# cloneofsimo/vqgan-training

Hardware: NVIDIA H100
Metric: images/sec (higher is better)
Workload: dtype bf16

## Files before the change

include/vqb200.h:

```cpp
#ifndef VQB200_H_
#define VQB200_H_

#include <stddef.h>
#include <stdint.h>

#ifdef __cplusplus
extern "C" {
#endif

#define VQB_OK 0
#define VQB_EINVAL (-1)
#define VQB_ENODEVICE (-2)
#define VQB_ECUDA (-3)

#define VQB_MAX_VIEWS 16
#define VQB_MAX_TAPS 16

#define VQB_EPI_BIAS 1
#define VQB_EPI_RES 2
#define VQB_EPI_RELU 4
#define VQB_EPI_MASK 8
#define VQB_EPI_STATS 16

typedef struct VqbView {
    int64_t offset;
    int32_t Wv, Hv, Nv;
    int32_t _pad;
    int64_t sw, sh, sn;
} VqbView;

typedef struct VqbTap {
    int32_t view, dw, dh, _pad;
} VqbTap;

typedef struct VqbConvDesc {
    int32_t C;
    int32_t Cout;
    int32_t N, H, W;
    int32_t nviews, ntaps;
    int32_t flags;
    int32_t out_f32;
    int32_t _pad;
    int64_t on, oh, ow, oc;
    VqbView views[VQB_MAX_VIEWS];
    VqbTap taps[VQB_MAX_TAPS];
} VqbConvDesc;

int vqb_conv_gemm(const VqbConvDesc* d, const void* a, const void* w_packed ,
                  const float* bias, const void* res, const void* mask, void* out, float* stats, void* stream);

typedef struct VqbWgradDesc {
    int32_t C;
    int32_t Cout;
    int32_t N, H, W;
    int32_t nviews, ntaps;
    int32_t ksplit;
    int64_t ld_override;
    int64_t col_offset;
    VqbView dy_view;
    VqbView views[VQB_MAX_VIEWS];
    VqbTap taps[VQB_MAX_TAPS];
} VqbWgradDesc;

int vqb_conv_stats_ok(const VqbConvDesc* d);

int vqb_wgrad_gemm(const VqbWgradDesc* d, const void* dy, const void* x, float* partial, void* stream);

int vqb_wgrad_cols(int ntaps, int C);

int vqb_wgrad_reduce(const float* partial, float* grad, int ksplit, int Cout, int CoutPad, int Cin, int T, int nslots,
                     int C64, const int* tapmap_dev, int accumulate, void* stream);

int vqb_pack_weights(const float* w_oihw, void* out, int Cout, int Cin, int T, int nslots, const int* tapmap_dev,
                     int transpose, int Kpad, void* stream);

int vqb_pack_weights_fold(const float* w_oihw, void* out, int Cout, int Cin, int T, int nslots, const int* tapmask_dev,
                          int transpose, int Kpad, void* stream);
int vqb_wgrad_reduce_fold(const float* partial, float* grad, int ksplit, int Cout, int CoutPad, int Cin, int T,
                          int nslots, int C64, const int* tapmask_dev, void* stream);

int vqb_nchw_to_nhwc(const float* x, void* y, int N, int C, int H, int W, int Cpad, const float* shift,
                     const float* inv_scale, void* stream);
int vqb_nhwc_to_nchw(const void* g, float* gx, int N, int C, int H, int W, int Cpad, const float* inv_scale,
                     void* stream);
int vqb_nchw_to_nhwc_pad(const float* x, void* y, int N, int C, int H, int W, int Cpad, int pad, const float* shift,
                         const float* inv_scale, void* stream);
int vqb_nhwc_to_nchw_pad(const void* g, float* gx, int N, int C, int H, int W, int Cpad, int pad,
                         const float* inv_scale, void* stream);

int vqb_gn_silu_fwd(const void* x, void* y, const float* gamma, const float* beta, float* mr, double* ws, int N,
                    int HW, int C, int G, float eps, int silu, void* stream);
int vqb_gn_silu_fwd_pre(const void* x, void* y, const float* gamma, const float* beta, float* mr, const float* chsums,
                        int N, int HW, int C, int G, float eps, int silu, void* stream);
int vqb_gn_silu_apply(const void* x, void* y, const float* gamma, const float* beta, const float* mr, int N, int HW,
                      int C, int G, int silu, void* stream);
int vqb_gn_silu_bwd(const void* x, const void* dy, const void* add, void* dx, const float* gamma, const float* beta,
                    const float* mr, float* dgamma, float* dbeta, float* ws, int N, int HW, int C, int G, int silu,
                    float* dx_colsum, void* stream);

int vqb_wavelet_fwd(const float* x, void* y, const float* filt, int N, int C, int H, int W, int Cpad, void* stream);

int vqb_pack_weights_bf16(const void* w_oihw, void* out, int Cout, int Cin, int T, int nslots, const int* tapmap_dev,
                          int transpose, int Kpad, void* stream);
int vqb_pack_weights_fold_bf16(const void* w_oihw, void* out, int Cout, int Cin, int T, int nslots,
                               const int* tapmask_dev, int transpose, int Kpad, void* stream);
int vqb_nchw_to_nhwc_bf16(const void* x, void* y, int N, int C, int H, int W, int Cpad, const float* shift,
                          const float* inv_scale, void* stream);
int vqb_nchw_to_nhwc_pad_bf16(const void* x, void* y, int N, int C, int H, int W, int Cpad, int pad,
                              const float* shift, const float* inv_scale, void* stream);
int vqb_nhwc_to_nchw_bf16(const void* y, void* x, int N, int C, int H, int W, int Cpad, void* stream);
int vqb_wavelet_fwd_bf16(const void* x, void* y, const float* filt, int N, int C, int H, int W, int Cpad,
                         void* stream);

#define VQB_MAX_VIEWS_3D 8
#define VQB_MAX_TAPS_3D 27

typedef struct VqbView3d {
    int64_t offset;
    int32_t Wv, Hv, Tv, Nv;
    int64_t sw, sh, st, sn;
} VqbView3d;

typedef struct VqbTap3d {
    int32_t view, dw, dh, dt;
} VqbTap3d;

typedef struct VqbConv3dDesc {
    int32_t C;
    int32_t Cout;
    int32_t N, T, H, W;
    int32_t nviews, ntaps;
    int32_t flags;
    int32_t out_f32;
    int64_t on, ot, oh, ow, oc;
    VqbView3d views[VQB_MAX_VIEWS_3D];
    VqbTap3d taps[VQB_MAX_TAPS_3D];
} VqbConv3dDesc;

int vqb_conv3d_gemm(const VqbConv3dDesc* d, const void* a, const void* w_packed ,
                    const float* bias, const void* res, void* out, void* stream);

#define VQB_MAX_TAPS_3D_DGRAD 64
typedef struct VqbConv3dDgradDesc {
    int32_t C;
    int32_t Cout;
    int32_t N, T, H, W;
    int32_t nviews, ntaps;
    int32_t flags;
    int32_t out_f32;
    int64_t on, ot, oh, ow, oc;
    VqbView3d views[VQB_MAX_VIEWS_3D];
    VqbTap3d taps[VQB_MAX_TAPS_3D_DGRAD];
} VqbConv3dDgradDesc;

int vqb_conv3d_dgrad_gemm(const VqbConv3dDgradDesc* d, const void* dy, const void* w_packed ,
                          void* dx, void* stream);

typedef struct VqbWgrad3dDesc {
    int32_t C;
    int32_t Cout;
    int32_t N, T, H, W;
    int32_t nviews, ntaps;
    int32_t ksplit, _pad;
    int64_t ld_override;
    int64_t col_offset;
    VqbView3d dy_view;
    VqbView3d views[VQB_MAX_VIEWS_3D];
    VqbTap3d taps[VQB_MAX_TAPS_3D];
} VqbWgrad3dDesc;

int vqb_wgrad3d_gemm(const VqbWgrad3dDesc* d, const void* dy, const void* x, float* partial, void* stream);

int vqb_attn_fwd_hd(const void* qkv, void* out, float* lse, int N, int T, int C, int head_dim, void* stream);
int vqb_attn_bwd_hd(const void* qkv, const void* out, const void* dout, const float* lse, float* dvec, void* dqkv,
                    int N, int T, int C, int head_dim, void* stream);

int vqb_gauss_reparam(const void* z, const void* eps, void* out, int N, int Z, int64_t S, int bf16, void* stream);
int vqb_gauss_reparam_bwd(const float* g, const float* z, const float* eps, float* dz, int N, int Z, int64_t S,
                          void* stream);

int vqb_ncthw_frames_to_nhwc_pad(const float* x, void* y, int B, int C, int T, int H, int W, int Cpad, int pad,
// ... 67 lines not shown
```

vqgan-training_b200/ae.py:

```python
from __future__ import annotations

import math
import os
import sys

_HERE = os.path.dirname(os.path.abspath(__file__))
if _HERE not in sys.path:
    sys.path.insert(0, _HERE)

import torch
import torch.nn.functional as F
from torch import Tensor, nn

import ops
import plans
from utils import wavelet_transform_multi_channel


class Act:

    __slots__ = ("t", "C", "stats", "framed")

    def __init__(self, t: Tensor, C: int, stats=None, framed=False):
        self.t = t
        self.C = C
        self.stats = stats
        self.framed = framed

    @property
    def shape(self):
        n, h, w, _ = self.t.shape
        return (n, self.C, h, w)


def _param_dtype(module: nn.Module):
    p = next(module.parameters(), None)
    if p is None:
        return torch.float32
    ops.check_master_dtype(p, f"{type(module).__name__} parameter")
    return p.dtype


def _enter(x, module: nn.Module):
    if isinstance(x, Act):
        return x, False
    _param_dtype(module)
    return Act(ops.to_nhwc(x), x.shape[1]), True


def _exit(a: Act, external: bool, module: nn.Module):
    return ops.to_nchw(a.t, a.C, _param_dtype(module)) if external else a


def _stats_fusion() -> bool:
    return torch.is_grad_enabled()


def swish(x):
    if isinstance(x, Act):
        raise RuntimeError("swish on internal activations is fused into FP32GroupNorm.forward(..., silu=True)")
    return x * torch.sigmoid(x)


class StandardizedC2d(nn.Conv2d):

    def __init__(self, *args, **kwargs):
        super().__init__(*args, **kwargs)
        self._packed = ops.PackedCache()

    def _kind(self):
        k, s, p = self.kernel_size[0], self.stride[0], self.padding[0]
        if s == 1 and p == (k - 1) // 2:
            return "s1"
        if s == 2 and k == 3 and p == 0:
            return "s2"
        if s == k and p == 0:
            return "patch"
        raise NotImplementedError(f"conv k={k} s={s} p={p} is not on the hot path")

    def forward_act(self, a: Act, residual: Act = None, relu=False, input_is_relu=False, nchw_out=False,
                    want_stats=False):
        want_stats = want_stats and not nchw_out
        kind = "fat3" if a.framed else self._kind()
        out = ops.conv(a.t, self.weight, self.bias, self._packed, kind,
                       residual.t if residual is not None else None, relu, input_is_relu, nchw_out, want_stats)
        if nchw_out:
            return out
        if want_stats:
            return Act(out[0], self.out_channels, out[1])
        return Act(out, self.out_channels)

    def forward(self, x):
        if isinstance(x, Act):
            return self.forward_act(x)
        if self._kind() == "s2":
            raise RuntimeError("stride-2 StandardizedC2d is only reachable through Downsample")
        a, ext = _enter(x, self)
        return _exit(self.forward_act(a), ext, self)


class FP32GroupNorm(nn.GroupNorm):

    def __init__(self, *args, **kwargs):
        super().__init__(*args, **kwargs)

    def forward(self, input, silu: bool = False):
        a, ext = _enter(input, self)
        y = ops.group_norm_silu(a.t, self.weight, self.bias, self.num_groups, self.eps, silu, chsums=a.stats)
        return _exit(Act(y, a.C), ext, self)

    def forward_with_skip(self, a: "Act", silu: bool = True):
        y, skip = ops.group_norm_silu(a.t, self.weight, self.bias, self.num_groups, self.eps, silu, with_skip=True,
                                      chsums=a.stats)
        return Act(y, a.C), Act(skip, a.C)


class AttnBlock(nn.Module):
    def __init__(self, in_channels: int):
        super().__init__()
        self.in_channels = in_channels

        self.head_dim = 64
        self.num_heads = in_channels // self.head_dim
        self.norm = FP32GroupNorm(num_groups=32, num_channels=in_channels, eps=1e-6, affine=True)
        self.qkv = StandardizedC2d(in_channels, in_channels * 3, kernel_size=1, bias=False)
        self.proj_out = StandardizedC2d(in_channels, in_channels, kernel_size=1, bias=False)
        nn.init.normal_(self.proj_out.weight, std=0.2 / math.sqrt(in_channels))

    def attention(self, h_) -> Act:
        a, _ = _enter(h_, self)
        return self.attention_from_normed(self.norm(a))

    def attention_from_normed(self, h: Act) -> Act:
        qkv = self.qkv.forward_act(h)
        import attention as attn_core

        o = attn_core.mhsa(qkv.t, self.num_heads, self.head_dim)
        return Act(o, self.in_channels)

    def forward(self, x):
        a, ext = _enter(x, self)
        hn, a_skip = self.norm.forward_with_skip(a, silu=False)
        h = self.attention_from_normed(hn)
        out = self.proj_out.forward_act(h, residual=a_skip)
        return _exit(out, ext, self)


class ResnetBlock(nn.Module):
    def __init__(self, in_channels: int, out_channels: int):
        super().__init__()
        self.in_channels = in_channels
        out_channels = in_channels if out_channels is None else out_channels
        self.out_channels = out_channels
        self.norm1 = FP32GroupNorm(num_groups=32, num_channels=in_channels, eps=1e-6, affine=True)
        self.conv1 = StandardizedC2d(in_channels, out_channels, kernel_size=3, stride=1, padding=1)
        self.norm2 = FP32GroupNorm(num_groups=32, num_channels=out_channels, eps=1e-6, affine=True)
        self.conv2 = StandardizedC2d(out_channels, out_channels, kernel_size=3, stride=1, padding=1)
        if self.in_channels != self.out_channels:
            self.nin_shortcut = StandardizedC2d(in_channels, out_channels, kernel_size=1, stride=1, padding=0)

        nn.init.normal_(self.conv2.weight, std=0.0001 / self.out_channels)
        nn.init.zeros_(self.conv2.bias)
        self.counter = 0

    def _recompute(self, a: Act) -> Act:
        nin = self.nin_shortcut if self.in_channels != self.out_channels else None
        spec = (self.norm1.num_groups, self.norm1.eps, self.norm2.num_groups, self.norm2.eps, self.conv1._packed,
                self.conv2._packed, nin._packed if nin is not None else None)
        out, stats = ops.resnet_block_recompute(
            a.t, a.stats, spec, self.norm1.weight, self.norm1.bias, self.conv1.weight, self.conv1.bias,
            self.norm2.weight, self.norm2.bias, self.conv2.weight, self.conv2.bias,
            nin.weight if nin is not None else None, nin.bias if nin is not None else None)
        return Act(out, self.out_channels, stats)

    def forward(self, x):
        a, ext = _enter(x, self)
        if torch.is_grad_enabled() and getattr(self, "_vqb_recompute", False):
            return _exit(self._recompute(a), ext, self)
        h, a_skip = self.norm1.forward_with_skip(a, silu=True)
        h = self.conv1.forward_act(h, want_stats=_stats_fusion())
        h = self.norm2(h, silu=True)
        skip = self.nin_shortcut.forward_act(a_skip) if self.in_channels != self.out_channels else a_skip
        out = self.conv2.forward_act(h, residual=skip, want_stats=_stats_fusion())
        return _exit(out, ext, self)


def enable_recompute(module: nn.Module, enabled: bool = True) -> nn.Module:
    for m in module.modules():
        if isinstance(m, ResnetBlock):
            m._vqb_recompute = bool(enabled)
    return module


class Downsample(nn.Module):
    def __init__(self, in_channels: int):
        super().__init__()
        self.conv = StandardizedC2d(in_channels, in_channels, kernel_size=3, stride=2, padding=0)
# ... 254 lines not shown
```

vqgan-training_b200/csrc/common.cu:

```cuda
#include "common.cuh"

#include <atomic>
#include <cstring>
#include <cudaTypedefs.h>
#include <mutex>

namespace vqb {

static thread_local char g_err[512] = "";
static std::atomic<int> g_launches{0};

int set_error(int code, const char* fmt, ...) {
    va_list ap;
    va_start(ap, fmt);
    vsnprintf(g_err, sizeof(g_err), fmt, ap);
    va_end(ap);
    return code;
}

void count_launch(int n) { g_launches.fetch_add(n, std::memory_order_relaxed); }

typedef CUresult (*EncodeTiledFn)(CUtensorMap*, CUtensorMapDataType, cuuint32_t, void*, const cuuint64_t*,
                                  const cuuint64_t*, const cuuint32_t*, const cuuint32_t*, CUtensorMapInterleave,
                                  CUtensorMapSwizzle, CUtensorMapL2promotion, CUtensorMapFloatOOBfill);
// ... 7 lines not shown
        if (cudaGetDriverEntryPoint("cuTensorMapEncodeTiled", &p, cudaEnableDefault, &q) == cudaSuccess &&
            q == cudaDriverEntryPointSuccess)
            fn = reinterpret_cast<EncodeTiledFn>(p);
        else
            (void)cudaGetLastError();
    });
    return fn;
}

int encode_tmap_bf16(CUtensorMap* out, const void* base, int rank, const uint64_t* dims, const uint64_t* strides_bytes,
                     const uint32_t* box, int swizzle_bytes) {
    EncodeTiledFn fn = get_encode_fn();
    if (!fn) return set_error(VQB_ENODEVICE, "cuTensorMapEncodeTiled driver entry point unavailable");
    if ((reinterpret_cast<uintptr_t>(base) & 15u) != 0)
        return set_error(VQB_EINVAL, "tensor map base %p not 16-byte aligned", base);
    cuuint64_t gdim[5];
    cuuint64_t gstr[4];
    cuuint32_t bx[5];
    cuuint32_t es[5];
    for (int i = 0; i < rank; ++i) {
        gdim[i] = dims[i];
        bx[i] = box[i];
        es[i] = 1;
        if (box[i] == 0 || box[i] > 256) return set_error(VQB_EINVAL, "tensor map box[%d]=%u out of range", i, box[i]);
    }
    for (int i = 0; i + 1 < rank; ++i) {
        gstr[i] = strides_bytes[i];
        if (gstr[i] % 16 != 0) return set_error(VQB_EINVAL, "tensor map stride[%d]=%llu not a multiple of 16 B", i,
                                                (unsigned long long)gstr[i]);
    }
    CUtensorMapSwizzle sw = CU_TENSOR_MAP_SWIZZLE_NONE;
    if (swizzle_bytes == 32) sw = CU_TENSOR_MAP_SWIZZLE_32B;
    if (swizzle_bytes == 64) sw = CU_TENSOR_MAP_SWIZZLE_64B;
    if (swizzle_bytes == 128) sw = CU_TENSOR_MAP_SWIZZLE_128B;
    CUresult r = fn(out, CU_TENSOR_MAP_DATA_TYPE_BFLOAT16, static_cast<cuuint32_t>(rank), const_cast<void*>(base), gdim,
                    gstr, bx, es, CU_TENSOR_MAP_INTERLEAVE_NONE, sw, CU_TENSOR_MAP_L2_PROMOTION_L2_256B,
                    CU_TENSOR_MAP_FLOAT_OOB_FILL_NONE);
    if (r == CUDA_ERROR_INVALID_CONTEXT || r == CUDA_ERROR_NOT_INITIALIZED) {
        cudaFree(nullptr);
        r = fn(out, CU_TENSOR_MAP_DATA_TYPE_BFLOAT16, static_cast<cuuint32_t>(rank), const_cast<void*>(base), gdim, gstr,
               bx, es, CU_TENSOR_MAP_INTERLEAVE_NONE, sw, CU_TENSOR_MAP_L2_PROMOTION_L2_256B,
               CU_TENSOR_MAP_FLOAT_OOB_FILL_NONE);
    }
    if (r != CUDA_SUCCESS) {
        return set_error(VQB_ECUDA,
                         "cuTensorMapEncodeTiled failed (%d): rank %d dims [%llu %llu %llu %llu] box [%u %u %u %u] "
                         "stride0 %llu",
                         (int)r, rank, (unsigned long long)gdim[0], (unsigned long long)(rank > 1 ? gdim[1] : 0),
                         (unsigned long long)(rank > 2 ? gdim[2] : 0), (unsigned long long)(rank > 3 ? gdim[3] : 0),
                         bx[0], rank > 1 ? bx[1] : 0, rank > 2 ? bx[2] : 0, rank > 3 ? bx[3] : 0,
                         (unsigned long long)(rank > 1 ? gstr[0] : 0));
    }
    return VQB_OK;
}

int num_sms() {
    static int n = 0;
    if (n == 0) {
        int dev = 0;
        if (cudaGetDevice(&dev) != cudaSuccess) return 0;
        if (cudaDeviceGetAttribute(&n, cudaDevAttrMultiProcessorCount, dev) != cudaSuccess) n = 0;
    }
    return n;
}

bool device_is_sm90() {
    int dev = 0, major = 0;
    if (cudaGetDevice(&dev) != cudaSuccess) {
        (void)cudaGetLastError();
        return false;
    }
    if (cudaDeviceGetAttribute(&major, cudaDevAttrComputeCapabilityMajor, dev) != cudaSuccess) {
        (void)cudaGetLastError();
        return false;
    }
    return major == 9;
}

}

extern "C" {

const char* vqb_last_error(void) { return vqb::g_err; }
int vqb_version(void) { return 103; }
int vqb_device_ok(void) { return (vqb::device_is_sm90() && vqb::get_encode_fn() != nullptr) ? 1 : 0; }
int vqb_kernel_launch_count(void) { return vqb::g_launches.load(std::memory_order_relaxed); }

}
```

vqgan-training_b200/csrc/conv_gemm.cu:

```cuda
#include "common.cuh"
#include "ptx.cuh"

#include <cstring>

namespace vqb {

constexpr int kBlockM = 128;
constexpr int kBlockK = 64;
constexpr int kABytes = kBlockM * kBlockK * 2;
constexpr int kThreads = 384;
constexpr int kMaxStages = 8;
constexpr int kConsumerWarps = 8;
constexpr int kProducerRegs = 40;
constexpr int kConsumerRegs = 232;
constexpr int kStagedKChunksPerTensor = 18;

struct alignas(64) ConvParams {
    static constexpr int kRank = 4;
    static constexpr int kViews = VQB_MAX_VIEWS;
    CUtensorMap amap[VQB_MAX_VIEWS];
    CUtensorMap bmap;
    CUtensorMap omap;
    CUtensorMap emap;
    int32_t tap_view[VQB_MAX_TAPS];
    int32_t tap_dw[VQB_MAX_TAPS];
    int32_t tap_dh[VQB_MAX_TAPS];
    int32_t ntaps, kchunks, C, Cout;
    int32_t N, H, W;
    int32_t lbw, lbh, lbn;
    int32_t tiles_w, tiles_h;
    int32_t n_tiles, total_tiles;
    int32_t stages, do_stats;
    int32_t flags, out_f32;
    int32_t vec_store, _pad0;
    int64_t on, oh, ow, oc;
    void* out;
    const void* res;
    const void* mask;
    const float* bias;
    float* stats;
};

template <int kTaps>
struct alignas(64) Conv3dParamsT {
    static constexpr int kRank = 5;
    static constexpr int kViews = VQB_MAX_VIEWS_3D;
    CUtensorMap amap[VQB_MAX_VIEWS_3D];
    CUtensorMap bmap;
    int32_t tap_view[kTaps];
    int32_t tap_dw[kTaps];
    int32_t tap_dh[kTaps];
    int32_t tap_dt[kTaps];
    int32_t ntaps, kchunks, C, Cout;
    int32_t N, T, H, W;
    int32_t lbw, lbh, lbt, lbn;
    int32_t tiles_w, tiles_h, tiles_t;
    int32_t n_tiles, total_tiles;
    int32_t stages, do_stats;
    int32_t flags, out_f32;
    int32_t vec_store, _pad0;
    int64_t on, ot, oh, ow, oc;
    void* out;
    const void* res;
    const void* mask;
    const float* bias;
    float* stats;
};
using Conv3dParams = Conv3dParamsT<VQB_MAX_TAPS_3D>;
using Conv3dDgradParams = Conv3dParamsT<VQB_MAX_TAPS_3D_DGRAD>;

template <int BN, class P, bool kStaged>
__global__ void __launch_bounds__(kThreads, 1) conv_gemm_kernel(const __grid_constant__ P p) {
    constexpr bool kR5 = P::kRank == 5;
    static_assert(!kStaged || (!kR5 && BN >= 64), "the staged epilogue stores whole 64-channel slabs of 2-D outputs");
    extern __shared__ uint8_t smem_raw[];
    constexpr uint32_t kBBytes = BN * kBlockK * 2;
    constexpr uint32_t kStageBytes = kABytes + kBBytes;
    uint8_t* base = smem_raw + ((1024u - (smem_u32(smem_raw) & 1023u)) & 1023u);
    const uint32_t stages = p.stages;
    constexpr uint32_t kSlabBytes = kBlockM * kBlockK * 2;
    constexpr uint32_t kEpiBytes = kBlockM * BN * 2;
    constexpr uint32_t kRowOff[4] = {0, 8 * 128, 64 * 128, 72 * 128};
    uint8_t* epi = base + stages * kStageBytes;
    float* sStat = reinterpret_cast<float*>(epi + (kStaged ? 2 * kEpiBytes : 0));
    uint64_t* full = reinterpret_cast<uint64_t*>(sStat + kConsumerWarps * BN * 2);
    uint64_t* empty = full + stages;
    uint64_t* order = empty + stages;
    uint64_t* epi_full = order + 2;
    uint64_t* epi_empty = epi_full + 2;
    const uint32_t wg = threadIdx.x >> 7;
    const uint32_t warp = (threadIdx.x >> 5) & 3u;
    const uint32_t lane = threadIdx.x & 31u;

    if (threadIdx.x == 0) {
        for (int v = 0; v < P::kViews; ++v) {
            bool used = false;
            for (int t = 0; t < p.ntaps; ++t) used |= (p.tap_view[t] == v);
            if (used) tma_prefetch_desc(&p.amap[v]);
        }
        tma_prefetch_desc(&p.bmap);
        if constexpr (kStaged) {
            tma_prefetch_desc(&p.omap);
            if (p.flags & (VQB_EPI_RES | VQB_EPI_MASK)) tma_prefetch_desc(&p.emap);
        }
        for (uint32_t i = 0; i < stages; ++i) {
            mbar_init(&full[i], 1);
            mbar_init(&empty[i], 4);
        }
        for (int c = 0; c < 2; ++c) {
            mbar_init(&order[c], 4);
            mbar_init(&epi_full[c], 1);
            mbar_init(&epi_empty[c], 1);
        }
        fence_mbar_init();
    }
    __syncthreads();

    const int num_kb = p.ntaps * p.kchunks;
    if (wg == 0) {
        setmaxnreg_dec<kProducerRegs>();
        if (warp == 0 && elect_one()) {
            uint32_t stage = 0, phase = 0;
            for (int tile = blockIdx.x, l = 0; tile < p.total_tiles; tile += gridDim.x, ++l) {
                const int n_tile = tile % p.n_tiles;
                const int m_tile = tile / p.n_tiles;
                const int tw = m_tile % p.tiles_w;
                const int th = (m_tile / p.tiles_w) % p.tiles_h;
                int tt = 0, tn;
                if constexpr (kR5) {
                    tt = (m_tile / (p.tiles_w * p.tiles_h)) % p.tiles_t;
                    tn = m_tile / (p.tiles_w * p.tiles_h * p.tiles_t);
                } else {
                    tn = m_tile / (p.tiles_w * p.tiles_h);
                }
                const int w0 = tw << p.lbw, h0 = th << p.lbh, n0 = tn << p.lbn;
                const int ncol0 = n_tile * BN;
                if constexpr (kStaged) {
                    const uint32_t c = l & 1;
                    mbar_wait(&epi_empty[c], ((l >> 1) & 1) ^ 1);
                    if (p.flags & (VQB_EPI_RES | VQB_EPI_MASK)) {
                        const int nslab = min(BN, p.Cout - ncol0) / kBlockK;
                        mbar_arrive_expect_tx(&epi_full[c], nslab * kSlabBytes);
                        for (int s = 0; s < nslab; ++s)
                            tma_load_4d(&p.emap, &epi_full[c], epi + c * kEpiBytes + s * kSlabBytes,
                                        ncol0 + s * kBlockK, w0, h0, n0);
                    } else {
                        mbar_arrive(&epi_full[c]);
                    }
                }
                for (int t = 0; t < p.ntaps; ++t) {
                    for (int kc = 0; kc < p.kchunks; ++kc) {
                        mbar_wait(&empty[stage], phase ^ 1);
                        uint8_t* a_dst = base + stage * kStageBytes;
                        mbar_arrive_expect_tx(&full[stage], kStageBytes);
                        if constexpr (kR5)
                            tma_load_5d(&p.amap[p.tap_view[t]], &full[stage], a_dst, kc * kBlockK, w0 + p.tap_dw[t],
                                        h0 + p.tap_dh[t], (tt << p.lbt) + p.tap_dt[t], n0);
                        else
                            tma_load_4d(&p.amap[p.tap_view[t]], &full[stage], a_dst, kc * kBlockK, w0 + p.tap_dw[t],
                                        h0 + p.tap_dh[t], n0);
                        tma_load_2d(&p.bmap, &full[stage], a_dst + kABytes, t * p.C + kc * kBlockK, ncol0);
                        if (++stage == stages) {
                            stage = 0;
                            phase ^= 1;
                        }
                    }
                }
            }
        }
        return;
    }

    setmaxnreg_inc<kConsumerRegs>();
    const uint32_t cw = wg - 1;
    const uint32_t cwarp = cw * 4 + warp;
    const uint32_t wtid = threadIdx.x & 127u;
    const uint32_t ring = smem_u32(base);
    const bool has_bias = p.flags & VQB_EPI_BIAS, has_res = p.flags & VQB_EPI_RES;
    const bool do_relu = !kR5 && (p.flags & VQB_EPI_RELU), has_mask = !kR5 && (p.flags & VQB_EPI_MASK);
    const bool vec_path = p.vec_store != 0;
    const bool reduce = !kR5 && p.do_stats;
    const __nv_bfloat16* res = reinterpret_cast<const __nv_bfloat16*>(p.res);
    const __nv_bfloat16* mask = reinterpret_cast<const __nv_bfloat16*>(p.mask);
    float acc[2][BN / 2];
#pragma unroll
    for (int mb = 0; mb < 2; ++mb)
#pragma unroll
        for (int i = 0; i < BN / 2; ++i) acc[mb][i] = 0.f;
    uint32_t stage = 0, phase = 0;
    for (int l = static_cast<int>(cw);; l += 2) {
        const int tile = blockIdx.x + l * gridDim.x;
        if (tile >= p.total_tiles) break;
        if (l > 0) {
            stage += num_kb;
            phase ^= (stage / stages) & 1u;
            stage %= stages;
            mbar_wait(&order[cw ^ 1u], ((l - 1) >> 1) & 1);
        }
        uint32_t prev = 0;
        for (int kb = 0; kb < num_kb; ++kb) {
            mbar_wait(&full[stage], phase);
            if (kb == num_kb - 1 && lane == 0) mbar_arrive(&order[cw]);
            const uint32_t a = ring + stage * kStageBytes;
            const uint64_t da0 = make_smem_desc(a, 16, 1024);
            const uint64_t da1 = make_smem_desc(a + 8192u, 16, 1024);
            const uint64_t db = make_smem_desc(a + kABytes, 16, 1024);
            fence_operands(acc[0]);
            fence_operands(acc[1]);
            wgmma_fence();
#pragma unroll
            for (int k = 0; k < kBlockK / 16; ++k) {
                wgmma_bf16<BN, 0, 0>(acc[0], da0 + 2 * k, db + 2 * k, (kb | k) != 0 ? 1u : 0u);
                wgmma_bf16<BN, 0, 0>(acc[1], da1 + 2 * k, db + 2 * k, (kb | k) != 0 ? 1u : 0u);
            }
            wgmma_commit();
            fence_operands(acc[0]);
            fence_operands(acc[1]);
            wgmma_wait<1>();
            if (kb > 0 && lane == 0) mbar_arrive(&empty[prev]);
            prev = stage;
            if (++stage == stages) {
                stage = 0;
                phase ^= 1;
            }
        }
        wgmma_wait<0>();
        fence_operands(acc[0]);
        fence_operands(acc[1]);
        if (lane == 0) mbar_arrive(&empty[prev]);

        const int n_tile = tile % p.n_tiles;
        const int m_tile = tile / p.n_tiles;
        const int tw = m_tile % p.tiles_w;
        const int th = (m_tile / p.tiles_w) % p.tiles_h;
        int tt = 0, tn;
        if constexpr (kR5) {
            tt = (m_tile / (p.tiles_w * p.tiles_h)) % p.tiles_t;
            tn = m_tile / (p.tiles_w * p.tiles_h * p.tiles_t);
        } else {
            tn = m_tile / (p.tiles_w * p.tiles_h);
        }
        const int col0 = n_tile * BN;
        uint8_t* tbuf = epi + cw * kEpiBytes;
        const uint32_t trow = smem_u32(tbuf) + (warp * 16 + (lane >> 2)) * 128u + (lane & 3u) * 4u;
        if (kStaged) mbar_wait(&epi_full[cw], (l >> 1) & 1);
        int64_t pix[4] = {0, 0, 0, 0};
        bool valid[4] = {true, true, true, true};
        if constexpr (!kStaged) {
#pragma unroll
            for (int r = 0; r < 4; ++r) {
                const uint32_t row = (r >> 1) * 64 + warp * 16 + (lane >> 2) + 8 * (r & 1);
                const int w = (tw << p.lbw) + static_cast<int>(row & ((1u << p.lbw) - 1));
                const int h = (th << p.lbh) + static_cast<int>((row >> p.lbw) & ((1u << p.lbh) - 1));
                if constexpr (kR5) {
                    const int t = (tt << p.lbt) + static_cast<int>((row >> (p.lbw + p.lbh)) & ((1u << p.lbt) - 1));
                    const int n = (tn << p.lbn) + static_cast<int>(row >> (p.lbw + p.lbh + p.lbt));
                    valid[r] = (w < p.W) && (h < p.H) && (t < p.T) && (n < p.N);
                    pix[r] = static_cast<int64_t>(n) * p.on + static_cast<int64_t>(t) * p.ot +
                             static_cast<int64_t>(h) * p.oh + static_cast<int64_t>(w) * p.ow;
                } else {
                    const int n = (tn << p.lbn) + static_cast<int>(row >> (p.lbw + p.lbh));
                    valid[r] = (w < p.W) && (h < p.H) && (n < p.N);
                    pix[r] = static_cast<int64_t>(n) * p.on + static_cast<int64_t>(h) * p.oh +
                             static_cast<int64_t>(w) * p.ow;
                }
            }
        }
#pragma unroll
        for (int j = 0; j < BN / 8; ++j) {
            const int col = col0 + j * 8 + 2 * static_cast<int>(lane & 3u);
            const bool ok0 = col < p.Cout, ok1 = col + 1 < p.Cout;
            float b0 = 0.f, b1 = 0.f;
            if (has_bias) {
                b0 = ok0 ? __ldg(p.bias + col) : 0.f;
                b1 = ok1 ? __ldg(p.bias + col + 1) : 0.f;
            }
            float r1[2] = {0.f, 0.f}, r2[2] = {0.f, 0.f};
            if (kStaged ? ok1 : vec_path && ok1) {
                __nv_bfloat162 rv[4], mv[4];
                const uint32_t tj = trow + (j >> 3) * kSlabBytes + (((j & 7u) ^ (lane >> 2)) << 4);
#pragma unroll
                for (int r = 0; r < 4; ++r) {
                    rv[r] = mv[r] = __floats2bfloat162_rn(0.f, 0.f);
                    if constexpr (kStaged) {
                        if (has_res || has_mask) {
                            const __nv_bfloat162 v = u32_as_bf16x2(ld_shared_u32(tj + kRowOff[r]));
                            if (has_res) rv[r] = v;
                            if (has_mask) mv[r] = v;
                        }
                        continue;
                    }
                    const int64_t o = pix[r] + col;
                    if (has_res && valid[r]) rv[r] = *reinterpret_cast<const __nv_bfloat162*>(res + o);
                    if (has_mask && valid[r]) mv[r] = *reinterpret_cast<const __nv_bfloat162*>(mask + o);
                }
#pragma unroll
                for (int r = 0; r < 4; ++r) {
                    if (!valid[r]) continue;
                    const int a0 = 4 * j + 2 * (r & 1);
                    float f[2] = {acc[r >> 1][a0] + b0, acc[r >> 1][a0 + 1] + b1};
                    if (has_res) {
                        const float2 rf = __bfloat1622float2(rv[r]);
                        f[0] += rf.x;
                        f[1] += rf.y;
                    }
                    if (do_relu) {
                        f[0] = fmaxf(f[0], 0.f);
                        f[1] = fmaxf(f[1], 0.f);
                    }
                    if (has_mask) {
                        const float2 m = __bfloat1622float2(mv[r]);
                        if (!(m.x > 0.f)) f[0] = 0.f;
                        if (!(m.y > 0.f)) f[1] = 0.f;
                    }
                    const __nv_bfloat162 ob = __floats2bfloat162_rn(f[0], f[1]);
                    if constexpr (kStaged)
                        st_shared_u32(tj + kRowOff[r], bf16x2_as_u32(ob));
                    else
                        *reinterpret_cast<__nv_bfloat162*>(reinterpret_cast<__nv_bfloat16*>(p.out) + pix[r] + col) = ob;
                    if (reduce) {
                        const float2 v = __bfloat1622float2(ob);
                        r1[0] += v.x;
                        r2[0] = fmaf(v.x, v.x, r2[0]);
                        r1[1] += v.y;
                        r2[1] = fmaf(v.y, v.y, r2[1]);
                    }
                }
            } else if constexpr (!kStaged) {
#pragma unroll
                for (int r = 0; r < 4; ++r) {
                    if (!valid[r]) continue;
                    const int a0 = 4 * j + 2 * (r & 1);
                    const float f[2] = {acc[r >> 1][a0] + b0, acc[r >> 1][a0 + 1] + b1};
#pragma unroll
                    for (int e = 0; e < 2; ++e) {
                        if (!(e ? ok1 : ok0)) continue;
                        const int64_t o = pix[r] + static_cast<int64_t>(col + e) * p.oc;
                        float x = f[e];
                        if (has_res) x += __bfloat162float(res[o]);
                        if (do_relu) x = fmaxf(x, 0.f);
                        if (has_mask && !(__bfloat162float(mask[o]) > 0.f)) x = 0.f;
                        if (p.out_f32)
                            reinterpret_cast<float*>(p.out)[o] = x;
                        else
                            reinterpret_cast<__nv_bfloat16*>(p.out)[o] = __float2bfloat16(x);
                    }
                }
            }
            if (reduce) {
#pragma unroll
                for (int off = 4; off < 32; off <<= 1) {
#pragma unroll
                    for (int e = 0; e < 2; ++e) {
                        r1[e] += __shfl_xor_sync(0xffffffffu, r1[e], off);
                        r2[e] += __shfl_xor_sync(0xffffffffu, r2[e], off);
                    }
                }
                if (lane < 4) {
                    float* s = sStat + (cwarp * BN + j * 8 + 2 * lane) * 2;
                    *reinterpret_cast<float4*>(s) = make_float4(r1[0], r2[0], r1[1], r2[1]);
                }
            }
        }
        if constexpr (kStaged) {
            fence_proxy_async_shared();
            named_bar_sync(1 + cw, 128);
            if (wtid == 0) {
                const int nslab = min(BN, p.Cout - col0) / kBlockK;
                for (int s = 0; s < nslab; ++s)
                    tma_store_4d(&p.omap, tbuf + s * kSlabBytes, col0 + s * kBlockK, tw << p.lbw, th << p.lbh,
                                 tn << p.lbn);
                bulk_commit_group();
            }
        }
        if (reduce) {
            named_bar_sync(1 + cw, 128);
            const int n_img = tn << p.lbn;
            const float* sw = sStat + cw * 4 * BN * 2;
            for (uint32_t idx = wtid; idx < BN * 2u; idx += 128u) {
                const int c = col0 + static_cast<int>(idx >> 1);
                float v = 0.f;
#pragma unroll
                for (int w4 = 0; w4 < 4; ++w4) v += sw[w4 * BN * 2 + idx];
                if (c < p.Cout) atomicAdd(p.stats + (static_cast<int64_t>(n_img) * p.Cout + c) * 2 + (idx & 1u), v);
            }
            named_bar_sync(1 + cw, 128);
        }
        if (kStaged && wtid == 0) {
            bulk_wait_group_read<0>();
            mbar_arrive(&epi_empty[cw]);
        }
    }
    if (kStaged && wtid == 0) bulk_wait_group<0>();
}

static int fill_views(const VqbView* views, int nviews, const void* a, int C, int lbw, int lbh, int lbn,
                      CUtensorMap* maps) {
    for (int v = 0; v < nviews; ++v) {
        const VqbView& vw = views[v];
        uint64_t dims[4] = {static_cast<uint64_t>(C), static_cast<uint64_t>(vw.Wv), static_cast<uint64_t>(vw.Hv),
                            static_cast<uint64_t>(vw.Nv)};
        uint64_t str[3] = {static_cast<uint64_t>(vw.sw) * 2, static_cast<uint64_t>(vw.sh) * 2,
                           static_cast<uint64_t>(vw.sn) * 2};
        uint32_t box[4] = {kBlockK, 1u << lbw, 1u << lbh, 1u << lbn};
        const void* base = static_cast<const uint8_t*>(a) + vw.offset * 2;
        int rc = encode_tmap_bf16(&maps[v], base, 4, dims, str, box, 128);
        if (rc != VQB_OK) return rc;
    }
    return VQB_OK;
}

static size_t conv_smem_bytes(int block_n, int stages, bool staged) {
    return 1024 + static_cast<size_t>(stages) * (kABytes + block_n * kBlockK * 2) +
           (staged ? 2 * kBlockM * block_n * 2 : 0) + kConsumerWarps * block_n * 2 * sizeof(float) + 8 * (2 * stages + 6);
}

static int ring_stages(int block_n, bool staged) {
    int stages = kMaxStages;
    while (conv_smem_bytes(block_n, stages, staged) > 227 * 1024) --stages;
    return stages;
}

template <int BN, bool kStaged = false, class P>
static int launch_conv(const P& p, void* stream) {
    const size_t smem = conv_smem_bytes(BN, p.stages, kStaged);
    static bool attr_set = false;
    if (!attr_set) {
        VQB_CUDA(cudaFuncSetAttribute(conv_gemm_kernel<BN, P, kStaged>, cudaFuncAttributeMaxDynamicSharedMemorySize,
                                      227 * 1024));
        attr_set = true;
    }
    const int grid = p.total_tiles < num_sms() ? p.total_tiles : num_sms();
    conv_gemm_kernel<BN, P, kStaged><<<grid, kThreads, smem, static_cast<cudaStream_t>(stream)>>>(p);
    VQB_CUDA(cudaGetLastError());
    return VQB_OK;
}

}

using namespace vqb;

static int conv_gemm_impl(const VqbConvDesc* d, const void* a, const void* w_packed, const float* bias, const void* res,
                          const void* mask, void* out, float* stats, void* stream, bool query_only);

extern "C" int vqb_conv_gemm(const VqbConvDesc* d, const void* a, const void* w_packed, const float* bias,
                             const void* res, const void* mask, void* out, float* stats, void* stream) {
    return conv_gemm_impl(d, a, w_packed, bias, res, mask, out, stats, stream, false);
}

extern "C" int vqb_conv_stats_ok(const VqbConvDesc* d) {
    if (!d) return 0;
    VqbConvDesc q = *d;
    q.flags &= ~VQB_EPI_STATS;
    alignas(16) static const uint64_t dummy_aligned[4] = {0, 0, 0, 0};
    const void* dp = dummy_aligned;
    const int r = conv_gemm_impl(&q, dp, dp, static_cast<const float*>(dp), dp, dp, const_cast<void*>(dp), nullptr,
                                 nullptr, true);
    return r == 1 ? 1 : 0;
}

static int conv_gemm_impl(const VqbConvDesc* d, const void* a, const void* w_packed, const float* bias, const void* res,
                          const void* mask, void* out, float* stats, void* stream, bool query_only) {
    VQB_CHECK(d && a && w_packed && out, "vqb_conv_gemm: null pointer");
    VQB_CHECK(d->C > 0 && d->C % 8 == 0, "vqb_conv_gemm: C=%d must be a positive multiple of 8", d->C);
    VQB_CHECK(d->Cout > 0 && d->N > 0 && d->H > 0 && d->W > 0, "vqb_conv_gemm: bad extents");
    VQB_CHECK(d->ntaps >= 1 && d->ntaps <= VQB_MAX_TAPS && d->nviews >= 1 && d->nviews <= VQB_MAX_VIEWS,
              "vqb_conv_gemm: ntaps=%d nviews=%d out of range", d->ntaps, d->nviews);
    VQB_CHECK(((int64_t)d->ntaps * d->C) % 8 == 0, "vqb_conv_gemm: weight row stride must be 16-byte aligned");
    if ((d->flags & VQB_EPI_BIAS))
        VQB_CHECK(bias != nullptr && (reinterpret_cast<uintptr_t>(bias) & 15u) == 0,
                  "vqb_conv_gemm: VQB_EPI_BIAS needs a 16-byte aligned bias pointer");
    if ((d->flags & VQB_EPI_RES)) VQB_CHECK(res != nullptr, "vqb_conv_gemm: VQB_EPI_RES without res");
    if ((d->flags & VQB_EPI_MASK)) VQB_CHECK(mask != nullptr, "vqb_conv_gemm: VQB_EPI_MASK without mask");
    if ((d->flags & VQB_EPI_STATS)) VQB_CHECK(stats != nullptr, "vqb_conv_gemm: VQB_EPI_STATS without stats");
    const uintptr_t ops = reinterpret_cast<uintptr_t>(res) | reinterpret_cast<uintptr_t>(mask);
    const bool nhwc_bf16 = d->oc == 1 && !d->out_f32 && d->on % 8 == 0 && d->oh % 8 == 0 && d->ow % 8 == 0 &&
                           (reinterpret_cast<uintptr_t>(out) & 15u) == 0 && (ops & 3u) == 0;
    if (!nhwc_bf16)
        VQB_CHECK((reinterpret_cast<uintptr_t>(out) & (d->out_f32 ? 3u : 1u)) == 0 && (ops & 1u) == 0,
                  "vqb_conv_gemm: misaligned output / residual / mask");
    for (int t = 0; t < d->ntaps; ++t)
        VQB_CHECK(d->taps[t].view >= 0 && d->taps[t].view < d->nviews, "vqb_conv_gemm: tap %d view out of range", t);
    if (!query_only && !device_is_sm90()) return set_error(VQB_ENODEVICE, "vqb_conv_gemm: current device is not sm_90");

    ConvParams p;
    const int block_n = d->Cout > 64 ? 128 : (d->Cout > 32 ? 64 : (d->Cout > 16 ? 32 : 16));
    p.n_tiles = (d->Cout + block_n - 1) / block_n;
    uint32_t bw = next_pow2(d->W);
    if (bw > 128) bw = 128;
    uint32_t bh = next_pow2(d->H);
    if (bh > 128 / bw) bh = 128 / bw;
    const uint32_t bn = 128 / (bw * bh);
    p.lbw = ilog2(bw);
    p.lbh = ilog2(bh);
    p.lbn = ilog2(bn);
    p.tiles_w = (d->W + bw - 1) / bw;
    p.tiles_h = (d->H + bh - 1) / bh;
    const int tiles_nb = (d->N + bn - 1) / bn;
    p.total_tiles = p.tiles_w * p.tiles_h * tiles_nb * p.n_tiles;
    const bool stats_ok = nhwc_bf16 && bn == 1 && (d->W % bw == 0) && (d->H % bh == 0) && (d->Cout % 64 == 0);
    if (d->flags & VQB_EPI_STATS) {
        if (!stats_ok)
            return set_error(VQB_EINVAL, "vqb_conv_gemm: VQB_EPI_STATS unsupported for this shape (N=%d H=%d W=%d Cout=%d)",
                             d->N, d->H, d->W, d->Cout);
    }
    p.do_stats = (d->flags & VQB_EPI_STATS) ? 1 : 0;
    if (query_only) return stats_ok ? 1 : 0;
    const bool has_res = d->flags & VQB_EPI_RES, has_mask = d->flags & VQB_EPI_MASK;
    const void* eop = has_res ? res : mask;
    const int moved = (has_res || has_mask) ? 2 : 1;
    const bool staged = nhwc_bf16 && d->Cout % 64 == 0 && d->on > 0 && d->oh > 0 && d->ow > 0 &&
                        !(has_res && has_mask) && (reinterpret_cast<uintptr_t>(eop) & 15u) == 0 &&
                        d->ntaps * ((d->C + kBlockK - 1) / kBlockK) <= kStagedKChunksPerTensor * moved;
    p.stages = ring_stages(block_n, staged);
    p.ntaps = d->ntaps;
    p.kchunks = (d->C + kBlockK - 1) / kBlockK;
    p.C = d->C;
    p.Cout = d->Cout;
    p.N = d->N;
    p.H = d->H;
    p.W = d->W;
    p.flags = d->flags;
    p.out_f32 = d->out_f32;
    p.vec_store = nhwc_bf16 ? 1 : 0;
    p._pad0 = 0;
    p.on = d->on;
    p.oh = d->oh;
    p.ow = d->ow;
    p.oc = d->oc;
    p.out = out;
    p.res = res;
    p.mask = mask;
    p.bias = bias;
    p.stats = stats;
    for (int t = 0; t < d->ntaps; ++t) {
        p.tap_view[t] = d->taps[t].view;
        p.tap_dw[t] = d->taps[t].dw;
        p.tap_dh[t] = d->taps[t].dh;
    }
    int rc = fill_views(d->views, d->nviews, a, d->C, p.lbw, p.lbh, p.lbn, p.amap);
    if (rc != VQB_OK) return rc;
    if (staged) {
        uint64_t dims[4] = {static_cast<uint64_t>(d->Cout), static_cast<uint64_t>(d->W), static_cast<uint64_t>(d->H),
                            static_cast<uint64_t>(d->N)};
        uint64_t str[3] = {static_cast<uint64_t>(d->ow) * 2, static_cast<uint64_t>(d->oh) * 2,
                           static_cast<uint64_t>(d->on) * 2};
        uint32_t box[4] = {kBlockK, bw, bh, bn};
        rc = encode_tmap_bf16(&p.omap, out, 4, dims, str, box, 128);
        if (rc == VQB_OK && (has_res || has_mask)) rc = encode_tmap_bf16(&p.emap, eop, 4, dims, str, box, 128);
        if (rc != VQB_OK) return rc;
    }
    {
        const uint64_t ktot = static_cast<uint64_t>(d->ntaps) * d->C;
        uint64_t dims[2] = {ktot, static_cast<uint64_t>(d->Cout)};
        uint64_t str[1] = {ktot * 2};
        uint32_t box[2] = {kBlockK, static_cast<uint32_t>(block_n)};
        rc = encode_tmap_bf16(&p.bmap, w_packed, 2, dims, str, box, 128);
        if (rc != VQB_OK) return rc;
    }
    switch (block_n) {
        case 16: rc = launch_conv<16>(p, stream); break;
        case 32: rc = launch_conv<32>(p, stream); break;
        case 64: rc = staged ? launch_conv<64, true>(p, stream) : launch_conv<64>(p, stream); break;
        default: rc = staged ? launch_conv<128, true>(p, stream) : launch_conv<128>(p, stream); break;
    }
    if (rc != VQB_OK) return rc;
    count_launch();
    return VQB_OK;
}

template <class D, class P, int kMaxTaps>
static int conv3d_impl(const char* fn, const D* d, const void* a, const void* w_packed, const float* bias,
                       const void* res, void* out, void* stream) {
    VQB_CHECK(d && a && w_packed && out, "%s: null pointer", fn);
    VQB_CHECK(d->C > 0 && d->C % 8 == 0, "%s: C=%d must be a positive multiple of 8", fn, d->C);
    VQB_CHECK(d->Cout > 0 && d->N > 0 && d->T > 0 && d->H > 0 && d->W > 0, "%s: bad extents", fn);
    VQB_CHECK(d->ntaps >= 1 && d->ntaps <= kMaxTaps && d->nviews >= 1 && d->nviews <= VQB_MAX_VIEWS_3D,
              "%s: ntaps=%d nviews=%d out of range", fn, d->ntaps, d->nviews);
    VQB_CHECK((d->flags & ~(VQB_EPI_BIAS | VQB_EPI_RES)) == 0,
              "%s: flags 0x%x: only VQB_EPI_BIAS and VQB_EPI_RES are supported", fn, d->flags);
    VQB_CHECK(d->out_f32 == 0 || d->out_f32 == 1, "%s: out_f32 must be 0 or 1", fn);
    if (d->flags & VQB_EPI_BIAS)
        VQB_CHECK(bias != nullptr && (reinterpret_cast<uintptr_t>(bias) & 15u) == 0,
                  "%s: VQB_EPI_BIAS needs a 16-byte aligned bias pointer", fn);
    if (d->flags & VQB_EPI_RES) VQB_CHECK(res != nullptr, "%s: VQB_EPI_RES without res", fn);
    VQB_CHECK(d->on >= 0 && d->ot >= 0 && d->oh >= 0 && d->ow >= 0 && d->oc > 0,
              "%s: output strides must be non-negative (oc > 0)", fn);
    const bool vec3 = d->oc == 1 && !d->out_f32 && d->on % 8 == 0 && d->ot % 8 == 0 && d->oh % 8 == 0 &&
                      d->ow % 8 == 0 && (reinterpret_cast<uintptr_t>(out) & 15u) == 0 &&
                      (reinterpret_cast<uintptr_t>(res) & 3u) == 0;
    if (!vec3)
        VQB_CHECK((reinterpret_cast<uintptr_t>(out) & (d->out_f32 ? 3u : 1u)) == 0 &&
                      (reinterpret_cast<uintptr_t>(res) & 1u) == 0,
                  "%s: misaligned output / residual", fn);
    for (int v = 0; v < d->nviews; ++v) {
        const VqbView3d& vw = d->views[v];
        VQB_CHECK(vw.offset >= 0 && vw.Wv > 0 && vw.Hv > 0 && vw.Tv > 0 && vw.Nv > 0 && vw.sw > 0 && vw.sw % 8 == 0 &&
                      vw.sh > 0 && vw.sh % 8 == 0 && vw.st > 0 && vw.st % 8 == 0 && vw.sn > 0 && vw.sn % 8 == 0,
                  "%s: view %d has bad extents / strides (strides must be positive multiples of 8)", fn, v);
    }
    for (int t = 0; t < d->ntaps; ++t)
        VQB_CHECK(d->taps[t].view >= 0 && d->taps[t].view < d->nviews, "%s: tap %d view out of range", fn, t);
    if (!device_is_sm90()) return set_error(VQB_ENODEVICE, "%s: current device is not sm_90", fn);

    P p;
    memset(&p, 0, sizeof(p));
    const int block_n = d->Cout > 64 ? 128 : (d->Cout > 32 ? 64 : (d->Cout > 16 ? 32 : 16));
    p.n_tiles = (d->Cout + block_n - 1) / block_n;
    uint32_t bw = next_pow2(d->W);
    if (bw > 128) bw = 128;
    uint32_t bh = next_pow2(d->H);
    if (bh > 128 / bw) bh = 128 / bw;
    uint32_t bt = next_pow2(d->T);
    if (bt > 128 / (bw * bh)) bt = 128 / (bw * bh);
    const uint32_t bn = 128 / (bw * bh * bt);
    p.lbw = ilog2(bw);
    p.lbh = ilog2(bh);
    p.lbt = ilog2(bt);
    p.lbn = ilog2(bn);
    p.tiles_w = (d->W + bw - 1) / bw;
    p.tiles_h = (d->H + bh - 1) / bh;
    p.tiles_t = (d->T + bt - 1) / bt;
    const int64_t total = static_cast<int64_t>(p.tiles_w) * p.tiles_h * p.tiles_t * ((d->N + bn - 1) / bn) * p.n_tiles;
    VQB_CHECK(total < (1ll << 31), "%s: too many tiles", fn);
    p.total_tiles = static_cast<int32_t>(total);
    p.stages = ring_stages(block_n, false);
    p.ntaps = d->ntaps;
    p.kchunks = (d->C + kBlockK - 1) / kBlockK;
    p.C = d->C;
    p.Cout = d->Cout;
    p.N = d->N;
    p.T = d->T;
    p.H = d->H;
    p.W = d->W;
    p.flags = d->flags;
    p.out_f32 = d->out_f32;
    p.vec_store = vec3 ? 1 : 0;
    p.on = d->on;
    p.ot = d->ot;
    p.oh = d->oh;
    p.ow = d->ow;
    p.oc = d->oc;
    p.out = out;
    p.res = res;
    p.bias = bias;
    for (int t = 0; t < d->ntaps; ++t) {
        p.tap_view[t] = d->taps[t].view;
// ... 50 lines not shown
```

vqgan-training_b200/csrc/elementwise.cu:

```cuda
#ifndef VQB_EXACT_SIGMOID
#define VQB_EXACT_SIGMOID 0
#endif
#include "common.cuh"
#include "ptx.cuh"

namespace vqb {

__device__ __forceinline__ void load8(const __nv_bfloat16* p, float (&f)[8]) {
    const uint4 u = *reinterpret_cast<const uint4*>(p);
    float2 a = unpack_bf16x2(u.x), b = unpack_bf16x2(u.y), c = unpack_bf16x2(u.z), d = unpack_bf16x2(u.w);
    f[0] = a.x; f[1] = a.y; f[2] = b.x; f[3] = b.y; f[4] = c.x; f[5] = c.y; f[6] = d.x; f[7] = d.y;
}
__device__ __forceinline__ uint4 ldg16(const __nv_bfloat16* p) { return __ldg(reinterpret_cast<const uint4*>(p)); }
__device__ __forceinline__ void cvt8(const uint4& u, float (&f)[8]) {
    float2 a = unpack_bf16x2(u.x), b = unpack_bf16x2(u.y), c = unpack_bf16x2(u.z), d = unpack_bf16x2(u.w);
    f[0] = a.x; f[1] = a.y; f[2] = b.x; f[3] = b.y; f[4] = c.x; f[5] = c.y; f[6] = d.x; f[7] = d.y;
}
__device__ __forceinline__ void store8(__nv_bfloat16* p, const float (&f)[8]) {
    uint4 u;
    u.x = pack_bf16x2(f[0], f[1]);
    u.y = pack_bf16x2(f[2], f[3]);
    u.z = pack_bf16x2(f[4], f[5]);
    u.w = pack_bf16x2(f[6], f[7]);
    *reinterpret_cast<uint4*>(p) = u;
}
__device__ __forceinline__ float sigmoidf_(float x) {
#if VQB_EXACT_SIGMOID
    return 1.f / (1.f + __expf(-x));
#else
    float t;
    asm("tanh.approx.f32 %0, %1;" : "=f"(t) : "f"(0.5f * x));
    return fmaf(0.5f, t, 0.5f);
#endif
}

__device__ __forceinline__ float tanh_fast(float x) {
#if VQB_EXACT_SIGMOID
    return 2.f / (1.f + __expf(-2.f * x)) - 1.f;
#else
    float t;
    asm("tanh.approx.f32 %0, %1;" : "=f"(t) : "f"(x));
    return t;
#endif
}

template <typename Src>
__global__ void pack_weights_kernel(const Src* __restrict__ w, __nv_bfloat16* __restrict__ out, int Cout, int Cin,
                                    int T, int nslots, const int* __restrict__ tapmap, int transpose, int Kpad) {
    const int R = transpose ? Cin : Cout;
    const int K = transpose ? Cout : Cin;
    const int64_t total = static_cast<int64_t>(R) * nslots * Kpad;
    for (int64_t i = blockIdx.x * static_cast<int64_t>(blockDim.x) + threadIdx.x; i < total;
         i += static_cast<int64_t>(gridDim.x) * blockDim.x) {
        const int k = static_cast<int>(i % Kpad);
        const int slot = static_cast<int>((i / Kpad) % nslots);
        const int r = static_cast<int>(i / (static_cast<int64_t>(Kpad) * nslots));
        float v = 0.f;
        if (k < K) {
            const int tap = tapmap[slot];
            const int co = transpose ? k : r, ci = transpose ? r : k;
            v = to_f32(w[(static_cast<int64_t>(co) * Cin + ci) * T + tap]);
        }
        out[i] = __float2bfloat16(v);
    }
}

template <typename Src>
__global__ void pack_weights_fold_kernel(const Src* __restrict__ w, __nv_bfloat16* __restrict__ out, int Cout,
                                         int Cin, int T, int nslots, const int* __restrict__ tapmask, int transpose,
                                         int Kpad) {
    const int R = transpose ? Cin : Cout;
    const int K = transpose ? Cout : Cin;
    const int64_t total = static_cast<int64_t>(R) * nslots * Kpad;
    for (int64_t i = blockIdx.x * static_cast<int64_t>(blockDim.x) + threadIdx.x; i < total;
         i += static_cast<int64_t>(gridDim.x) * blockDim.x) {
        const int k = static_cast<int>(i % Kpad);
        const int slot = static_cast<int>((i / Kpad) % nslots);
        const int r = static_cast<int>(i / (static_cast<int64_t>(Kpad) * nslots));
        float v = 0.f;
        if (k < K) {
            const int mask = tapmask[slot];
            const int co = transpose ? k : r, ci = transpose ? r : k;
            const Src* wp = w + (static_cast<int64_t>(co) * Cin + ci) * T;
            for (int t = 0; t < T; ++t)
                if ((mask >> t) & 1) v += to_f32(wp[t]);
        }
        out[i] = __float2bfloat16(v);
    }
}

template <typename In>
__global__ void nchw_to_nhwc_kernel(const In* __restrict__ x, __nv_bfloat16* __restrict__ y, int N, int C, int HW,
                                    int Cpad, const float* __restrict__ shift, const float* __restrict__ inv_scale,
                                    int W, int pad) {
    const int64_t total = static_cast<int64_t>(N) * HW;
    const int H = HW / W;
    for (int64_t i = blockIdx.x * static_cast<int64_t>(blockDim.x) + threadIdx.x; i < total;
         i += static_cast<int64_t>(gridDim.x) * blockDim.x) {
        const int64_t n = i / HW, p = i % HW;
        const In* xp = x + n * C * HW + p;
        int64_t opix = i;
        if (pad) {
            const int h = static_cast<int>(p / W), w = static_cast<int>(p % W);
            opix = (n * (H + 2 * pad) + h + pad) * (W + 2 * pad) + w + pad;
        }
        __nv_bfloat16* yp = y + opix * Cpad;
        for (int c0 = 0; c0 < Cpad; c0 += 8) {
            float f[8];
#pragma unroll
            for (int j = 0; j < 8; ++j) {
                const int c = c0 + j;
                float v = 0.f;
                if (c < C) {
                    v = to_f32(xp[static_cast<int64_t>(c) * HW]);
                    if (shift) v = (v - shift[c]) * inv_scale[c];
                }
                f[j] = v;
            }
            store8(yp + c0, f);
        }
    }
}

template <typename Out>
__global__ void nhwc_to_nchw_kernel(const __nv_bfloat16* __restrict__ g, Out* __restrict__ gx, int N, int C, int HW,
// ... 180 lines not shown
    const int n = blockIdx.y, cpg = C / G;
    float a[8], b[8];
#pragma unroll
    for (int j = 0; j < 8; ++j) {
        const int c = cv * 8 + j, g = c / cpg;
        const float mean = mr[(n * G + g) * 2], rstd = mr[(n * G + g) * 2 + 1];
        a[j] = rstd * gamma[c];
        b[j] = beta[c] - mean * a[j];
    }
    const int p0 = blockIdx.x * pix_per_chunk;
    const int p1 = min(HW, p0 + pix_per_chunk);
    const int64_t base = (static_cast<int64_t>(n) * HW) * C + cv * 8;
    int p = p0 + pr;
    for (; p + 3 * R < p1; p += 4 * R) {
        uint4 u4[4];
#pragma unroll
        for (int k = 0; k < 4; ++k) u4[k] = ldg16(x + base + static_cast<int64_t>(p + k * R) * C);
#pragma unroll
        for (int k = 0; k < 4; ++k) {
            float f[8];
            cvt8(u4[k], f);
#pragma unroll
            for (int j = 0; j < 8; ++j) {
                float u = fmaf(a[j], f[j], b[j]);
                f[j] = silu ? u * sigmoidf_(u) : u;
            }
            store8(y + base + static_cast<int64_t>(p + k * R) * C, f);
        }
    }
    for (; p < p1; p += R) {
        float f[8];
        load8(x + base + static_cast<int64_t>(p) * C, f);
#pragma unroll
        for (int j = 0; j < 8; ++j) {
            float u = fmaf(a[j], f[j], b[j]);
            f[j] = silu ? u * sigmoidf_(u) : u;
        }
        store8(y + base + static_cast<int64_t>(p) * C, f);
    }
}

__global__ void gn_bwd_reduce_kernel(const __nv_bfloat16* __restrict__ x, const __nv_bfloat16* __restrict__ dy,
                                     const float* __restrict__ mr, const float* __restrict__ gamma,
                                     const float* __restrict__ beta, float* __restrict__ cs , int HW,
                                     int C, int G, int pix_per_chunk, int silu) {
    extern __shared__ float sm[];
    const int V = C >> 3, R = blockDim.x / V;
    const int cv = threadIdx.x % V, pr = threadIdx.x / V;
    const int n = blockIdx.y, cpg = C / G;
    for (int i = threadIdx.x; i < 2 * C; i += blockDim.x) sm[i] = 0.f;
    __syncthreads();
    if (pr < R) {
        float mean[8], rstd[8], a2[8], b2[8], s1[8], s2[8];
#pragma unroll
        for (int j = 0; j < 8; ++j) {
            const int c = cv * 8 + j, g = c / cpg;
            mean[j] = mr[(n * G + g) * 2];
            rstd[j] = mr[(n * G + g) * 2 + 1];
            const float a = gamma[c] * rstd[j];
            a2[j] = 0.5f * a;
            b2[j] = 0.5f * (beta[c] - mean[j] * a);
            s1[j] = s2[j] = 0.f;
        }
        const int p0 = blockIdx.x * pix_per_chunk;
        const int p1 = min(HW, p0 + pix_per_chunk);
        const int64_t base = (static_cast<int64_t>(n) * HW) * C + cv * 8;
        constexpr int U = 4;
        for (int p = p0 + pr; p < p1; p += U * R) {
            uint4 ux[U], ud[U];
#pragma unroll
            for (int k = 0; k < U; ++k) {
                const bool in = (p + k * R) < p1;
                ux[k] = in ? ldg16(x + base + static_cast<int64_t>(p + k * R) * C) : make_uint4(0, 0, 0, 0);
                ud[k] = in ? ldg16(dy + base + static_cast<int64_t>(p + k * R) * C) : make_uint4(0, 0, 0, 0);
            }
#pragma unroll
            for (int k = 0; k < U; ++k) {
                if ((p + k * R) >= p1) break;
                float f[8], d[8];
                cvt8(ux[k], f);
                cvt8(ud[k], d);
#pragma unroll
                for (int j = 0; j < 8; ++j) {
                    float du2 = 2.f * d[j];
                    if (silu) {
                        const float h = fmaf(f[j], a2[j], b2[j]);
                        const float t = tanh_fast(h);
                        const float r = fmaf(-h, t, h + 1.f);
                        du2 = d[j] * fmaf(t, r, r);
                    }
                    s1[j] += du2;
                    s2[j] = fmaf(du2, f[j] - mean[j], s2[j]);
                }
            }
        }
#pragma unroll
        for (int j = 0; j < 8; ++j) {
            atomicAdd(&sm[(cv * 8 + j) * 2], 0.5f * s1[j]);
            atomicAdd(&sm[(cv * 8 + j) * 2 + 1], 0.5f * rstd[j] * s2[j]);
        }
    }
    __syncthreads();
    for (int i = threadIdx.x; i < 2 * C; i += blockDim.x) atomicAdd(&cs[static_cast<int64_t>(n) * 2 * C + i], sm[i]);
}

__global__ void gn_bwd_finalize_kernel(const float* __restrict__ cs, const float* __restrict__ gamma,
                                       float* __restrict__ gs , float* __restrict__ dgamma,
                                       float* __restrict__ dbeta, int N, int C, int G, int HW) {
    const int i = blockIdx.x * blockDim.x + threadIdx.x;
    const int cpg = C / G;
    if (i < N * G) {
        const int n = i / G, g = i % G;
        float a = 0.f, b = 0.f;
        for (int c = g * cpg; c < (g + 1) * cpg; ++c) {
            a += gamma[c] * cs[(static_cast<int64_t>(n) * C + c) * 2];
            b += gamma[c] * cs[(static_cast<int64_t>(n) * C + c) * 2 + 1];
        }
        const float m = static_cast<float>(cpg) * HW;
        gs[i * 2] = a / m;
        gs[i * 2 + 1] = b / m;
    }
    if (i < C) {
        float a = 0.f, b = 0.f;
        for (int n = 0; n < N; ++n) {
            a += cs[(static_cast<int64_t>(n) * C + i) * 2];
            b += cs[(static_cast<int64_t>(n) * C + i) * 2 + 1];
        }
        dbeta[i] = a;
        dgamma[i] = b;
    }
}

template <bool ADD, int U>
__global__ void __launch_bounds__(256, 2)
gn_bwd_apply_kernel(const __nv_bfloat16* __restrict__ x, const __nv_bfloat16* __restrict__ dy,
                    const __nv_bfloat16* __restrict__ add, __nv_bfloat16* __restrict__ dx,
                    const float* __restrict__ mr, const float* __restrict__ gs, const float* __restrict__ gamma,
                    const float* __restrict__ beta, int HW, int C, int G, int pix_per_chunk, int silu,
                    float* __restrict__ colsum ) {
    extern __shared__ float sm[];
    const int V = C >> 3, R = blockDim.x / V;
    const int cv = threadIdx.x % V, pr = threadIdx.x / V;
    if (colsum) {
        for (int i = threadIdx.x; i < C; i += blockDim.x) sm[i] = 0.f;
        __syncthreads();
    }
    if (pr < R) {
        const int n = blockIdx.y, cpg = C / G;
        float mean[8], a2[8], b2[8], k0[8], k2[8], cs8[8];
#pragma unroll
        for (int j = 0; j < 8; ++j) {
            const int c = cv * 8 + j, g = c / cpg;
            mean[j] = mr[(n * G + g) * 2];
            const float rstd = mr[(n * G + g) * 2 + 1];
            const float a = gamma[c] * rstd;
            a2[j] = 0.5f * a;
            b2[j] = 0.5f * (beta[c] - mean[j] * a);
            k0[j] = -rstd * gs[(n * G + g) * 2];
            k2[j] = -rstd * rstd * gs[(n * G + g) * 2 + 1];
            cs8[j] = 0.f;
        }
        const int p0 = blockIdx.x * pix_per_chunk;
        const int p1 = min(HW, p0 + pix_per_chunk);
        const int64_t base = (static_cast<int64_t>(n) * HW) * C + cv * 8;
        for (int pp = p0 + pr; pp < p1; pp += U * R) {
            uint4 ux[U], ud[U], ua[U];
#pragma unroll
            for (int k = 0; k < U; ++k) {
                const bool in = (pp + k * R) < p1;
                const int64_t off = base + static_cast<int64_t>(pp + k * R) * C;
                ux[k] = in ? ldg16(x + off) : make_uint4(0, 0, 0, 0);
                ud[k] = in ? ldg16(dy + off) : make_uint4(0, 0, 0, 0);
                if (ADD) ua[k] = in ? ldg16(add + off) : make_uint4(0, 0, 0, 0);
            }
#pragma unroll
            for (int k = 0; k < U; ++k) {
                if ((pp + k * R) >= p1) break;
                float f[8], d[8], r[8];
                cvt8(ux[k], f);
                cvt8(ud[k], d);
                if (ADD) cvt8(ua[k], r);
#pragma unroll
                for (int j = 0; j < 8; ++j) {
                    float du2 = 2.f * d[j];
                    if (silu) {
                        const float h = fmaf(f[j], a2[j], b2[j]);
                        const float t = tanh_fast(h);
                        const float rr = fmaf(-h, t, h + 1.f);
                        du2 = d[j] * fmaf(t, rr, rr);
                    }
                    float v = fmaf(du2, a2[j], fmaf(f[j] - mean[j], k2[j], k0[j]));
                    if (ADD) v += r[j];
                    f[j] = v;
                    cs8[j] += __bfloat162float(__float2bfloat16(v));
                }
                store8(dx + base + static_cast<int64_t>(pp + k * R) * C, f);
            }
        }
        if (colsum) {
#pragma unroll
            for (int j = 0; j < 8; ++j) atomicAdd(&sm[cv * 8 + j], cs8[j]);
        }
    }
    if (colsum) {
        __syncthreads();
        for (int i = threadIdx.x; i < C; i += blockDim.x) atomicAdd(&colsum[i], sm[i]);
    }
}

__global__ void colsum_kernel(const __nv_bfloat16* __restrict__ x, float* __restrict__ out ,
                              int64_t P, int C, int pix_per_chunk) {
    extern __shared__ float sm[];
    const int V = C >> 3, R = blockDim.x / V;
    const int cv = threadIdx.x % V, pr = threadIdx.x / V;
    for (int i = threadIdx.x; i < C; i += blockDim.x) sm[i] = 0.f;
    __syncthreads();
    if (pr < R) {
        float s[8];
#pragma unroll
        for (int j = 0; j < 8; ++j) s[j] = 0.f;
        const int64_t p0 = static_cast<int64_t>(blockIdx.x) * pix_per_chunk;
        const int64_t p1 = min(P, p0 + pix_per_chunk);
        int64_t p = p0 + pr;
        for (; p + 3 * R < p1; p += 4 * R) {
            uint4 u[4];
#pragma unroll
            for (int k = 0; k < 4; ++k) u[k] = ldg16(x + (p + k * R) * C + cv * 8);
#pragma unroll
            for (int k = 0; k < 4; ++k) {
                float f[8];
                cvt8(u[k], f);
#pragma unroll
                for (int j = 0; j < 8; ++j) s[j] += f[j];
            }
        }
        for (; p < p1; p += R) {
            float f[8];
            load8(x + p * C + cv * 8, f);
#pragma unroll
            for (int j = 0; j < 8; ++j) s[j] += f[j];
        }
#pragma unroll
        for (int j = 0; j < 8; ++j) atomicAdd(&sm[cv * 8 + j], s[j]);
    }
    __syncthreads();
    for (int i = threadIdx.x; i < C; i += blockDim.x) atomicAdd(&out[i], sm[i]);
}

__global__ void wgrad_reduce_kernel(const float* __restrict__ partial, float* __restrict__ grad, int ksplit, int Cout,
                                    int CoutPad, int Cin, int T, int nslots, int C64,
                                    const int* __restrict__ tapmap, int accumulate) {
    const int64_t total = static_cast<int64_t>(Cout) * Cin * T;
    const int64_t ld = static_cast<int64_t>(nslots) * C64;
    for (int64_t i = blockIdx.x * static_cast<int64_t>(blockDim.x) + threadIdx.x; i < total;
         i += static_cast<int64_t>(gridDim.x) * blockDim.x) {
        const int ci = static_cast<int>(i % Cin);
        const int tap = static_cast<int>((i / Cin) % T);
        const int co = static_cast<int>(i / (static_cast<int64_t>(T) * Cin));
        float acc = 0.f;
        bool any = false;
        for (int slot = 0; slot < nslots; ++slot) {
            if (tapmap[slot] != tap) continue;
            any = true;
            for (int s = 0; s < ksplit; ++s)
                acc += partial[(static_cast<int64_t>(s) * CoutPad + co) * ld + static_cast<int64_t>(slot) * C64 + ci];
        }
        const int64_t o = (static_cast<int64_t>(co) * Cin + ci) * T + tap;
        if (any || !accumulate) grad[o] = accumulate ? grad[o] + acc : acc;
    }
}

__global__ void wgrad_reduce_fold_kernel(const float* __restrict__ partial, float* __restrict__ grad, int ksplit,
                                         int Cout, int CoutPad, int Cin, int T, int nslots, int C64,
// ... 336 lines not shown
int vqb_ncthw_frames_to_nhwc(const float* x, void* y, int B, int C, int T, int H, int W, int Cpad, const int* frames,
                             int Tsel, const float* shift, const float* inv_scale, void* stream) {
    return clip_to_frames("vqb_ncthw_frames_to_nhwc", x, y, B, C, T, H, W, Cpad, 0, frames, Tsel, shift, inv_scale,
                          stream);
}

int vqb_ncthw_frames_to_nhwc_bf16(const void* x, void* y, int B, int C, int T, int H, int W, int Cpad,
                                  const int* frames, int Tsel, const float* shift, const float* inv_scale,
                                  void* stream) {
    return clip_to_frames("vqb_ncthw_frames_to_nhwc_bf16", static_cast<const __nv_bfloat16*>(x), y, B, C, T, H, W,
                          Cpad, 0, frames, Tsel, shift, inv_scale, stream);
}

int vqb_nhwc_pad_frames_to_ncthw(const void* g, float* gx, int B, int C, int T, int H, int W, int Cpad, int pad,
                                 const int* frames, int Tsel, const float* inv_scale, void* stream) {
    return frames_to_clip("vqb_nhwc_pad_frames_to_ncthw", g, gx, B, C, T, H, W, Cpad, pad, frames, Tsel, inv_scale,
                          stream);
}

int vqb_nhwc_frames_to_ncthw(const void* g, float* gx, int B, int C, int T, int H, int W, int Cpad, const int* frames,
                             int Tsel, const float* inv_scale, void* stream) {
    return frames_to_clip("vqb_nhwc_frames_to_ncthw", g, gx, B, C, T, H, W, Cpad, 0, frames, Tsel, inv_scale, stream);
}

int vqb_gn_silu_fwd(const void* x, void* y, const float* gamma, const float* beta, float* mr, double* ws, int N,
                    int HW, int C, int G, float eps, int silu, void* stream) {
    VQB_CHECK(x && y && gamma && beta && mr && ws, "vqb_gn_silu_fwd: null pointer");
    VQB_CHECK(C % 8 == 0 && C % G == 0 && C <= 2048, "vqb_gn_silu_fwd: C=%d G=%d unsupported", C, G);
    cudaStream_t st = static_cast<cudaStream_t>(stream);
    VQB_CUDA(cudaMemsetAsync(ws, 0, sizeof(double) * 2 * N * C, st));
    int chunks, ppc;
    const int T = cv_threads(C);
    const size_t stats_smem = static_cast<size_t>(T / (C / 8)) * 2 * C * sizeof(float);
    cv_grid(HW, C, N, gn_stats_kernel, stats_smem, chunks, ppc);
    gn_stats_kernel<<<dim3(chunks, N), T, stats_smem, st>>>(static_cast<const __nv_bfloat16*>(x), ws, HW, C,
                                                                        ppc);
    gn_finalize_kernel<<<(N * G + 127) / 128, 128, 0, st>>>(ws, mr, N, C, G, HW, eps);
    cv_grid(HW, C, N, gn_apply_kernel, 0, chunks, ppc);
    gn_apply_kernel<<<dim3(chunks, N), T, 0, st>>>(static_cast<const __nv_bfloat16*>(x),
                                                   static_cast<__nv_bfloat16*>(y), mr, gamma, beta, HW, C, G, ppc,
                                                   silu);
    VQB_CUDA(cudaGetLastError());
    count_launch(3);
    return VQB_OK;
}

int vqb_gn_silu_apply(const void* x, void* y, const float* gamma, const float* beta, const float* mr, int N, int HW,
                      int C, int G, int silu, void* stream) {
    VQB_CHECK(x && y && gamma && beta && mr, "vqb_gn_silu_apply: null pointer");
    VQB_CHECK(N > 0 && HW > 0 && G > 0 && C % 8 == 0 && C % G == 0 && C <= 2048 && (silu == 0 || silu == 1),
              "vqb_gn_silu_apply: N=%d HW=%d C=%d G=%d silu=%d unsupported", N, HW, C, G, silu);
    VQB_CHECK(((reinterpret_cast<uintptr_t>(x) | reinterpret_cast<uintptr_t>(y)) & 15u) == 0 &&
                  ((reinterpret_cast<uintptr_t>(gamma) | reinterpret_cast<uintptr_t>(beta) |
                    reinterpret_cast<uintptr_t>(mr)) & 3u) == 0,
              "vqb_gn_silu_apply: x and y must be 16-byte aligned, gamma, beta and mr 4-byte aligned");
    if (!device_is_sm90()) return set_error(VQB_ENODEVICE, "vqb_gn_silu_apply: current device is not sm_90");
    int chunks, ppc;
    const int T = cv_threads(C);
    cv_grid(HW, C, N, gn_apply_kernel, 0, chunks, ppc);
    gn_apply_kernel<<<dim3(chunks, N), T, 0, static_cast<cudaStream_t>(stream)>>>(
        static_cast<const __nv_bfloat16*>(x), static_cast<__nv_bfloat16*>(y), mr, gamma, beta, HW, C, G, ppc, silu);
    VQB_CUDA(cudaGetLastError());
    count_launch();
    return VQB_OK;
}

int vqb_gn_silu_fwd_pre(const void* x, void* y, const float* gamma, const float* beta, float* mr, const float* chsums,
                        int N, int HW, int C, int G, float eps, int silu, void* stream) {
    VQB_CHECK(x && y && gamma && beta && mr && chsums, "vqb_gn_silu_fwd_pre: null pointer");
    VQB_CHECK(C % 8 == 0 && C % G == 0 && C <= 2048, "vqb_gn_silu_fwd_pre: C=%d G=%d unsupported", C, G);
    cudaStream_t st = static_cast<cudaStream_t>(stream);
    gn_finalize_f32_kernel<<<(N * G + 127) / 128, 128, 0, st>>>(chsums, mr, N, C, G, HW, eps);
    int chunks, ppc;
    const int T = cv_threads(C);
    cv_grid(HW, C, N, gn_apply_kernel, 0, chunks, ppc);
    gn_apply_kernel<<<dim3(chunks, N), T, 0, st>>>(static_cast<const __nv_bfloat16*>(x),
                                                   static_cast<__nv_bfloat16*>(y), mr, gamma, beta, HW, C, G, ppc,
                                                   silu);
    VQB_CUDA(cudaGetLastError());
    count_launch(2);
    return VQB_OK;
}

int vqb_gn_silu_bwd(const void* x, const void* dy, const void* add, void* dx, const float* gamma, const float* beta,
                    const float* mr, float* dgamma, float* dbeta, float* ws, int N, int HW, int C, int G, int silu,
                    float* dx_colsum, void* stream) {
    VQB_CHECK(x && dy && dx && gamma && beta && mr && dgamma && dbeta && ws, "vqb_gn_silu_bwd: null pointer");
    VQB_CHECK(C % 8 == 0 && C % G == 0 && C <= 2048, "vqb_gn_silu_bwd: C=%d G=%d unsupported", C, G);
    cudaStream_t st = static_cast<cudaStream_t>(stream);
    int chunks, ppc;
    const int T = cv_threads(C);
    float* cs = ws;
    float* gsum = ws + static_cast<int64_t>(N) * C * 2;
    VQB_CUDA(cudaMemsetAsync(cs, 0, sizeof(float) * 2 * N * C, st));
    cv_grid(HW, C, N, gn_bwd_reduce_kernel, 2 * C * sizeof(float), chunks, ppc);
    gn_bwd_reduce_kernel<<<dim3(chunks, N), T, 2 * C * sizeof(float), st>>>(
        static_cast<const __nv_bfloat16*>(x), static_cast<const __nv_bfloat16*>(dy), mr, gamma, beta, cs, HW, C, G,
        ppc, silu);
    count_launch();
    const int fin = (N * G > C ? N * G : C);
    gn_bwd_finalize_kernel<<<(fin + 127) / 128, 128, 0, st>>>(cs, gamma, gsum, dgamma, dbeta, N, C, G, HW);
    const size_t cs_smem = dx_colsum ? C * sizeof(float) : 0;
    if (dx_colsum) VQB_CUDA(cudaMemsetAsync(dx_colsum, 0, sizeof(float) * C, st));
    if (add) {
        cv_grid(HW, C, N, gn_bwd_apply_kernel<true, 2>, cs_smem, chunks, ppc);
        gn_bwd_apply_kernel<true, 2><<<dim3(chunks, N), T, cs_smem, st>>>(
            static_cast<const __nv_bfloat16*>(x), static_cast<const __nv_bfloat16*>(dy),
            static_cast<const __nv_bfloat16*>(add), static_cast<__nv_bfloat16*>(dx), mr, gsum, gamma, beta, HW, C, G,
            ppc, silu, dx_colsum);
    } else {
        cv_grid(HW, C, N, gn_bwd_apply_kernel<false, 3>, cs_smem, chunks, ppc);
        gn_bwd_apply_kernel<false, 3><<<dim3(chunks, N), T, cs_smem, st>>>(
            static_cast<const __nv_bfloat16*>(x), static_cast<const __nv_bfloat16*>(dy), nullptr,
            static_cast<__nv_bfloat16*>(dx), mr, gsum, gamma, beta, HW, C, G, ppc, silu, dx_colsum);
    }
    VQB_CUDA(cudaGetLastError());
    count_launch(2);
    return VQB_OK;
}

int vqb_wavelet_fwd(const float* x, void* y, const float* filt, int N, int C, int H, int W, int Cpad, void* stream) {
    VQB_CHECK(x && y && filt && H % 2 == 0 && W % 2 == 0 && Cpad % 8 == 0 && Cpad >= 4 * C,
              "vqb_wavelet_fwd: bad arguments (H, W even; Cpad >= 4C, multiple of 8)");
    const int64_t total = static_cast<int64_t>(N) * (H / 2) * (W / 2);
    wavelet_fwd_kernel<float><<<gs_blocks(total, 128), 128, 0, static_cast<cudaStream_t>(stream)>>>(
        x, static_cast<__nv_bfloat16*>(y), filt, N, C, H, W, Cpad);
    VQB_CUDA(cudaGetLastError());
    count_launch();
    return VQB_OK;
}

int vqb_wavelet_fwd_bf16(const void* x, void* y, const float* filt, int N, int C, int H, int W, int Cpad,
                         void* stream) {
    VQB_CHECK(x && y && filt && N > 0 && C > 0 && H > 0 && W > 0 && H % 2 == 0 && W % 2 == 0 && Cpad % 8 == 0 &&
                  Cpad >= 4 * C,
              "vqb_wavelet_fwd_bf16: bad arguments (H, W even; Cpad >= 4C, multiple of 8)");
    if (!device_is_sm90()) return set_error(VQB_ENODEVICE, "vqb_wavelet_fwd_bf16: current device is not sm_90");
    const int64_t total = static_cast<int64_t>(N) * (H / 2) * (W / 2);
    wavelet_fwd_kernel<__nv_bfloat16><<<gs_blocks(total, 128), 128, 0, static_cast<cudaStream_t>(stream)>>>(
        static_cast<const __nv_bfloat16*>(x), static_cast<__nv_bfloat16*>(y), filt, N, C, H, W, Cpad);
    VQB_CUDA(cudaGetLastError());
    count_launch();
    return VQB_OK;
}

int vqb_colsum(const void* x, float* out, int64_t P, int C, void* stream) {
    VQB_CHECK(x && out && C % 8 == 0 && C <= 2048, "vqb_colsum: bad arguments");
    cudaStream_t st = static_cast<cudaStream_t>(stream);
    VQB_CUDA(cudaMemsetAsync(out, 0, sizeof(float) * C, st));
    const int V = C / 8, T = cv_threads(C), R = T / V;
    int bpsm = 0;
    if (cudaOccupancyMaxActiveBlocksPerMultiprocessor(&bpsm, colsum_kernel, T, C * sizeof(float)) != cudaSuccess || bpsm < 1)
        bpsm = 4;
    const int64_t concurrent = static_cast<int64_t>(num_sms() > 0 ? num_sms() : 132) * bpsm;
    int64_t nblk = concurrent;
    while (nblk < concurrent * 8 && (P + nblk - 1) / nblk > 2048) nblk += concurrent;
    int64_t ppc = (P + nblk - 1) / nblk;
    if (ppc < R * 4) ppc = R * 4;
    ppc = ((ppc + R - 1) / R) * R;
    const int chunks = static_cast<int>((P + ppc - 1) / ppc);
    colsum_kernel<<<chunks, T, C * sizeof(float), st>>>(static_cast<const __nv_bfloat16*>(x), out, P, C,
                                                        static_cast<int>(ppc));
    VQB_CUDA(cudaGetLastError());
    count_launch();
    return VQB_OK;
}

int vqb_wgrad_reduce(const float* partial, float* grad, int ksplit, int Cout, int CoutPad, int Cin, int T, int nslots,
                     int C64, const int* tapmap_dev, int accumulate, void* stream) {
    VQB_CHECK(partial && grad && tapmap_dev, "vqb_wgrad_reduce: null pointer");
    const int64_t total = static_cast<int64_t>(Cout) * Cin * T;
    wgrad_reduce_kernel<<<gs_blocks(total, 256), 256, 0, static_cast<cudaStream_t>(stream)>>>(
        partial, grad, ksplit, Cout, CoutPad, Cin, T, nslots, C64, tapmap_dev, accumulate);
    VQB_CUDA(cudaGetLastError());
    count_launch();
    return VQB_OK;
}

int vqb_gauss_reparam(const void* z, const void* eps, void* out, int N, int Z, int64_t S, int bf16, void* stream) {
    VQB_CHECK(z && eps && out, "vqb_gauss_reparam: null pointer");
    VQB_CHECK(N > 0 && Z > 0 && S > 0 && (bf16 == 0 || bf16 == 1),
              "vqb_gauss_reparam: bad arguments (N=%d Z=%d S=%lld bf16=%d)", N, Z, (long long)S, bf16);
    if (!device_is_sm90()) return set_error(VQB_ENODEVICE, "vqb_gauss_reparam: current device is not sm_90");
    const int64_t total = static_cast<int64_t>(N) * Z * S;
    cudaStream_t st = static_cast<cudaStream_t>(stream);
    if (bf16)
        gauss_reparam_kernel<__nv_bfloat16><<<gs_blocks(total, 256), 256, 0, st>>>(
            static_cast<const __nv_bfloat16*>(z), static_cast<const __nv_bfloat16*>(eps),
            static_cast<__nv_bfloat16*>(out), Z, S, total);
    else
        gauss_reparam_kernel<float><<<gs_blocks(total, 256), 256, 0, st>>>(
            static_cast<const float*>(z), static_cast<const float*>(eps), static_cast<float*>(out), Z, S, total);
    VQB_CUDA(cudaGetLastError());
    count_launch();
    return VQB_OK;
}

int vqb_gauss_reparam_bwd(const float* g, const float* z, const float* eps, float* dz, int N, int Z, int64_t S,
                          void* stream) {
    VQB_CHECK(g && z && eps && dz, "vqb_gauss_reparam_bwd: null pointer");
    VQB_CHECK(N > 0 && Z > 0 && S > 0, "vqb_gauss_reparam_bwd: bad arguments (N=%d Z=%d S=%lld)", N, Z, (long long)S);
// ... 14 lines not shown
```

vqgan-training_b200/csrc/ptx.cuh:

```cuda
#pragma once
#include <cstdint>
#include <cstdio>
#include <cuda.h>
#include <cuda_runtime.h>
#include <cuda_bf16.h>

namespace vqb {

__device__ __forceinline__ uint32_t smem_u32(const void* p) {
    return static_cast<uint32_t>(__cvta_generic_to_shared(p));
}

__device__ __forceinline__ uint32_t elect_one() {
    uint32_t pred = 0;
    asm volatile(
        "{\n"
        ".reg .b32 %%rx;\n"
        ".reg .pred %%px;\n"
        "elect.sync %%rx|%%px, %1;\n"
        "@%%px mov.s32 %0, 1;\n"
        "}\n"
        : "+r"(pred)
        : "r"(0xFFFFFFFFu));
    return pred;
}

__device__ __forceinline__ void mbar_init(uint64_t* bar, uint32_t count) {
    asm volatile("mbarrier.init.shared::cta.b64 [%0], %1;" ::"r"(smem_u32(bar)), "r"(count) : "memory");
}

__device__ __forceinline__ void fence_mbar_init() {
    asm volatile("fence.mbarrier_init.release.cluster;" ::: "memory");
}

__device__ __forceinline__ void mbar_arrive(uint64_t* bar) {
    asm volatile("mbarrier.arrive.shared::cta.b64 _, [%0];" ::"r"(smem_u32(bar)) : "memory");
}

__device__ __forceinline__ void mbar_arrive_expect_tx(uint64_t* bar, uint32_t bytes) {
    asm volatile("mbarrier.arrive.expect_tx.shared::cta.b64 _, [%0], %1;" ::"r"(smem_u32(bar)), "r"(bytes)
                 : "memory");
}

__device__ __forceinline__ bool mbar_try_wait(uint64_t* bar, uint32_t parity) {
    uint32_t ok;
    asm volatile(
        "{\n"
        ".reg .pred p;\n"
        "mbarrier.try_wait.parity.shared::cta.b64 p, [%1], %2;\n"
        "selp.u32 %0, 1, 0, p;\n"
        "}\n"
        : "=r"(ok)
        : "r"(smem_u32(bar)), "r"(parity)
        : "memory");
    return ok != 0;
}

#ifndef VQB_WATCHDOG
#define VQB_WATCHDOG 1
#endif
__device__ __forceinline__ uint64_t globaltimer_ns() {
    uint64_t t;
    asm volatile("mov.u64 %0, %%globaltimer;" : "=l"(t));
    return t;
}
__device__ __forceinline__ void mbar_wait(uint64_t* bar, uint32_t parity) {
#if VQB_WATCHDOG
    if (mbar_try_wait(bar, parity)) return;
    const uint64_t t0 = globaltimer_ns();
    while (!mbar_try_wait(bar, parity)) {
        if (globaltimer_ns() - t0 > 4000000000ull) __trap();
    }
#else
    while (!mbar_try_wait(bar, parity)) {
    }
#endif
}

__device__ __forceinline__ void tma_prefetch_desc(const void* desc) {
    asm volatile("prefetch.tensormap [%0];" ::"l"(reinterpret_cast<uint64_t>(desc)) : "memory");
}

__device__ __forceinline__ void tma_load_2d(const void* desc, uint64_t* bar, void* smem, int32_t c0, int32_t c1) {
    asm volatile(
        "cp.async.bulk.tensor.2d.shared::cluster.global.mbarrier::complete_tx::bytes"
        " [%0], [%1, {%3, %4}], [%2];"
        :
        : "r"(smem_u32(smem)), "l"(reinterpret_cast<uint64_t>(desc)), "r"(smem_u32(bar)), "r"(c0), "r"(c1)
// ... 108 lines not shown
        "{\n"
        ".reg .pred p;\n"
        "setp.ne.b32 p, %34, 0;\n"
        "wgmma.mma_async.sync.aligned.m64n64k16.f32.bf16.bf16 "
        "{"
        "%0, %1, %2, %3, %4, %5, %6, %7, %8, %9, %10, %11, %12, %13, %14, %15, "
        "%16, %17, %18, %19, %20, %21, %22, %23, %24, %25, %26, %27, %28, %29, %30, %31"
        "}, %32, %33, p, 1, 1, %35, %36;\n"
        "}\n"
        : "+f"(d[0]), "+f"(d[1]), "+f"(d[2]), "+f"(d[3]), "+f"(d[4]), "+f"(d[5]), "+f"(d[6]), "+f"(d[7]),
          "+f"(d[8]), "+f"(d[9]), "+f"(d[10]), "+f"(d[11]), "+f"(d[12]), "+f"(d[13]), "+f"(d[14]), "+f"(d[15]),
          "+f"(d[16]), "+f"(d[17]), "+f"(d[18]), "+f"(d[19]), "+f"(d[20]), "+f"(d[21]), "+f"(d[22]), "+f"(d[23]),
          "+f"(d[24]), "+f"(d[25]), "+f"(d[26]), "+f"(d[27]), "+f"(d[28]), "+f"(d[29]), "+f"(d[30]), "+f"(d[31])
        : "l"(da), "l"(db), "r"(scale_d), "n"(TA), "n"(TB));
}

template <int TA, int TB>
__device__ __forceinline__ void wgmma_m64n128(float (&d)[64], uint64_t da, uint64_t db, uint32_t scale_d) {
    asm volatile(
        "{\n"
        ".reg .pred p;\n"
        "setp.ne.b32 p, %66, 0;\n"
        "wgmma.mma_async.sync.aligned.m64n128k16.f32.bf16.bf16 "
        "{"
        "%0, %1, %2, %3, %4, %5, %6, %7, %8, %9, %10, %11, %12, %13, %14, %15, "
        "%16, %17, %18, %19, %20, %21, %22, %23, %24, %25, %26, %27, %28, %29, %30, %31, "
        "%32, %33, %34, %35, %36, %37, %38, %39, %40, %41, %42, %43, %44, %45, %46, %47, "
        "%48, %49, %50, %51, %52, %53, %54, %55, %56, %57, %58, %59, %60, %61, %62, %63"
        "}, %64, %65, p, 1, 1, %67, %68;\n"
        "}\n"
        : "+f"(d[0]), "+f"(d[1]), "+f"(d[2]), "+f"(d[3]), "+f"(d[4]), "+f"(d[5]), "+f"(d[6]), "+f"(d[7]),
          "+f"(d[8]), "+f"(d[9]), "+f"(d[10]), "+f"(d[11]), "+f"(d[12]), "+f"(d[13]), "+f"(d[14]), "+f"(d[15]),
          "+f"(d[16]), "+f"(d[17]), "+f"(d[18]), "+f"(d[19]), "+f"(d[20]), "+f"(d[21]), "+f"(d[22]), "+f"(d[23]),
          "+f"(d[24]), "+f"(d[25]), "+f"(d[26]), "+f"(d[27]), "+f"(d[28]), "+f"(d[29]), "+f"(d[30]), "+f"(d[31]),
          "+f"(d[32]), "+f"(d[33]), "+f"(d[34]), "+f"(d[35]), "+f"(d[36]), "+f"(d[37]), "+f"(d[38]), "+f"(d[39]),
          "+f"(d[40]), "+f"(d[41]), "+f"(d[42]), "+f"(d[43]), "+f"(d[44]), "+f"(d[45]), "+f"(d[46]), "+f"(d[47]),
          "+f"(d[48]), "+f"(d[49]), "+f"(d[50]), "+f"(d[51]), "+f"(d[52]), "+f"(d[53]), "+f"(d[54]), "+f"(d[55]),
          "+f"(d[56]), "+f"(d[57]), "+f"(d[58]), "+f"(d[59]), "+f"(d[60]), "+f"(d[61]), "+f"(d[62]), "+f"(d[63])
        : "l"(da), "l"(db), "r"(scale_d), "n"(TA), "n"(TB));
}


template <int N>
__device__ __forceinline__ void fence_operands(float (&d)[N]) {
#pragma unroll
    for (int i = 0; i < N; ++i) asm volatile("" : "+f"(d[i])::"memory");
}

template <int N, int TA, int TB>
__device__ __forceinline__ void wgmma_bf16(float (&d)[N / 2], uint64_t da, uint64_t db, uint32_t scale_d) {
    if constexpr (N == 16) wgmma_m64n16<TA, TB>(d, da, db, scale_d);
    else if constexpr (N == 32) wgmma_m64n32<TA, TB>(d, da, db, scale_d);
    else if constexpr (N == 64) wgmma_m64n64<TA, TB>(d, da, db, scale_d);
    else {
        static_assert(N == 128, "wgmma_bf16: N must be 16, 32, 64 or 128");
        wgmma_m64n128<TA, TB>(d, da, db, scale_d);
    }
}

__device__ __forceinline__ uint32_t pack_bf16x2(float a, float b) {
    __nv_bfloat162 h = __floats2bfloat162_rn(a, b);
    return *reinterpret_cast<uint32_t*>(&h);
}
__device__ __forceinline__ __nv_bfloat162 u32_as_bf16x2(uint32_t u) { return *reinterpret_cast<__nv_bfloat162*>(&u); }
__device__ __forceinline__ uint32_t bf16x2_as_u32(__nv_bfloat162 h) { return *reinterpret_cast<uint32_t*>(&h); }
__device__ __forceinline__ uint32_t ld_shared_u32(uint32_t addr) {
    uint32_t v;
    asm volatile("ld.shared.b32 %0, [%1];" : "=r"(v) : "r"(addr) : "memory");
    return v;
}
__device__ __forceinline__ void st_shared_u32(uint32_t addr, uint32_t v) {
    asm volatile("st.shared.b32 [%0], %1;" ::"r"(addr), "r"(v) : "memory");
}
__device__ __forceinline__ float2 unpack_bf16x2(uint32_t u) {
    __nv_bfloat162 h = *reinterpret_cast<__nv_bfloat162*>(&u);
    return __bfloat1622float2(h);
}

__device__ __forceinline__ float to_f32(float v) { return v; }
__device__ __forceinline__ float to_f32(__nv_bfloat16 v) { return __bfloat162float(v); }
__device__ __forceinline__ void from_f32(float& d, float v) { d = v; }
__device__ __forceinline__ void from_f32(__nv_bfloat16& d, float v) { d = __float2bfloat16(v); }

}
```

vqgan-training_b200/native.py:

```python
from __future__ import annotations

import ctypes as C
import os

import torch

_HERE = os.path.dirname(os.path.abspath(__file__))
_LIB_PATH = os.path.join(_HERE, "libvqb200.so")

VQB_MAX_VIEWS = 16
VQB_MAX_TAPS = 16
VQB_MAX_VIEWS_3D = 8
VQB_MAX_TAPS_3D = 27
VQB_MAX_TAPS_3D_DGRAD = 64
EPI_BIAS, EPI_RES, EPI_RELU, EPI_MASK, EPI_STATS = 1, 2, 4, 8, 16


class VqbView(C.Structure):
    _fields_ = [("offset", C.c_int64), ("Wv", C.c_int32), ("Hv", C.c_int32), ("Nv", C.c_int32), ("_pad", C.c_int32),
                ("sw", C.c_int64), ("sh", C.c_int64), ("sn", C.c_int64)]


class VqbTap(C.Structure):
    _fields_ = [("view", C.c_int32), ("dw", C.c_int32), ("dh", C.c_int32), ("_pad", C.c_int32)]


class VqbConvDesc(C.Structure):
    _fields_ = [("C", C.c_int32), ("Cout", C.c_int32), ("N", C.c_int32), ("H", C.c_int32), ("W", C.c_int32),
                ("nviews", C.c_int32), ("ntaps", C.c_int32), ("flags", C.c_int32), ("out_f32", C.c_int32),
                ("_pad", C.c_int32), ("on", C.c_int64), ("oh", C.c_int64), ("ow", C.c_int64), ("oc", C.c_int64),
                ("views", VqbView * VQB_MAX_VIEWS), ("taps", VqbTap * VQB_MAX_TAPS)]


class VqbWgradDesc(C.Structure):
    _fields_ = [("C", C.c_int32), ("Cout", C.c_int32), ("N", C.c_int32), ("H", C.c_int32), ("W", C.c_int32),
                ("nviews", C.c_int32), ("ntaps", C.c_int32), ("ksplit", C.c_int32), ("ld_override", C.c_int64),
                ("col_offset", C.c_int64), ("dy_view", VqbView),
                ("views", VqbView * VQB_MAX_VIEWS), ("taps", VqbTap * VQB_MAX_TAPS)]


class VqbPackJob(C.Structure):
    _fields_ = [("w", C.c_void_p), ("out", C.c_void_p), ("tapmap", C.c_void_p), ("Cout", C.c_int32), ("Cin", C.c_int32),
                ("T", C.c_int32), ("nslots", C.c_int32), ("transpose", C.c_int32), ("Kpad", C.c_int32),
                ("fold", C.c_int32), ("sg", C.c_int32), ("ld_g", C.c_int32), ("ld_r", C.c_int32),
                ("first_block", C.c_int32), ("w_bf16", C.c_int32)]


class VqbView3d(C.Structure):
    _fields_ = [("offset", C.c_int64), ("Wv", C.c_int32), ("Hv", C.c_int32), ("Tv", C.c_int32), ("Nv", C.c_int32),
                ("sw", C.c_int64), ("sh", C.c_int64), ("st", C.c_int64), ("sn", C.c_int64)]


class VqbTap3d(C.Structure):
    _fields_ = [("view", C.c_int32), ("dw", C.c_int32), ("dh", C.c_int32), ("dt", C.c_int32)]


class VqbConv3dDesc(C.Structure):
    _fields_ = [("C", C.c_int32), ("Cout", C.c_int32), ("N", C.c_int32), ("T", C.c_int32), ("H", C.c_int32),
                ("W", C.c_int32), ("nviews", C.c_int32), ("ntaps", C.c_int32), ("flags", C.c_int32),
                ("out_f32", C.c_int32), ("on", C.c_int64), ("ot", C.c_int64), ("oh", C.c_int64), ("ow", C.c_int64),
                ("oc", C.c_int64), ("views", VqbView3d * VQB_MAX_VIEWS_3D), ("taps", VqbTap3d * VQB_MAX_TAPS_3D)]


class VqbConv3dDgradDesc(C.Structure):
    _fields_ = [("C", C.c_int32), ("Cout", C.c_int32), ("N", C.c_int32), ("T", C.c_int32), ("H", C.c_int32),
                ("W", C.c_int32), ("nviews", C.c_int32), ("ntaps", C.c_int32), ("flags", C.c_int32),
                ("out_f32", C.c_int32), ("on", C.c_int64), ("ot", C.c_int64), ("oh", C.c_int64), ("ow", C.c_int64),
                ("oc", C.c_int64), ("views", VqbView3d * VQB_MAX_VIEWS_3D),
                ("taps", VqbTap3d * VQB_MAX_TAPS_3D_DGRAD)]


class VqbWgrad3dDesc(C.Structure):
    _fields_ = [("C", C.c_int32), ("Cout", C.c_int32), ("N", C.c_int32), ("T", C.c_int32), ("H", C.c_int32),
                ("W", C.c_int32), ("nviews", C.c_int32), ("ntaps", C.c_int32), ("ksplit", C.c_int32),
                ("_pad", C.c_int32), ("ld_override", C.c_int64), ("col_offset", C.c_int64), ("dy_view", VqbView3d),
                ("views", VqbView3d * VQB_MAX_VIEWS_3D), ("taps", VqbTap3d * VQB_MAX_TAPS_3D)]


class VqbAdamwGroup(C.Structure):
    _fields_ = [("lr", C.c_float), ("beta1", C.c_float), ("beta2", C.c_float), ("eps", C.c_float),
                ("weight_decay", C.c_float), ("step", C.c_int32)]


_lib = None


def lib_path() -> str:
    return _LIB_PATH


def load():
    global _lib
    if _lib is not None:
        return _lib
    if not os.path.exists(_LIB_PATH):
        raise RuntimeError(
            f"{_LIB_PATH} is missing: run `python vqgan-training_b200/build_native.py` (nvcc, sm_90a). "
            "There is no CPU / PyTorch fallback for the hot path.")
    L = C.CDLL(_LIB_PATH)
    vp, i32, i64, f32 = C.c_void_p, C.c_int, C.c_int64, C.c_float
    sigs = {
        "vqb_last_error": (C.c_char_p, []),
        "vqb_version": (i32, []),
        "vqb_device_ok": (i32, []),
        "vqb_kernel_launch_count": (i32, []),
        "vqb_wgrad_cols": (i32, [i32, i32]),
        "vqb_conv_gemm": (i32, [C.POINTER(VqbConvDesc), vp, vp, vp, vp, vp, vp, vp, vp]),
        "vqb_wgrad_gemm": (i32, [C.POINTER(VqbWgradDesc), vp, vp, vp, vp]),
        "vqb_pack_weights": (i32, [vp, vp, i32, i32, i32, i32, vp, i32, i32, vp]),
        "vqb_nchw_to_nhwc": (i32, [vp, vp, i32, i32, i32, i32, i32, vp, vp, vp]),
        "vqb_nhwc_to_nchw": (i32, [vp, vp, i32, i32, i32, i32, i32, vp, vp]),
        "vqb_gn_silu_fwd": (i32, [vp, vp, vp, vp, vp, vp, i32, i32, i32, i32, f32, i32, vp]),
        "vqb_gn_silu_bwd": (i32, [vp, vp, vp, vp, vp, vp, vp, vp, vp, vp, i32, i32, i32, i32, i32, vp, vp]),
        "vqb_wavelet_fwd": (i32, [vp, vp, vp, i32, i32, i32, i32, i32, vp]),
        "vqb_colsum": (i32, [vp, vp, i64, i32, vp]),
        "vqb_wgrad_reduce": (i32, [vp, vp, i32, i32, i32, i32, i32, i32, i32, vp, i32, vp]),
        "vqb_maxpool2_fwd": (i32, [vp, vp, i32, i32, i32, i32, vp]),
        "vqb_maxpool2_bwd": (i32, [vp, vp, vp, vp, i32, i32, i32, i32, i32, vp]),
        "vqb_lpips_tail_fwd": (i32, [vp, vp, vp, vp, i32, i32, i32, vp]),
        "vqb_lpips_tail_bwd": (i32, [vp, vp, vp, vp, vp, i32, i32, i32, vp]),
        "vqb_lpips_tail_fwd_dropout": (i32, [vp, vp, vp, vp, i32, i32, i32, C.c_uint64, vp]),
        "vqb_lpips_tail_bwd_dropout": (i32, [vp, vp, vp, vp, vp, i32, i32, i32, C.c_uint64, vp]),
        "vqb_lpips_dropout_mask": (i32, [C.c_uint64, i32, i32, i32, vp, vp]),
        "vqb_attn_fwd": (i32, [vp, vp, vp, i32, i32, i32, vp]),
        "vqb_attn_bwd": (i32, [vp, vp, vp, vp, vp, vp, i32, i32, i32, vp]),
        "vqb_vq_argmin": (i32, [vp, vp, vp, vp, vp, i32, i32, i32, vp]),
        "vqb_nchw_to_nhwc_pad": (i32, [vp, vp, i32, i32, i32, i32, i32, i32, vp, vp, vp]),
        "vqb_nhwc_to_nchw_pad": (i32, [vp, vp, i32, i32, i32, i32, i32, i32, vp, vp]),
        "vqb_gn_silu_fwd_pre": (i32, [vp, vp, vp, vp, vp, vp, i32, i32, i32, i32, f32, i32, vp]),
        "vqb_conv_stats_ok": (i32, [C.POINTER(VqbConvDesc)]),
        "vqb_pack_weights_fold": (i32, [vp, vp, i32, i32, i32, i32, vp, i32, i32, vp]),
        "vqb_wgrad_reduce_fold": (i32, [vp, vp, i32, i32, i32, i32, i32, i32, i32, vp, vp]),
        "vqb_adamw_flat": (i32, [vp, vp, vp, vp, vp, i64, i32, C.POINTER(VqbAdamwGroup), f32, vp]),
        "vqb_pack_weights_multi": (i32, [vp, i32, i32, vp]),
        "vqb_adamw_fill_record": (i32, [i32, C.POINTER(VqbAdamwGroup), vp]),
        "vqb_adamw_flat_dev": (i32, [vp, vp, vp, vp, vp, i64, vp, f32, vp]),
        "vqb_pack_weights_bf16": (i32, [vp, vp, i32, i32, i32, i32, vp, i32, i32, vp]),
        "vqb_pack_weights_fold_bf16": (i32, [vp, vp, i32, i32, i32, i32, vp, i32, i32, vp]),
        "vqb_nchw_to_nhwc_bf16": (i32, [vp, vp, i32, i32, i32, i32, i32, vp, vp, vp]),
        "vqb_nchw_to_nhwc_pad_bf16": (i32, [vp, vp, i32, i32, i32, i32, i32, i32, vp, vp, vp]),
        "vqb_nhwc_to_nchw_bf16": (i32, [vp, vp, i32, i32, i32, i32, i32, vp]),
        "vqb_wavelet_fwd_bf16": (i32, [vp, vp, vp, i32, i32, i32, i32, i32, vp]),
        "vqb_conv3d_gemm": (i32, [C.POINTER(VqbConv3dDesc), vp, vp, vp, vp, vp, vp]),
        "vqb_attn_fwd_hd": (i32, [vp, vp, vp, i32, i32, i32, i32, vp]),
        "vqb_gauss_reparam": (i32, [vp, vp, vp, i32, i32, i64, i32, vp]),
        "vqb_conv3d_dgrad_gemm": (i32, [C.POINTER(VqbConv3dDgradDesc), vp, vp, vp, vp]),
        "vqb_wgrad3d_gemm": (i32, [C.POINTER(VqbWgrad3dDesc), vp, vp, vp, vp]),
        "vqb_attn_bwd_hd": (i32, [vp, vp, vp, vp, vp, vp, i32, i32, i32, i32, vp]),
        "vqb_gauss_reparam_bwd": (i32, [vp, vp, vp, vp, i32, i32, i64, vp]),
        "vqb_gn_silu_apply": (i32, [vp, vp, vp, vp, vp, i32, i32, i32, i32, i32, vp]),
        "vqb_ncthw_frames_to_nhwc_pad": (i32, [vp, vp] + [i32] * 7 + [vp, i32, vp, vp, vp]),
        "vqb_ncthw_frames_to_nhwc_pad_bf16": (i32, [vp, vp] + [i32] * 7 + [vp, i32, vp, vp, vp]),
        "vqb_ncthw_frames_to_nhwc": (i32, [vp, vp] + [i32] * 6 + [vp, i32, vp, vp, vp]),
        "vqb_ncthw_frames_to_nhwc_bf16": (i32, [vp, vp] + [i32] * 6 + [vp, i32, vp, vp, vp]),
        "vqb_nhwc_pad_frames_to_ncthw": (i32, [vp, vp] + [i32] * 7 + [vp, i32, vp, vp]),
        "vqb_nhwc_frames_to_ncthw": (i32, [vp, vp] + [i32] * 6 + [vp, i32, vp, vp]),
    }
    for name, (res, args) in sigs.items():
        fn = getattr(L, name, None)
        if fn is None:
            continue
        fn.restype = res
        fn.argtypes = args
    _lib = L
    return L


def check(rc: int, what: str = ""):
    if rc != 0:
        msg = load().vqb_last_error().decode(errors="replace")
        raise RuntimeError(f"libvqb200 {what} failed (code {rc}): {msg}")


def stream_ptr() -> int:
    return torch.cuda.current_stream().cuda_stream


def ptr(t) -> int:
    return 0 if t is None else t.data_ptr()


def launch_count() -> int:
    return load().vqb_kernel_launch_count()


def dense_view3d(N: int, T: int, H: int, W: int, Cs: int) -> VqbView3d:
    return VqbView3d(offset=0, Wv=W, Hv=H, Tv=T, Nv=N, sw=Cs, sh=W * Cs, st=H * W * Cs, sn=T * H * W * Cs)


def dense_view(N: int, H: int, W: int, Cs: int) -> VqbView:
    return VqbView(offset=0, Wv=W, Hv=H, Nv=N, _pad=0, sw=Cs, sh=W * Cs, sn=H * W * Cs)
```

vqgan-training_b200/ops.py:

```python
from __future__ import annotations

import math
import os
import threading
import weakref
from typing import Optional

import torch

import native
import plans
from native import EPI_BIAS, EPI_MASK, EPI_RELU, EPI_RES, check, ptr, stream_ptr

_tapmap_cache = {}


def _L():
    return native.load()


def require_cuda(t: torch.Tensor):
    if not t.is_cuda:
        raise RuntimeError("vqgan-training_b200: the hot path runs on sm_90a CUDA tensors only (no CPU fallback)")


def tapmap_tensor(tapmap, device) -> torch.Tensor:
    key = (tuple(tapmap), str(device))
    t = _tapmap_cache.get(key)
    if t is None:
        t = torch.tensor(list(tapmap), dtype=torch.int32, device=device)
        _tapmap_cache[key] = t
    return t


MASTER_DTYPES = (torch.float32, torch.bfloat16)


def check_master_dtype(t: torch.Tensor, what="parameter"):
    if t.dtype not in MASTER_DTYPES:
        raise RuntimeError(f"vqgan-training_b200: {what} has dtype {t.dtype}; supported parameter dtypes are "
                           "torch.float32 (training and inference) and torch.bfloat16 (inference only)")


def inference_only(*params):
    for p in params:
        if p is not None and p.dtype != torch.float32:
            raise RuntimeError(
                f"vqgan-training_b200: bf16 modules are inference-only: backward through a module with {p.dtype} "
                "parameters is not supported. Run it under torch.no_grad() / torch.inference_mode(), or train the "
                "float32 module (`.float()`).")


def pack_weights(weight: torch.Tensor, tapmap, transpose: bool, Kpad: int, fold: bool = False) -> torch.Tensor:
    Cout, Cin, KH, KW = weight.shape
    R = Cin if transpose else Cout
    out = torch.empty(R, len(tapmap), Kpad, device=weight.device, dtype=torch.bfloat16)
    tm = tapmap_tensor(tapmap, weight.device)
    w = weight.detach()
    if w.dtype == torch.bfloat16:
        w = w.contiguous()
        fn = _L().vqb_pack_weights_fold_bf16 if fold else _L().vqb_pack_weights_bf16
    else:
        if w.dtype != torch.float32 or not w.is_contiguous():
            w = w.float().contiguous()
        fn = _L().vqb_pack_weights_fold if fold else _L().vqb_pack_weights
    check(fn(ptr(w), ptr(out), Cout, Cin, KH * KW, len(tapmap), ptr(tm), 1 if transpose else 0, Kpad, stream_ptr()),
          "pack_weights")
    return out


class _PackEntry:

    __slots__ = ("wref", "out", "tm", "spec", "ver", "dtype", "__weakref__")

    def __init__(self, weight, out, tm, spec):
        self.wref = weakref.ref(weight)
        self.out, self.tm, self.spec = out, tm, spec
        self.ver = (weight._version, weight.data_ptr())
        self.dtype = weight.dtype

    def job(self, first_block):
        w = self.wref()
        Cout, Cin, T, nslots, transpose, Kpad, fold, sg, ld_g, ld_r = self.spec
        return native.VqbPackJob(w=w.data_ptr(), out=self.out.data_ptr(), tapmap=self.tm.data_ptr(), Cout=Cout, Cin=Cin,
# ... 137 lines not shown
            self._store[key] = ent
            with torch.no_grad():
                _run_pack([ent])
        elif ent.ver[0] != weight._version:
            with torch.no_grad():
                _run_pack([ent])
        return ent.out


_grad_slots = {}


def register_grad_slot(param, store, index):
    _grad_slots[param.data_ptr()] = (weakref.ref(store), index)


def grad_out(param: torch.Tensor) -> torch.Tensor:
    ent = _grad_slots.get(param.data_ptr())
    if ent is not None:
        store = ent[0]()
        if store is None:
            _grad_slots.pop(param.data_ptr(), None)
        else:
            q = store.plist[ent[1]]
            if q.data_ptr() == param.data_ptr() and q.shape == param.shape:
                s = store.take_slot(ent[1])
                if s is not None:
                    return s
    return torch.empty(param.shape, device=param.device, dtype=torch.float32)


H100_SMS = 132


def _num_sms() -> int:
    if torch.cuda.is_available():
        return torch.cuda.get_device_properties(torch.cuda.current_device()).multi_processor_count
    return H100_SMS


def _wgrad_block_n(cols: int) -> int:
    return 128 if cols % 128 == 0 else 64


def _wgrad_tile_blocks(cols: int) -> int:
    return 2 if cols % 256 == 0 else 1


def choose_ksplit(g: plans.ConvGeom, Cout_pad: int) -> int:
    cols = len(g.taps) * ((g.C + 63) // 64) * 64
    rows = 128
    kpix = 64
    tiles = ((Cout_pad + rows - 1) // rows) * (cols // (_wgrad_block_n(cols) * _wgrad_tile_blocks(cols)))

    def p2(v, cap):
        p = 1
        while p < v:
            p <<= 1
        return min(p, cap)

    bw = p2(g.Wo, kpix)
    bh = p2(g.Ho, kpix // bw)
    if isinstance(g, plans.ConvGeom3d):
        bt = p2(g.To, kpix // (bw * bh))
        bn = kpix // (bw * bh * bt)
        boxes = -(-g.Wo // bw) * -(-g.Ho // bh) * -(-g.To // bt) * -(-g.N // bn)
    else:
        bn = kpix // (bw * bh)
        boxes = -(-g.Wo // bw) * -(-g.Ho // bh) * -(-g.N // bn)
    sms = _num_sms()
    max_ks = max(1, min(boxes // 4, 128, (256 << 20) // max(1, Cout_pad * cols * 4)))
    best, best_score = 1, -1.0
    for ks in range(1, max_ks + 1):
        units = tiles * ks
        waves = -(-units // sms)
        eff = units / (waves * sms)
        score = eff - 0.06 * (waves - 1) - 0.0005 * ks
        if score > best_score:
            best, best_score = ks, score
    return best


def run_conv_gemm(g: plans.ConvGeom, a: torch.Tensor, wp: torch.Tensor, Cout: int, out: torch.Tensor, out_strides,
                  out_ptr_offset_bytes=0, bias=None, res=None, mask=None, relu=False, out_f32=False, stats=None):
    flags = (EPI_BIAS if bias is not None else 0) | (EPI_RES if res is not None else 0) | \
            (EPI_MASK if mask is not None else 0) | (EPI_RELU if relu else 0) | \
            (native.EPI_STATS if stats is not None else 0)
    dk = (Cout, tuple(out_strides), flags, out_f32)
    descs = g.__dict__.setdefault("_descs", {})
    d = descs.get(dk)
    if d is None:
        d = plans.conv_desc(g, Cout, out_strides, flags, out_f32)
        descs[dk] = d
    off = out_ptr_offset_bytes
    check(_L().vqb_conv_gemm(d, ptr(a), ptr(wp), ptr(bias), (ptr(res) + off) if res is not None else 0,
                             (ptr(mask) + off) if mask is not None else 0, ptr(out) + off, ptr(stats), stream_ptr()),
          "conv_gemm")


def conv_stats_supported(g: plans.ConvGeom, Cout: int, out_strides) -> bool:
    descs = g.__dict__.setdefault("_descs", {})
    key = ("stats_ok", Cout, tuple(out_strides))
    ok = descs.get(key)
    if ok is None:
        ok = bool(_L().vqb_conv_stats_ok(plans.conv_desc(g, Cout, out_strides, 0, False)))
        descs[key] = ok
    return ok


def run_wgrad(g: plans.ConvGeom, x: torch.Tensor, dy: torch.Tensor, weight_shape, Cout_pad: int,
              dy_view=None, out=None) -> torch.Tensor:
    Cout, Cin, KH, KW = weight_shape
    wk = ("wgrad", Cout_pad, dy_view is not None)
    descs = g.__dict__.setdefault("_descs", {})
    ent = descs.get(wk)
    if ent is None:
        ksplit = choose_ksplit(g, Cout_pad)
        ent = (ksplit, plans.wgrad_desc(g, Cout_pad, ksplit, dy_view=dy_view), _L().vqb_wgrad_cols(len(g.taps), g.C))
        descs[wk] = ent
    ksplit, d, cols = ent
    partial = torch.empty(ksplit, Cout_pad, cols, device=x.device, dtype=torch.float32)
    check(_L().vqb_wgrad_gemm(d, ptr(dy), ptr(x), ptr(partial), stream_ptr()), "wgrad_gemm")
    grad = out if out is not None else torch.empty(Cout, Cin, KH, KW, device=x.device, dtype=torch.float32)
    assert grad.shape == (Cout, Cin, KH, KW) and grad.is_contiguous()
    tm = tapmap_tensor(g.tapmap if len(g.tapmap) == len(g.taps) else list(range(len(g.taps))), x.device)
    check(_L().vqb_wgrad_reduce(ptr(partial), ptr(grad), ksplit, Cout, Cout_pad, Cin, KH * KW, len(g.taps),
                                cols // len(g.taps), ptr(tm), 0, stream_ptr()), "wgrad_reduce")
    return grad


class _Slot(threading.local):

    def __init__(self):
        self.v = None

    def __getitem__(self, i):
        return self.v

    def __setitem__(self, i, val):
        self.v = val


_dx_colsum_slot = _Slot()


def _take_dx_colsum(dy: torch.Tensor, C: int):
    ent = _dx_colsum_slot[0]
    if ent is None:
        return None
    t, ver, cs = ent
    if (t.data_ptr() == dy.data_ptr() and t.shape == dy.shape and t.stride() == dy.stride() and t.dtype == dy.dtype
            and dy._version == ver and cs.numel() == C):
        _dx_colsum_slot[0] = None
        return cs
    return None


def colsum(x2d_rows: int, x: torch.Tensor, C: int, out=None) -> torch.Tensor:
    if out is None:
        out = torch.empty(C, device=x.device, dtype=torch.float32)
    check(_L().vqb_colsum(ptr(x), ptr(out), x2d_rows, C, stream_ptr()), "colsum")
    return out


class ToNHWC(torch.autograd.Function):

    @staticmethod
    def forward(ctx, x, shift, inv_scale, frame):
        require_cuda(x)
        x = x.detach()
        bf16 = x.dtype == torch.bfloat16
        if bf16:
            x = x.contiguous()
        elif x.dtype != torch.float32 or not x.is_contiguous():
            x = x.float().contiguous()
        N, C, H, W = x.shape
        Cp = plans.cpad(C)
        if frame:
            y = alloc_framed(N, H, W, Cp, x.device)
            fn = _L().vqb_nchw_to_nhwc_pad_bf16 if bf16 else _L().vqb_nchw_to_nhwc_pad
            check(fn(ptr(x), ptr(y), N, C, H, W, Cp, 1, ptr(shift), ptr(inv_scale), stream_ptr()), "nchw_to_nhwc_pad")
        else:
            y = torch.empty(N, H, W, Cp, device=x.device, dtype=torch.bfloat16)
            fn = _L().vqb_nchw_to_nhwc_bf16 if bf16 else _L().vqb_nchw_to_nhwc
            check(fn(ptr(x), ptr(y), N, C, H, W, Cp, ptr(shift), ptr(inv_scale), stream_ptr()), "nchw_to_nhwc")
        ctx.shape = (N, C, H, W, Cp)
        ctx.inv_scale, ctx.frame = inv_scale, frame
        return y

    @staticmethod
    def backward(ctx, gy):
        N, C, H, W, Cp = ctx.shape
        gy = gy.contiguous()
        gx = torch.empty(N, C, H, W, device=gy.device, dtype=torch.float32)
        if ctx.frame:
            check(_L().vqb_nhwc_to_nchw_pad(ptr(gy), ptr(gx), N, C, H, W, Cp, 1, ptr(ctx.inv_scale), stream_ptr()),
                  "nhwc_to_nchw_pad")
        else:
            check(_L().vqb_nhwc_to_nchw(ptr(gy), ptr(gx), N, C, H, W, Cp, ptr(ctx.inv_scale), stream_ptr()),
                  "nhwc_to_nchw")
        return gx, None, None, None


def alloc_framed(N, H, W, C, device) -> torch.Tensor:
    n = N * (H + 2) * (W + 2) * C
    return torch.zeros(n + 64, device=device, dtype=torch.bfloat16)[:n].view(N, H + 2, W + 2, C)


def _fat_weights(cache: "PackedCache", weight, key, tapmap, transpose, Kpad):
    return cache.get(weight, tuple(key) + ("k64",), tapmap, transpose, Kpad, fat=True)


_fat_state = {"ok": None}


def fat_conv_enabled() -> bool:
    if _fat_state["ok"] is None:
        _fat_state["ok"] = False
        try:
            with torch.inference_mode(False):
                g = torch.Generator(device="cuda").manual_seed(1)
                x = torch.rand(2, 3, 16, 24, device="cuda", generator=g) - 0.5
                w = torch.rand(64, 3, 3, 3, device="cuda", generator=g) - 0.5
                c1, c2 = PackedCache(), PackedCache()
                a = conv(ToNHWC.apply(x, None, None, False), w, None, c1, "s1")
                b = conv(ToNHWC.apply(x, None, None, True), w, None, c2, "fat3")
                torch.cuda.synchronize()
                _fat_state["ok"] = bool(torch.allclose(a.float(), b.float(), rtol=2e-2, atol=2e-2))
        except Exception:
            _fat_state["ok"] = False
    return _fat_state["ok"]


def wavelet_to_nhwc(x: torch.Tensor, filt: torch.Tensor) -> torch.Tensor:
    require_cuda(x)
    if x.requires_grad:
        raise RuntimeError("wavelet front-end: the input image must not require grad (input-side op without backward)")
    bf16 = x.dtype == torch.bfloat16
    x = x.detach().contiguous() if bf16 else x.detach().float().contiguous()
    N, C, H, W = x.shape
# ... 26 lines not shown
    return f.to(torch.int32).reshape(-1), f.shape[1]


class ClipToFrames(torch.autograd.Function):

    @staticmethod
    def forward(ctx, x, shift, inv_scale, frame, sel, Tsel):
        require_cuda(x)
        x = x.detach()
        bf16 = x.dtype == torch.bfloat16
        if bf16:
            x = x.contiguous()
        elif x.dtype != torch.float32 or not x.is_contiguous():
            x = x.float().contiguous()
        B, C, T, H, W = x.shape
        Cp = plans.cpad(C)
        sel_dev = None if sel is None else sel.pin_memory().to(x.device, non_blocking=True)
        if frame:
            y = alloc_framed(B * Tsel, H, W, Cp, x.device)
            fn = _L().vqb_ncthw_frames_to_nhwc_pad_bf16 if bf16 else _L().vqb_ncthw_frames_to_nhwc_pad
            check(fn(ptr(x), ptr(y), B, C, T, H, W, Cp, 1, ptr(sel_dev), Tsel, ptr(shift), ptr(inv_scale),
                     stream_ptr()), "ncthw_frames_to_nhwc_pad")
        else:
            y = torch.empty(B * Tsel, H, W, Cp, device=x.device, dtype=torch.bfloat16)
            fn = _L().vqb_ncthw_frames_to_nhwc_bf16 if bf16 else _L().vqb_ncthw_frames_to_nhwc
            check(fn(ptr(x), ptr(y), B, C, T, H, W, Cp, ptr(sel_dev), Tsel, ptr(shift), ptr(inv_scale), stream_ptr()),
                  "ncthw_frames_to_nhwc")
        ctx.shape = (B, C, T, H, W, Cp, Tsel)
        ctx.inv_scale, ctx.frame, ctx.sel_dev = inv_scale, frame, sel_dev
        return y

    @staticmethod
    def backward(ctx, gy):
        B, C, T, H, W, Cp, Tsel = ctx.shape
        gy = gy.contiguous()
        gx = torch.empty(B, C, T, H, W, device=gy.device, dtype=torch.float32)
        if ctx.frame:
            check(_L().vqb_nhwc_pad_frames_to_ncthw(ptr(gy), ptr(gx), B, C, T, H, W, Cp, 1, ptr(ctx.sel_dev), Tsel,
                                                    ptr(ctx.inv_scale), stream_ptr()), "nhwc_pad_frames_to_ncthw")
        else:
            check(_L().vqb_nhwc_frames_to_ncthw(ptr(gy), ptr(gx), B, C, T, H, W, Cp, ptr(ctx.sel_dev), Tsel,
                                                ptr(ctx.inv_scale), stream_ptr()), "nhwc_frames_to_ncthw")
        return gx, None, None, None, None, None


def clip_to_frames(x, shift=None, inv_scale=None, frame=False, frames=None):
    if x.dim() != 5:
        raise ValueError(f"clip_to_frames: expected a [B, C, T, H, W] clip, got shape {tuple(x.shape)}")
    sel, Tsel = clip_frame_selection(frames, x.shape[0], x.shape[2])
    return ClipToFrames.apply(x, shift, inv_scale, frame, sel, Tsel)


class ToNCHW(torch.autograd.Function):

    @staticmethod
    def forward(ctx, y, C, dtype=torch.float32):
        N, H, W, Cp = y.shape
        y = y.contiguous()
        if dtype == torch.bfloat16:
            x = torch.empty(N, C, H, W, device=y.device, dtype=torch.bfloat16)
            check(_L().vqb_nhwc_to_nchw_bf16(ptr(y), ptr(x), N, C, H, W, Cp, stream_ptr()), "nhwc_to_nchw_bf16")
        else:
            x = torch.empty(N, C, H, W, device=y.device, dtype=torch.float32)
            check(_L().vqb_nhwc_to_nchw(ptr(y), ptr(x), N, C, H, W, Cp, 0, stream_ptr()), "nhwc_to_nchw")
        ctx.shape = (N, C, H, W, Cp)
        return x

    @staticmethod
    def backward(ctx, gx):
        N, C, H, W, Cp = ctx.shape
        gx = gx.float().contiguous()
        gy = torch.empty(N, H, W, Cp, device=gx.device, dtype=torch.bfloat16)
        check(_L().vqb_nchw_to_nhwc(ptr(gx), ptr(gy), N, C, H, W, Cp, 0, 0, stream_ptr()), "nchw_to_nhwc")
        return gy, None, None


def to_nchw(y, C, dtype=torch.float32):
    return ToNCHW.apply(y, C, dtype)


class ConvFn(torch.autograd.Function):

    @staticmethod
    def forward(ctx, x, weight, bias, residual, cache, kind, relu, input_is_relu, nchw_out, want_stats=False):
        require_cuda(x)
        N, H, W, Cp = x.shape
        Cout, Cin, KH, KW = weight.shape
        assert Cp == plans.cpad(Cin), f"conv input has {Cp} channels, weight expects {Cin}"
        x = x.contiguous()
        if kind == "fat3":
            assert Cp == 8 and KH == 3
        g, H, W = _conv_geom(cache, kind, N, H, W, Cp, KH)
        if kind == "fat3":
            wp = _fat_weights(cache, weight, ("fwd", kind), g.tapmap, False, Cp)
        else:
            wp = cache.get(weight, ("fwd", kind), g.tapmap, False, Cp)
        Cop = plans.cpad(Cout)
        b = None
        if bias is not None:
            b = bias.detach()
            if b.dtype != torch.float32:
                b = b.float()
        if nchw_out:
            f32 = weight.dtype == torch.float32
            out = torch.empty(N, Cout, g.Ho, g.Wo, device=x.device, dtype=torch.float32 if f32 else torch.bfloat16)
            run_conv_gemm(g, x, wp, Cout, out, plans.nchw_strides(Cout, g.Ho, g.Wo), bias=b, relu=relu, out_f32=f32)
        else:
            alloc = torch.empty if Cop == Cout else torch.zeros
            out = alloc(N, g.Ho, g.Wo, Cop, device=x.device, dtype=torch.bfloat16)
            res = residual.contiguous() if residual is not None else None
            ostr = plans.nhwc_strides(g.Ho, g.Wo, Cop)
            stats = None
            if want_stats and Cop == Cout and conv_stats_supported(g, Cout, ostr):
                stats = torch.zeros(N, Cout, 2, device=x.device, dtype=torch.float32)
            run_conv_gemm(g, x, wp, Cout, out, ostr, bias=b, res=res, relu=relu, stats=stats)
        ctx.save_for_backward(x, weight)
        ctx.cache, ctx.kind = cache, kind
        ctx.has_bias, ctx.has_res = bias is not None, residual is not None
        ctx.input_is_relu, ctx.nchw_out = input_is_relu, nchw_out
        if want_stats and not nchw_out:
            if stats is None:
                stats = torch.empty(0, device=x.device)
            ctx.mark_non_differentiable(stats)
            return out, stats
        return out

    @staticmethod
    def backward(ctx, gout, _gstats=None):
        x, weight = ctx.saved_tensors
        inference_only(weight)
        gx, gw, gb, gres = conv_backward(x, weight, gout, ctx.cache, ctx.kind, ctx.has_bias, ctx.has_res,
                                         ctx.input_is_relu, ctx.nchw_out, ctx.needs_input_grad[:4])
        return gx, gw, gb, gres, None, None, None, None, None, None


def _conv_geom(cache, kind, N, H, W, Cp, KH):
    if kind == "fat3":
        H, W = H - 2, W - 2
        return cache.geom(("fat", N, H, W), lambda: plans.geom_fat3(N, H, W)), H, W
    if kind == "s1":
        return cache.geom(("f", N, H, W), lambda: plans.geom_s1(N, H, W, Cp, KH)), H, W
    if kind == "s2":
        return cache.geom(("f", N, H, W), lambda: plans.geom_s2(N, H, W, Cp)), H, W
    if kind == "patch":
        return cache.geom(("f", N, H, W), lambda: plans.geom_patch(N, H, W, Cp, KH)), H, W
    raise ValueError(kind)


def conv_backward(x, weight, gout, cache, kind, has_bias, has_res, input_is_relu, nchw_out, needs):
    N, H, W, Cp = x.shape
    Cout, Cin, KH, KW = weight.shape
    g, H, W = _conv_geom(cache, kind, N, H, W, Cp, KH)
    Cop = plans.cpad(Cout)
    dy_framed = False
    if nchw_out:
        gn = gout.float().contiguous()
        if Cop == 8 and KH == 3 and kind == "s1" and fat_conv_enabled():
            dy_framed = True
            dy = alloc_framed(N, g.Ho, g.Wo, Cop, x.device)
            check(_L().vqb_nchw_to_nhwc_pad(ptr(gn), ptr(dy), N, Cout, g.Ho, g.Wo, Cop, 1, 0, 0, stream_ptr()),
                  "nchw_to_nhwc_pad")
        else:
            dy = torch.empty(N, g.Ho, g.Wo, Cop, device=x.device, dtype=torch.bfloat16)
            check(_L().vqb_nchw_to_nhwc(ptr(gn), ptr(dy), N, Cout, g.Ho, g.Wo, Cop, 0, 0, stream_ptr()),
                  "nchw_to_nhwc")
    else:
        dy = gout.contiguous()
    gx = gw = gb = gres = None
    if needs[0]:
        mask = x if input_is_relu else None
        gx_alloc = torch.empty if Cp == Cin else torch.zeros
        if kind == "fat3":
            gx = torch.zeros(N, H + 2, W + 2, Cp, device=x.device, dtype=torch.bfloat16)
            gd = cache.geom(("d", N, H, W), lambda: plans.geom_s1_dgrad(N, H, W, Cop, KH))
            wpd = cache.get(weight, ("dgrad", "s1"), gd.tapmap, True, Cop)
            run_conv_gemm(gd, dy, wpd, Cin, gx, ((H + 2) * (W + 2) * Cp, (W + 2) * Cp, Cp, 1),
                          out_ptr_offset_bytes=((W + 2) + 1) * Cp * 2)
        elif dy_framed:
            gx = gx_alloc(N, H, W, Cp, device=x.device, dtype=torch.bfloat16)
            gdf = cache.geom(("dfat", N, H, W), lambda: plans.geom_fat3(N, H, W, dgrad=True))
            wpd = _fat_weights(cache, weight, ("dgrad", "fat3"), gdf.tapmap, True, Cop)
            run_conv_gemm(gdf, dy, wpd, Cin, gx, plans.nhwc_strides(H, W, Cp), mask=mask)
        else:
            gx = gx_alloc(N, H, W, Cp, device=x.device, dtype=torch.bfloat16)
        if kind == "fat3" or dy_framed:
            pass
        elif kind == "s1":
            gd = cache.geom(("d", N, H, W), lambda: plans.geom_s1_dgrad(N, H, W, Cop, KH))
            wpd = cache.get(weight, ("dgrad", kind), gd.tapmap, True, Cop)
            run_conv_gemm(gd, dy, wpd, Cin, gx, plans.nhwc_strides(H, W, Cp), mask=mask)
        elif kind == "s2":
            for ph, pw, gd in cache.geom(("d", N, H, W), lambda: plans.geom_s2_dgrad_classes(N, H, W, Cop)):
                wpd = cache.get(weight, ("dgrad", kind, ph, pw), gd.tapmap, True, Cop)
                run_conv_gemm(gd, dy, wpd, Cin, gx, (H * W * Cp, 2 * W * Cp, 2 * Cp, 1),
                              out_ptr_offset_bytes=(ph * W + pw) * Cp * 2, mask=mask)
        elif kind == "patch":
            k = KH
            for kh in range(k):
                for kw in range(k):
                    gd = cache.geom(("d", N, H, W, kh, kw), lambda: plans.ConvGeom(
                        N, g.Ho, g.Wo, Cop, [native.dense_view(N, g.Ho, g.Wo, Cop)], [(0, 0, 0)], [kh * k + kw]))
                    wpd = cache.get(weight, ("dgrad", kind, kh, kw), gd.tapmap, True, Cop)
                    run_conv_gemm(gd, dy, wpd, Cin, gx, (H * W * Cp, k * W * Cp, k * Cp, 1),
                                  out_ptr_offset_bytes=(kh * W + kw) * Cp * 2, mask=mask)
    if needs[1]:
        if kind == "fat3":
            g3 = run_wgrad(g, x, dy, (Cout, plans.FAT_K, 3, 1), Cop)
            gw = g3[:, :24, :, 0].reshape(Cout, 3, 8, 3)[:, :, :Cin, :].permute(0, 2, 3, 1).contiguous()
        elif dy_framed:
            gw = run_wgrad(g, x, dy, weight.shape, Cop,
                           dy_view=plans.framed_interior_view(N, g.Ho, g.Wo, Cop), out=grad_out(weight))
        else:
            gw = run_wgrad(g, x, dy, weight.shape, Cop, out=grad_out(weight))
    if has_bias and needs[2]:
        rows = N * (g.Ho + 2) * (g.Wo + 2) if dy_framed else N * g.Ho * g.Wo
        gb = None if dy_framed else _take_dx_colsum(dy, Cop)
        if gb is None:
            gb = colsum(rows, dy, Cop)[:Cout]
    if has_res and needs[3]:
        gres = dy
    return gx, gw, gb, gres


def conv(x, weight, bias, cache, kind="s1", residual=None, relu=False, input_is_relu=False, nchw_out=False,
         want_stats=False):
    if want_stats and not nchw_out:
        out, st = ConvFn.apply(x, weight, bias, residual, cache, kind, relu, input_is_relu, nchw_out, True)
        return out, (st if st.numel() > 0 else None)
    return ConvFn.apply(x, weight, bias, residual, cache, kind, relu, input_is_relu, nchw_out, False)


class UpConvFn(torch.autograd.Function):

    @staticmethod
    def forward(ctx, x, weight, bias, cache, want_stats=False):
        require_cuda(x)
        x = x.contiguous()
        N, h, w, Cp = x.shape
        Cout, Cin, KH, KW = weight.shape
        assert KH == 3 and KW == 3 and Cp == plans.cpad(Cin)
        Cop = plans.cpad(Cout)
        alloc = torch.empty if Cop == Cout else torch.zeros
        out = alloc(N, 2 * h, 2 * w, Cop, device=x.device, dtype=torch.bfloat16)
        b = bias.detach().float() if bias is not None else None
        strides = (4 * h * w * Cop, 2 * 2 * w * Cop, 2 * Cop, 1)
        stats = None
        g00 = cache.geom(("uf", N, h, w, 0, 0), lambda: plans.geom_up_fwd(N, h, w, Cp, 0, 0))
        if want_stats and Cop == Cout and conv_stats_supported(g00, Cout, strides):
            stats = torch.zeros(N, Cout, 2, device=x.device, dtype=torch.float32)
        for ph in range(2):
            for pw in range(2):
                g = cache.geom(("uf", N, h, w, ph, pw), lambda: plans.geom_up_fwd(N, h, w, Cp, ph, pw))
                wp = cache.get(weight, ("ufwd", ph, pw), g.tapmask, False, Cp, fold=True)
                run_conv_gemm(g, x, wp, Cout, out, strides, out_ptr_offset_bytes=(ph * 2 * w + pw) * Cop * 2, bias=b,
                              stats=stats)
        ctx.save_for_backward(x, weight)
        ctx.cache, ctx.has_bias = cache, bias is not None
        if want_stats:
            if stats is None:
                stats = torch.empty(0, device=x.device)
            ctx.mark_non_differentiable(stats)
            return out, stats
        return out

    @staticmethod
    def backward(ctx, gout, _gstats=None):
        x, weight = ctx.saved_tensors
        inference_only(weight)
        cache = ctx.cache
        N, h, w, Cp = x.shape
        Cout, Cin, KH, KW = weight.shape
        Cop = plans.cpad(Cout)
        dy = gout.contiguous()
        gx = gw = gb = None
        if ctx.needs_input_grad[0]:
            gd = cache.geom(("ud", N, h, w), lambda: plans.geom_up_dgrad(N, h, w, Cop))
            wpd = cache.get(weight, ("udgrad",), gd.tapmask, True, Cop, fold=True)
            gx_alloc = torch.empty if Cp == Cin else torch.zeros
            gx = gx_alloc(N, h, w, Cp, device=x.device, dtype=torch.bfloat16)
            run_conv_gemm(gd, dy, wpd, Cin, gx, plans.nhwc_strides(h, w, Cp))
        if ctx.needs_input_grad[1]:
            C64 = ((Cp + 63) // 64) * 64
            g00 = cache.geom(("uf", N, h, w, 0, 0), lambda: plans.geom_up_fwd(N, h, w, Cp, 0, 0))
            ksplit = choose_ksplit(g00, Cop)
            partial = torch.empty(ksplit, Cop, 16 * C64, device=x.device, dtype=torch.float32)
            masks = []
            for ph in range(2):
                for pw in range(2):
                    g = cache.geom(("uf", N, h, w, ph, pw), lambda: plans.geom_up_fwd(N, h, w, Cp, ph, pw))
                    dk = ("uwgrad", Cop, ksplit)
                    descs = g.__dict__.setdefault("_descs", {})
                    d = descs.get(dk)
                    if d is None:
                        d = plans.wgrad_desc(g, Cop, ksplit, dy_view=plans.up_dy_view(N, h, w, Cop, ph, pw),
                                             ld_override=16 * C64, col_offset=(ph * 2 + pw) * 4 * C64)
                        descs[dk] = d
                    check(_L().vqb_wgrad_gemm(d, ptr(dy), ptr(x), ptr(partial), stream_ptr()), "wgrad_gemm(up)")
                    masks += g.tapmask
            gw = grad_out(weight)
            tm = tapmap_tensor(masks, x.device)
            check(_L().vqb_wgrad_reduce_fold(ptr(partial), ptr(gw), ksplit, Cout, Cop, Cin, 9, 16, C64, ptr(tm),
                                             stream_ptr()), "wgrad_reduce_fold")
        if ctx.has_bias and ctx.needs_input_grad[2]:
            gb = _take_dx_colsum(dy, Cop)
            if gb is None:
                gb = colsum(N * 4 * h * w, dy, Cop)[:Cout]
        return gx, gw, gb, None, None


def upsample_conv(x, weight, bias, cache, want_stats=False):
    if want_stats:
        out, st = UpConvFn.apply(x, weight, bias, cache, True)
        return out, (st if st.numel() > 0 else None)
    return UpConvFn.apply(x, weight, bias, cache, False)


class GroupNormSiLUFn(torch.autograd.Function):

    @staticmethod
    def forward(ctx, x, gamma, beta, groups, eps, silu, with_skip, chsums=None):
        require_cuda(x)
        x = x.contiguous()
        if chsums is not None:
            y, mr = gn_silu_fwd_pre(x, gamma, beta, chsums, groups, eps, silu)
        else:
            y, mr = gn_silu_fwd(x, gamma, beta, groups, eps, silu)
        ctx.save_for_backward(x, gamma, beta, mr)
        ctx.groups, ctx.silu, ctx.with_skip = groups, silu, with_skip
        ctx.set_materialize_grads(False)
        if with_skip:
            return y, x.view_as(x)
        return y

    @staticmethod
    def backward(ctx, gy, gskip=None):
        x, gamma, beta, mr = ctx.saved_tensors
        inference_only(gamma, beta)
        if gy is None:
            return (gskip, None, None, None, None, None, None, None)
        dx, dg, db = gn_silu_bwd(x, gy, gskip, gamma, beta, mr, ctx.groups, ctx.silu)
        return dx, dg, db, None, None, None, None, None


def gn_silu_fwd(x, gamma, beta, groups, eps, silu):
    N, H, W, C = x.shape
    y = torch.empty_like(x)
    mr = torch.empty(N, groups, 2, device=x.device, dtype=torch.float32)
    ga, be = gamma.detach().float(), beta.detach().float()
    ws = torch.empty(N * C * 2, device=x.device, dtype=torch.float64)
    check(_L().vqb_gn_silu_fwd(ptr(x), ptr(y), ptr(ga), ptr(be), ptr(mr), ptr(ws), N, H * W, C, groups, eps,
                               1 if silu else 0, stream_ptr()), "gn_silu_fwd")
    return y, mr


def gn_silu_fwd_pre(x, gamma, beta, chsums, groups, eps, silu):
    N, H, W, C = x.shape
    y = torch.empty_like(x)
    mr = torch.empty(N, groups, 2, device=x.device, dtype=torch.float32)
    ga, be = gamma.detach().float(), beta.detach().float()
    check(_L().vqb_gn_silu_fwd_pre(ptr(x), ptr(y), ptr(ga), ptr(be), ptr(mr), ptr(chsums), N, H * W, C, groups, eps,
                                   1 if silu else 0, stream_ptr()), "gn_silu_fwd_pre")
    return y, mr


def gn_silu_apply(x, gamma, beta, mr, silu):
    N, H, W, C = x.shape
    y = torch.empty_like(x)
    ga, be = gamma.detach().float(), beta.detach().float()
    check(_L().vqb_gn_silu_apply(ptr(x), ptr(y), ptr(ga), ptr(be), ptr(mr), N, H * W, C, mr.shape[1],
                                 1 if silu else 0, stream_ptr()), "gn_silu_apply")
    return y


def gn_silu_bwd(x, gy, gskip, gamma, beta, mr, groups, silu):
    N, H, W, C = x.shape
    gy = gy.contiguous()
    add = gskip.contiguous() if gskip is not None else None
    dx = torch.empty_like(x)
    dg, db = grad_out(gamma), grad_out(beta)
    ws = torch.empty(N * C * 2 + N * groups * 2, device=x.device, dtype=torch.float32)
    ga, be = gamma.detach().float(), beta.detach().float()
    cs = torch.empty(C, device=x.device, dtype=torch.float32)
    check(_L().vqb_gn_silu_bwd(ptr(x), ptr(gy), ptr(add), ptr(dx), ptr(ga), ptr(be), ptr(mr), ptr(dg), ptr(db),
                               ptr(ws), N, H * W, C, groups, 1 if silu else 0, ptr(cs), stream_ptr()), "gn_silu_bwd")
    _dx_colsum_slot[0] = (dx, dx._version, cs)
    return dx, dg, db


def group_norm_silu(x, gamma, beta, groups=32, eps=1e-6, silu=True, with_skip=False, chsums=None):
    return GroupNormSiLUFn.apply(x, gamma, beta, groups, eps, silu, with_skip, chsums)


class ResnetBlockRecomputeFn(torch.autograd.Function):

    @staticmethod
    def forward(ctx, x, chsums, spec, n1w, n1b, c1w, c1b, n2w, n2b, c2w, c2b, sw, sb):
        require_cuda(x)
        g1, e1, g2, e2, k1, k2, ks = spec
        x = x.contiguous()
        if chsums is not None:
            hn, mr1 = gn_silu_fwd_pre(x, n1w, n1b, chsums, g1, e1, True)
        else:
            hn, mr1 = gn_silu_fwd(x, n1w, n1b, g1, e1, True)
        h, st = conv(hn, c1w, c1b, k1, "s1", want_stats=True)
        del hn
        if st is not None:
            h2, mr2 = gn_silu_fwd_pre(h, n2w, n2b, st, g2, e2, True)
        else:
            h2, mr2 = gn_silu_fwd(h, n2w, n2b, g2, e2, True)
        del h
        skip = conv(x, sw, sb, ks, "s1") if sw is not None else x
        out, stats = conv(h2, c2w, c2b, k2, "s1", residual=skip, want_stats=True)
        ctx.save_for_backward(x, mr1, mr2, n1w, n1b, c1w, c1b, n2w, n2b, c2w, c2b, sw, sb)
        ctx.spec = spec
        if stats is None:
            stats = torch.empty(0, device=x.device)
        ctx.mark_non_differentiable(stats)
        return out, stats

    @staticmethod
    def backward(ctx, gout, _gstats=None):
        x, mr1, mr2, n1w, n1b, c1w, c1b, n2w, n2b, c2w, c2b, sw, sb = ctx.saved_tensors
        inference_only(n1w, n1b, c1w, c1b, n2w, n2b, c2w, c2b, sw, sb)
        g1, _, g2, _, k1, k2, ks = ctx.spec
        nig = ctx.needs_input_grad
        hn = gn_silu_apply(x, n1w, n1b, mr1, True)
        h = conv(hn, c1w, c1b, k1, "s1")
        h2 = gn_silu_apply(h, n2w, n2b, mr2, True)
        need_hn = nig[0] or nig[3] or nig[4]
        need_h = need_hn or nig[5] or nig[6]
        need_h2 = need_h or nig[7] or nig[8]
        need_res = need_hn or (sw is not None and (nig[11] or nig[12]))
        gx = gn1w = gn1b = gc1w = gc1b = gn2w = gn2b = gsw = gsb = None
        gh2, gc2w, gc2b, gskip = conv_backward(h2, c2w, gout, k2, "s1", c2b is not None, True, False, False,
                                               (need_h2, nig[9], nig[10], need_res))
        del h2
        if sw is not None and need_res:
            gskip, gsw, gsb, _ = conv_backward(x, sw, gskip, ks, "s1", sb is not None, False, False, False,
                                               (need_hn, nig[11], nig[12], False))
        if need_h2:
            gh, gn2w, gn2b = gn_silu_bwd(h, gh2, None, n2w, n2b, mr2, g2, True)
            del h, gh2
            if need_h:
                ghn, gc1w, gc1b, _ = conv_backward(hn, c1w, gh, k1, "s1", c1b is not None, False, False, False,
                                                   (need_hn, nig[5], nig[6], False))
                del hn, gh
                if need_hn:
                    gx, gn1w, gn1b = gn_silu_bwd(x, ghn, gskip, n1w, n1b, mr1, g1, True)
        grads = (gn1w, gn1b, gc1w, gc1b, gn2w, gn2b, gc2w, gc2b, gsw, gsb)
        return (gx, None, None) + tuple(g if nig[i + 3] else None for i, g in enumerate(grads))


def resnet_block_recompute(x, chsums, spec, *params):
    out, st = ResnetBlockRecomputeFn.apply(x, chsums, spec, *params)
    return out, (st if st.numel() > 0 else None)


class MaxPool2Fn(torch.autograd.Function):

    @staticmethod
    def forward(ctx, x):
        x = x.contiguous()
        N, H, W, C = x.shape
        y = torch.empty(N, H // 2, W // 2, C, device=x.device, dtype=x.dtype)
        check(_L().vqb_maxpool2_fwd(ptr(x), ptr(y), N, H // 2, W // 2, C, stream_ptr()), "maxpool2_fwd")
        ctx.save_for_backward(x)
        return y

    @staticmethod
    def backward(ctx, gy):
        (x,) = ctx.saved_tensors
        gy = gy.contiguous()
        N, H, W, C = x.shape
        gx = torch.empty_like(x)
        check(_L().vqb_maxpool2_bwd(ptr(x), ptr(gy), 0, ptr(gx), N, H // 2, W // 2, C, 1, stream_ptr()),
              "maxpool2_bwd")
        return gx


def maxpool2(x):
    return MaxPool2Fn.apply(x)


class LpipsTailFn(torch.autograd.Function):

    @staticmethod
    def forward(ctx, f0, f1, w, seed):
        f0, f1 = f0.contiguous(), f1.contiguous()
        N, H, W, C = f0.shape
        out = torch.zeros(N, device=f0.device, dtype=torch.float32)
        wv = w.detach().reshape(-1).float().contiguous()
        if seed is None:
            check(_L().vqb_lpips_tail_fwd(ptr(f0), ptr(f1), ptr(wv), ptr(out), N, H * W, C, stream_ptr()),
                  "lpips_tail_fwd")
        else:
            check(_L().vqb_lpips_tail_fwd_dropout(ptr(f0), ptr(f1), ptr(wv), ptr(out), N, H * W, C, seed, stream_ptr()),
                  "lpips_tail_fwd_dropout")
        ctx.save_for_backward(f0, f1, wv)
        ctx.seed = seed
        return out

    @staticmethod
    def backward(ctx, g):
        f0, f1, wv = ctx.saved_tensors
        N, H, W, C = f0.shape
        g = g.float().contiguous()
        df0 = torch.empty_like(f0)
        if ctx.seed is None:
            check(_L().vqb_lpips_tail_bwd(ptr(f0), ptr(f1), ptr(wv), ptr(g), ptr(df0), N, H * W, C, stream_ptr()),
                  "lpips_tail_bwd")
        else:
            check(_L().vqb_lpips_tail_bwd_dropout(ptr(f0), ptr(f1), ptr(wv), ptr(g), ptr(df0), N, H * W, C, ctx.seed,
                                                  stream_ptr()), "lpips_tail_bwd_dropout")
        return df0, None, None, None


def lpips_tail(f0, f1, w, dropout_seed=None):
    return LpipsTailFn.apply(f0, f1, w, dropout_seed)


def lpips_dropout_mask(seed: int, N: int, HW: int, C: int, device) -> torch.Tensor:
    m = torch.empty(N, HW, C, device=device, dtype=torch.uint8)
    check(_L().vqb_lpips_dropout_mask(seed, N, HW, C, ptr(m), stream_ptr()), "lpips_dropout_mask")
    return m


def vq_argmin(z_flat: torch.Tensor, codebook: torch.Tensor):
    require_cuda(z_flat)
# ... 397 lines not shown
```

Baseline: 165.1.

## Fuse GroupNorm-SiLU backward channel reductions into dgrad conv GEMM epilogue

Adds a GroupNorm-backward epilogue variant to the conv GEMM. When a stride-1 dgrad output feeds a GroupNorm+SiLU backward, the epilogue TMA-loads the pre-norm input x and computes per-channel sums of the SiLU-adjusted gradient and its product with (x-mean). It accumulates them atomically into a sums buffer. The GN backward kernel then consumes those sums and skips its own reduction pass over x and dy. This costs an extra x tile load in the epilogue, more shared memory (possibly fewer ring stages), and extra plumbing that threads mean/rstd through Act and autograd.

```diff
diff --git a/include/vqb200.h b/include/vqb200.h
--- a/include/vqb200.h
+++ b/include/vqb200.h
@@ -63,6 +63,19 @@
 } VqbWgradDesc;
 
 int vqb_conv_stats_ok(const VqbConvDesc* d);
+
+typedef struct VqbGnBwdFuse {
+    const void* x;
+    const float* mr;
+    const float* gamma;
+    const float* beta;
+    float* sums;
+    int32_t groups;
+    int32_t silu;
+} VqbGnBwdFuse;
+int vqb_conv_gemm_gnbwd(const VqbConvDesc* d, const void* a, const void* w_packed, void* out, const VqbGnBwdFuse* f,
+                        void* stream);
+int vqb_conv_gnbwd_ok(const VqbConvDesc* d);
 
 int vqb_wgrad_gemm(const VqbWgradDesc* d, const void* dy, const void* x, float* partial, void* stream);
 
@@ -97,6 +110,9 @@
 int vqb_gn_silu_bwd(const void* x, const void* dy, const void* add, void* dx, const float* gamma, const float* beta,
                     const float* mr, float* dgamma, float* dbeta, float* ws, int N, int HW, int C, int G, int silu,
                     float* dx_colsum, void* stream);
+int vqb_gn_silu_bwd_sums(const void* x, const void* dy, const void* add, void* dx, const float* gamma,
+                         const float* beta, const float* mr, const float* sums, float* dgamma, float* dbeta, float* ws,
+                         int N, int HW, int C, int G, int silu, float* dx_colsum, void* stream);
 
 int vqb_wavelet_fwd(const float* x, void* y, const float* filt, int N, int C, int H, int W, int Cpad, void* stream);
 
diff --git a/vqgan-training_b200/ae.py b/vqgan-training_b200/ae.py
--- a/vqgan-training_b200/ae.py
+++ b/vqgan-training_b200/ae.py
@@ -19,13 +19,14 @@
 
 class Act:
 
-    __slots__ = ("t", "C", "stats", "framed")
-
-    def __init__(self, t: Tensor, C: int, stats=None, framed=False):
+    __slots__ = ("t", "C", "stats", "framed", "gn")
+
+    def __init__(self, t: Tensor, C: int, stats=None, framed=False, gn=None):
         self.t = t
         self.C = C
         self.stats = stats
         self.framed = framed
+        self.gn = gn
 
     @property
     def shape(self):
@@ -83,7 +84,7 @@
         want_stats = want_stats and not nchw_out
         kind = "fat3" if a.framed else self._kind()
         out = ops.conv(a.t, self.weight, self.bias, self._packed, kind,
-                       residual.t if residual is not None else None, relu, input_is_relu, nchw_out, want_stats)
+                       residual.t if residual is not None else None, relu, input_is_relu, nchw_out, want_stats, a.gn)
         if nchw_out:
             return out
         if want_stats:
@@ -104,15 +105,19 @@
     def __init__(self, *args, **kwargs):
         super().__init__(*args, **kwargs)
 
+    def _link(self, a: "Act", mr, silu: bool):
+        return (a.t, mr, self.weight, self.bias, self.num_groups, silu) if torch.is_grad_enabled() else None
+
     def forward(self, input, silu: bool = False):
         a, ext = _enter(input, self)
-        y = ops.group_norm_silu(a.t, self.weight, self.bias, self.num_groups, self.eps, silu, chsums=a.stats)
-        return _exit(Act(y, a.C), ext, self)
+        y, mr = ops.group_norm_silu(a.t, self.weight, self.bias, self.num_groups, self.eps, silu, chsums=a.stats,
+                                    with_mr=True)
+        return _exit(Act(y, a.C, gn=self._link(a, mr, silu)), ext, self)
 
     def forward_with_skip(self, a: "Act", silu: bool = True):
-        y, skip = ops.group_norm_silu(a.t, self.weight, self.bias, self.num_groups, self.eps, silu, with_skip=True,
-                                      chsums=a.stats)
-        return Act(y, a.C), Act(skip, a.C)
+        y, skip, mr = ops.group_norm_silu(a.t, self.weight, self.bias, self.num_groups, self.eps, silu, with_skip=True,
+                                          chsums=a.stats, with_mr=True)
+        return Act(y, a.C, gn=self._link(a, mr, silu)), Act(skip, a.C)
 
 
 class AttnBlock(nn.Module):
diff --git a/vqgan-training_b200/csrc/common.cu b/vqgan-training_b200/csrc/common.cu
--- a/vqgan-training_b200/csrc/common.cu
+++ b/vqgan-training_b200/csrc/common.cu
@@ -113,7 +113,7 @@
 extern "C" {
 
 const char* vqb_last_error(void) { return vqb::g_err; }
-int vqb_version(void) { return 103; }
+int vqb_version(void) { return 104; }
 int vqb_device_ok(void) { return (vqb::device_is_sm90() && vqb::get_encode_fn() != nullptr) ? 1 : 0; }
 int vqb_kernel_launch_count(void) { return vqb::g_launches.load(std::memory_order_relaxed); }
 
diff --git a/vqgan-training_b200/csrc/conv_gemm.cu b/vqgan-training_b200/csrc/conv_gemm.cu
--- a/vqgan-training_b200/csrc/conv_gemm.cu
+++ b/vqgan-training_b200/csrc/conv_gemm.cu
@@ -39,6 +39,10 @@
     const void* mask;
     const float* bias;
     float* stats;
+    const float* gn_mr;
+    const float* gn_gamma;
+    const float* gn_beta;
+    int32_t gn_groups, gn_cpg, gn_silu, _pad1;
 };
 
 template <int kTaps>
@@ -69,10 +73,11 @@
 using Conv3dParams = Conv3dParamsT<VQB_MAX_TAPS_3D>;
 using Conv3dDgradParams = Conv3dParamsT<VQB_MAX_TAPS_3D_DGRAD>;
 
-template <int BN, class P, bool kStaged>
+template <int BN, class P, bool kStaged, bool kGnBwd = false>
 __global__ void __launch_bounds__(kThreads, 1) conv_gemm_kernel(const __grid_constant__ P p) {
     constexpr bool kR5 = P::kRank == 5;
     static_assert(!kStaged || (!kR5 && BN >= 64), "the staged epilogue stores whole 64-channel slabs of 2-D outputs");
+    static_assert(!kGnBwd || kStaged, "the GroupNorm-backward epilogue reads x from the staged tile");
     extern __shared__ uint8_t smem_raw[];
     constexpr uint32_t kBBytes = BN * kBlockK * 2;
     constexpr uint32_t kStageBytes = kABytes + kBBytes;
@@ -83,7 +88,8 @@
     constexpr uint32_t kRowOff[4] = {0, 8 * 128, 64 * 128, 72 * 128};
     uint8_t* epi = base + stages * kStageBytes;
     float* sStat = reinterpret_cast<float*>(epi + (kStaged ? 2 * kEpiBytes : 0));
-    uint64_t* full = reinterpret_cast<uint64_t*>(sStat + kConsumerWarps * BN * 2);
+    float4* sCoef = reinterpret_cast<float4*>(sStat + kConsumerWarps * BN * 2);
+    uint64_t* full = reinterpret_cast<uint64_t*>(sCoef + (kGnBwd ? 2 * BN : 0));
     uint64_t* empty = full + stages;
     uint64_t* order = empty + stages;
     uint64_t* epi_full = order + 2;
@@ -101,7 +107,7 @@
         tma_prefetch_desc(&p.bmap);
         if constexpr (kStaged) {
             tma_prefetch_desc(&p.omap);
-            if (p.flags & (VQB_EPI_RES | VQB_EPI_MASK)) tma_prefetch_desc(&p.emap);
+            if (kGnBwd || (p.flags & (VQB_EPI_RES | VQB_EPI_MASK))) tma_prefetch_desc(&p.emap);
         }
         for (uint32_t i = 0; i < stages; ++i) {
             mbar_init(&full[i], 1);
@@ -138,7 +144,7 @@
                 if constexpr (kStaged) {
                     const uint32_t c = l & 1;
                     mbar_wait(&epi_empty[c], ((l >> 1) & 1) ^ 1);
-                    if (p.flags & (VQB_EPI_RES | VQB_EPI_MASK)) {
+                    if (kGnBwd || (p.flags & (VQB_EPI_RES | VQB_EPI_MASK))) {
                         const int nslab = min(BN, p.Cout - ncol0) / kBlockK;
                         mbar_arrive_expect_tx(&epi_full[c], nslab * kSlabBytes);
                         for (int s = 0; s < nslab; ++s)
@@ -176,8 +182,9 @@
     const uint32_t cwarp = cw * 4 + warp;
     const uint32_t wtid = threadIdx.x & 127u;
     const uint32_t ring = smem_u32(base);
-    const bool has_bias = p.flags & VQB_EPI_BIAS, has_res = p.flags & VQB_EPI_RES;
-    const bool do_relu = !kR5 && (p.flags & VQB_EPI_RELU), has_mask = !kR5 && (p.flags & VQB_EPI_MASK);
+    const bool has_bias = !kGnBwd && (p.flags & VQB_EPI_BIAS), has_res = !kGnBwd && (p.flags & VQB_EPI_RES);
+    const bool do_relu = !kR5 && !kGnBwd && (p.flags & VQB_EPI_RELU);
+    const bool has_mask = !kR5 && !kGnBwd && (p.flags & VQB_EPI_MASK);
     const bool vec_path = p.vec_store != 0;
     const bool reduce = !kR5 && p.do_stats;
     const __nv_bfloat16* res = reinterpret_cast<const __nv_bfloat16*>(p.res);
@@ -241,8 +248,24 @@
             tn = m_tile / (p.tiles_w * p.tiles_h);
         }
         const int col0 = n_tile * BN;
+        const int n_img = tn << p.lbn;
         uint8_t* tbuf = epi + cw * kEpiBytes;
         const uint32_t trow = smem_u32(tbuf) + (warp * 16 + (lane >> 2)) * 128u + (lane & 3u) * 4u;
+        const float4* coef = sCoef + cw * BN;
+        if constexpr (kGnBwd) {
+            for (uint32_t i = wtid; i < BN; i += 128u) {
+                const int c = col0 + static_cast<int>(i);
+                float4 v = make_float4(0.f, 0.f, 0.f, 0.f);
+                if (c < p.Cout) {
+                    const float* m = p.gn_mr + (static_cast<int64_t>(n_img) * p.gn_groups + c / p.gn_cpg) * 2;
+                    const float mean = __ldg(m), rstd = __ldg(m + 1);
+                    const float a = __ldg(p.gn_gamma + c) * rstd;
+                    v = make_float4(mean, 0.5f * a, 0.5f * (__ldg(p.gn_beta + c) - mean * a), 0.5f * rstd);
+                }
+                sCoef[cw * BN + i] = v;
+            }
+            named_bar_sync(1 + cw, 128);
+        }
         if (kStaged) mbar_wait(&epi_full[cw], (l >> 1) & 1);
         int64_t pix[4] = {0, 0, 0, 0};
         bool valid[4] = {true, true, true, true};
@@ -283,9 +306,9 @@
                 for (int r = 0; r < 4; ++r) {
                     rv[r] = mv[r] = __floats2bfloat162_rn(0.f, 0.f);
                     if constexpr (kStaged) {
-                        if (has_res || has_mask) {
+                        if (kGnBwd || has_res || has_mask) {
                             const __nv_bfloat162 v = u32_as_bf16x2(ld_shared_u32(tj + kRowOff[r]));
-                            if (has_res) rv[r] = v;
+                            if (kGnBwd || has_res) rv[r] = v;
                             if (has_mask) mv[r] = v;
                         }
                         continue;
@@ -320,10 +343,21 @@
                         *reinterpret_cast<__nv_bfloat162*>(reinterpret_cast<__nv_bfloat16*>(p.out) + pix[r] + col) = ob;
                     if (reduce) {
                         const float2 v = __bfloat1622float2(ob);
-                        r1[0] += v.x;
-                        r2[0] = fmaf(v.x, v.x, r2[0]);
-                        r1[1] += v.y;
-                        r2[1] = fmaf(v.y, v.y, r2[1]);
+                        if constexpr (kGnBwd) {
+                            const float2 xf = __bfloat1622float2(rv[r]);
+                            const float4 k0 = coef[j * 8 + 2 * (lane & 3u)], k1 = coef[j * 8 + 2 * (lane & 3u) + 1];
+                            const float d0 = gn_bwd_du2(v.x, xf.x, k0.y, k0.z, p.gn_silu != 0);
+                            const float d1 = gn_bwd_du2(v.y, xf.y, k1.y, k1.z, p.gn_silu != 0);
+                            r1[0] += d0;
+                            r2[0] = fmaf(d0, xf.x - k0.x, r2[0]);
+                            r1[1] += d1;
+                            r2[1] = fmaf(d1, xf.y - k1.x, r2[1]);
+                        } else {
+                            r1[0] += v.x;
+                            r2[0] = fmaf(v.x, v.x, r2[0]);
+                            r1[1] += v.y;
+                            r2[1] = fmaf(v.y, v.y, r2[1]);
+                        }
                     }
                 }
             } else if constexpr (!kStaged) {
@@ -375,14 +409,27 @@
         }
         if (reduce) {
             named_bar_sync(1 + cw, 128);
-            const int n_img = tn << p.lbn;
             const float* sw = sStat + cw * 4 * BN * 2;
-            for (uint32_t idx = wtid; idx < BN * 2u; idx += 128u) {
-                const int c = col0 + static_cast<int>(idx >> 1);
-                float v = 0.f;
-#pragma unroll
-                for (int w4 = 0; w4 < 4; ++w4) v += sw[w4 * BN * 2 + idx];
-                if (c < p.Cout) atomicAdd(p.stats + (static_cast<int64_t>(n_img) * p.Cout + c) * 2 + (idx & 1u), v);
+            for (uint32_t q = wtid; q < BN / 2u; q += 128u) {
+                const int c = col0 + 2 * static_cast<int>(q);
+                float4 v = make_float4(0.f, 0.f, 0.f, 0.f);
+#pragma unroll
+                for (int w4 = 0; w4 < 4; ++w4) {
+                    const float4 t = *reinterpret_cast<const float4*>(sw + w4 * BN * 2 + 4 * q);
+                    v.x += t.x;
+                    v.y += t.y;
+                    v.z += t.z;
+                    v.w += t.w;
+                }
+                if (c < p.Cout) {
+                    if constexpr (kGnBwd) {
+                        v.x *= 0.5f;
+                        v.y *= coef[2 * q].w;
+                        v.z *= 0.5f;
+                        v.w *= coef[2 * q + 1].w;
+                    }
+                    red_add_v4(p.stats + (static_cast<int64_t>(n_img) * p.Cout + c) * 2, v);
+                }
             }
             named_bar_sync(1 + cw, 128);
         }
@@ -410,28 +457,29 @@
     return VQB_OK;
 }
 
-static size_t conv_smem_bytes(int block_n, int stages, bool staged) {
+static size_t conv_smem_bytes(int block_n, int stages, bool staged, bool gnbwd = false) {
     return 1024 + static_cast<size_t>(stages) * (kABytes + block_n * kBlockK * 2) +
-           (staged ? 2 * kBlockM * block_n * 2 : 0) + kConsumerWarps * block_n * 2 * sizeof(float) + 8 * (2 * stages + 6);
-}
-
-static int ring_stages(int block_n, bool staged) {
+           (staged ? 2 * kBlockM * block_n * 2 : 0) + kConsumerWarps * block_n * 2 * sizeof(float) +
+           (gnbwd ? 2 * block_n * 4 * sizeof(float) : 0) + 8 * (2 * stages + 6);
+}
+
+static int ring_stages(int block_n, bool staged, bool gnbwd = false) {
     int stages = kMaxStages;
-    while (conv_smem_bytes(block_n, stages, staged) > 227 * 1024) --stages;
+    while (conv_smem_bytes(block_n, stages, staged, gnbwd) > 227 * 1024) --stages;
     return stages;
 }
 
-template <int BN, bool kStaged = false, class P>
+template <int BN, bool kStaged = false, bool kGnBwd = false, class P>
 static int launch_conv(const P& p, void* stream) {
-    const size_t smem = conv_smem_bytes(BN, p.stages, kStaged);
+    const size_t smem = conv_smem_bytes(BN, p.stages, kStaged, kGnBwd);
     static bool attr_set = false;
     if (!attr_set) {
-        VQB_CUDA(cudaFuncSetAttribute(conv_gemm_kernel<BN, P, kStaged>, cudaFuncAttributeMaxDynamicSharedMemorySize,
-                                      227 * 1024));
+        VQB_CUDA(cudaFuncSetAttribute(conv_gemm_kernel<BN, P, kStaged, kGnBwd>,
+                                      cudaFuncAttributeMaxDynamicSharedMemorySize, 227 * 1024));
         attr_set = true;
     }
     const int grid = p.total_tiles < num_sms() ? p.total_tiles : num_sms();
-    conv_gemm_kernel<BN, P, kStaged><<<grid, kThreads, smem, static_cast<cudaStream_t>(stream)>>>(p);
+    conv_gemm_kernel<BN, P, kStaged, kGnBwd><<<grid, kThreads, smem, static_cast<cudaStream_t>(stream)>>>(p);
     VQB_CUDA(cudaGetLastError());
     return VQB_OK;
 }
@@ -441,11 +489,30 @@
 using namespace vqb;
 
 static int conv_gemm_impl(const VqbConvDesc* d, const void* a, const void* w_packed, const float* bias, const void* res,
-                          const void* mask, void* out, float* stats, void* stream, bool query_only);
+                          const void* mask, void* out, float* stats, void* stream, bool query_only,
+                          const VqbGnBwdFuse* gnb = nullptr);
 
 extern "C" int vqb_conv_gemm(const VqbConvDesc* d, const void* a, const void* w_packed, const float* bias,
                              const void* res, const void* mask, void* out, float* stats, void* stream) {
     return conv_gemm_impl(d, a, w_packed, bias, res, mask, out, stats, stream, false);
+}
+
+extern "C" int vqb_conv_gemm_gnbwd(const VqbConvDesc* d, const void* a, const void* w_packed, void* out,
+                                   const VqbGnBwdFuse* f, void* stream) {
+    VQB_CHECK(f != nullptr, "vqb_conv_gemm_gnbwd: null VqbGnBwdFuse");
+    return conv_gemm_impl(d, a, w_packed, nullptr, nullptr, nullptr, out, nullptr, stream, false, f);
+}
+
+extern "C" int vqb_conv_gnbwd_ok(const VqbConvDesc* d) {
+    if (!d) return 0;
+    alignas(16) static const uint64_t dummy_aligned[4] = {0, 0, 0, 0};
+    const void* dp = dummy_aligned;
+    const float* fp = static_cast<const float*>(dp);
+    const int32_t groups = d->Cout % 32 == 0 ? 32 : 1;
+    const VqbGnBwdFuse f = {dp, fp, fp, fp, const_cast<float*>(fp), groups, 1};
+    const int r = conv_gemm_impl(d, dp, dp, nullptr, nullptr, nullptr, const_cast<void*>(dp), nullptr, nullptr, true,
+                                 &f);
+    return r == 1 ? 1 : 0;
 }
 
 extern "C" int vqb_conv_stats_ok(const VqbConvDesc* d) {
@@ -460,8 +527,17 @@
 }
 
 static int conv_gemm_impl(const VqbConvDesc* d, const void* a, const void* w_packed, const float* bias, const void* res,
-                          const void* mask, void* out, float* stats, void* stream, bool query_only) {
+                          const void* mask, void* out, float* stats, void* stream, bool query_only,
+                          const VqbGnBwdFuse* gnb) {
     VQB_CHECK(d && a && w_packed && out, "vqb_conv_gemm: null pointer");
+    if (gnb) {
+        VQB_CHECK(d->flags == 0, "vqb_conv_gemm_gnbwd: flags 0x%x: the GroupNorm-backward epilogue takes no other",
+                  d->flags);
+        VQB_CHECK(gnb->x && gnb->mr && gnb->gamma && gnb->beta && gnb->sums, "vqb_conv_gemm_gnbwd: null pointer");
+        VQB_CHECK((reinterpret_cast<uintptr_t>(gnb->sums) & 15u) == 0, "vqb_conv_gemm_gnbwd: sums must be 16-byte aligned");
+        VQB_CHECK(gnb->groups > 0 && d->Cout % gnb->groups == 0 && (gnb->silu == 0 || gnb->silu == 1),
+                  "vqb_conv_gemm_gnbwd: groups=%d silu=%d unsupported for Cout=%d", gnb->groups, gnb->silu, d->Cout);
+    }
     VQB_CHECK(d->C > 0 && d->C % 8 == 0, "vqb_conv_gemm: C=%d must be a positive multiple of 8", d->C);
     VQB_CHECK(d->Cout > 0 && d->N > 0 && d->H > 0 && d->W > 0, "vqb_conv_gemm: bad extents");
     VQB_CHECK(d->ntaps >= 1 && d->ntaps <= VQB_MAX_TAPS && d->nviews >= 1 && d->nviews <= VQB_MAX_VIEWS,
@@ -472,7 +548,9 @@
                   "vqb_conv_gemm: VQB_EPI_BIAS needs a 16-byte aligned bias pointer");
     if ((d->flags & VQB_EPI_RES)) VQB_CHECK(res != nullptr, "vqb_conv_gemm: VQB_EPI_RES without res");
     if ((d->flags & VQB_EPI_MASK)) VQB_CHECK(mask != nullptr, "vqb_conv_gemm: VQB_EPI_MASK without mask");
-    if ((d->flags & VQB_EPI_STATS)) VQB_CHECK(stats != nullptr, "vqb_conv_gemm: VQB_EPI_STATS without stats");
+    if ((d->flags & VQB_EPI_STATS))
+        VQB_CHECK(stats != nullptr && (reinterpret_cast<uintptr_t>(stats) & 15u) == 0,
+                  "vqb_conv_gemm: VQB_EPI_STATS needs a 16-byte aligned stats pointer");
     const uintptr_t ops = reinterpret_cast<uintptr_t>(res) | reinterpret_cast<uintptr_t>(mask);
     const bool nhwc_bf16 = d->oc == 1 && !d->out_f32 && d->on % 8 == 0 && d->oh % 8 == 0 && d->ow % 8 == 0 &&
                            (reinterpret_cast<uintptr_t>(out) & 15u) == 0 && (ops & 3u) == 0;
@@ -504,15 +582,22 @@
             return set_error(VQB_EINVAL, "vqb_conv_gemm: VQB_EPI_STATS unsupported for this shape (N=%d H=%d W=%d Cout=%d)",
                              d->N, d->H, d->W, d->Cout);
     }
-    p.do_stats = (d->flags & VQB_EPI_STATS) ? 1 : 0;
-    if (query_only) return stats_ok ? 1 : 0;
+    p.do_stats = (gnb || (d->flags & VQB_EPI_STATS)) ? 1 : 0;
+    if (query_only && !gnb) return stats_ok ? 1 : 0;
     const bool has_res = d->flags & VQB_EPI_RES, has_mask = d->flags & VQB_EPI_MASK;
-    const void* eop = has_res ? res : mask;
-    const int moved = (has_res || has_mask) ? 2 : 1;
+    const void* eop = gnb ? gnb->x : has_res ? res : mask;
+    const int moved = (has_res || has_mask || gnb) ? 2 : 1;
     const bool staged = nhwc_bf16 && d->Cout % 64 == 0 && d->on > 0 && d->oh > 0 && d->ow > 0 &&
                         !(has_res && has_mask) && (reinterpret_cast<uintptr_t>(eop) & 15u) == 0 &&
                         d->ntaps * ((d->C + kBlockK - 1) / kBlockK) <= kStagedKChunksPerTensor * moved;
-    p.stages = ring_stages(block_n, staged);
+    if (gnb) {
+        if (query_only) return stats_ok && staged ? 1 : 0;
+        if (!(stats_ok && staged))
+            return set_error(VQB_EINVAL,
+                             "vqb_conv_gemm_gnbwd: unsupported for this shape (N=%d H=%d W=%d Cout=%d, %d K-chunks)",
+                             d->N, d->H, d->W, d->Cout, d->ntaps * ((d->C + kBlockK - 1) / kBlockK));
+    }
+    p.stages = ring_stages(block_n, staged, gnb != nullptr);
     p.ntaps = d->ntaps;
     p.kchunks = (d->C + kBlockK - 1) / kBlockK;
     p.C = d->C;
@@ -532,7 +617,14 @@
     p.res = res;
     p.mask = mask;
     p.bias = bias;
-    p.stats = stats;
+    p.stats = gnb ? gnb->sums : stats;
+    p.gn_mr = gnb ? gnb->mr : nullptr;
+    p.gn_gamma = gnb ? gnb->gamma : nullptr;
+    p.gn_beta = gnb ? gnb->beta : nullptr;
+    p.gn_groups = gnb ? gnb->groups : 0;
+    p.gn_cpg = gnb ? d->Cout / gnb->groups : 0;
+    p.gn_silu = gnb ? gnb->silu : 0;
+    p._pad1 = 0;
     for (int t = 0; t < d->ntaps; ++t) {
         p.tap_view[t] = d->taps[t].view;
         p.tap_dw[t] = d->taps[t].dw;
@@ -547,7 +639,7 @@
                            static_cast<uint64_t>(d->on) * 2};
         uint32_t box[4] = {kBlockK, bw, bh, bn};
         rc = encode_tmap_bf16(&p.omap, out, 4, dims, str, box, 128);
-        if (rc == VQB_OK && (has_res || has_mask)) rc = encode_tmap_bf16(&p.emap, eop, 4, dims, str, box, 128);
+        if (rc == VQB_OK && (has_res || has_mask || gnb)) rc = encode_tmap_bf16(&p.emap, eop, 4, dims, str, box, 128);
         if (rc != VQB_OK) return rc;
     }
     {
@@ -561,8 +653,14 @@
     switch (block_n) {
         case 16: rc = launch_conv<16>(p, stream); break;
         case 32: rc = launch_conv<32>(p, stream); break;
-        case 64: rc = staged ? launch_conv<64, true>(p, stream) : launch_conv<64>(p, stream); break;
-        default: rc = staged ? launch_conv<128, true>(p, stream) : launch_conv<128>(p, stream); break;
+        case 64:
+            rc = gnb ? launch_conv<64, true, true>(p, stream)
+                     : staged ? launch_conv<64, true>(p, stream) : launch_conv<64>(p, stream);
+            break;
+        default:
+            rc = gnb ? launch_conv<128, true, true>(p, stream)
+                     : staged ? launch_conv<128, true>(p, stream) : launch_conv<128>(p, stream);
+            break;
     }
     if (rc != VQB_OK) return rc;
     count_launch();
diff --git a/vqgan-training_b200/csrc/elementwise.cu b/vqgan-training_b200/csrc/elementwise.cu
--- a/vqgan-training_b200/csrc/elementwise.cu
+++ b/vqgan-training_b200/csrc/elementwise.cu
@@ -1,6 +1,3 @@
-#ifndef VQB_EXACT_SIGMOID
-#define VQB_EXACT_SIGMOID 0
-#endif
 #include "common.cuh"
 #include "ptx.cuh"
 
@@ -31,16 +28,6 @@
     float t;
     asm("tanh.approx.f32 %0, %1;" : "=f"(t) : "f"(0.5f * x));
     return fmaf(0.5f, t, 0.5f);
-#endif
-}
-
-__device__ __forceinline__ float tanh_fast(float x) {
-#if VQB_EXACT_SIGMOID
-    return 2.f / (1.f + __expf(-2.f * x)) - 1.f;
-#else
-    float t;
-    asm("tanh.approx.f32 %0, %1;" : "=f"(t) : "f"(x));
-    return t;
 #endif
 }
 
@@ -387,13 +374,7 @@
                 cvt8(ud[k], d);
 #pragma unroll
                 for (int j = 0; j < 8; ++j) {
-                    float du2 = 2.f * d[j];
-                    if (silu) {
-                        const float h = fmaf(f[j], a2[j], b2[j]);
-                        const float t = tanh_fast(h);
-                        const float r = fmaf(-h, t, h + 1.f);
-                        du2 = d[j] * fmaf(t, r, r);
-                    }
+                    const float du2 = gn_bwd_du2(d[j], f[j], a2[j], b2[j], silu);
                     s1[j] += du2;
                     s2[j] = fmaf(du2, f[j] - mean[j], s2[j]);
                 }
@@ -487,13 +468,7 @@
                 if (ADD) cvt8(ua[k], r);
 #pragma unroll
                 for (int j = 0; j < 8; ++j) {
-                    float du2 = 2.f * d[j];
-                    if (silu) {
-                        const float h = fmaf(f[j], a2[j], b2[j]);
-                        const float t = tanh_fast(h);
-                        const float rr = fmaf(-h, t, h + 1.f);
-                        du2 = d[j] * fmaf(t, rr, rr);
-                    }
+                    const float du2 = gn_bwd_du2(d[j], f[j], a2[j], b2[j], silu);
                     float v = fmaf(du2, a2[j], fmaf(f[j] - mean[j], k2[j], k0[j]));
                     if (ADD) v += r[j];
                     f[j] = v;
@@ -996,6 +971,32 @@
     return VQB_OK;
 }
 
+static int gn_bwd_finish(const void* x, const void* dy, const void* add, void* dx, const float* gamma, const float* beta,
+                         const float* mr, float* dgamma, float* dbeta, const float* cs, float* gsum, int N, int HW,
+                         int C, int G, int silu, float* dx_colsum, cudaStream_t st) {
+    int chunks, ppc;
+    const int T = cv_threads(C);
+    const int fin = (N * G > C ? N * G : C);
+    gn_bwd_finalize_kernel<<<(fin + 127) / 128, 128, 0, st>>>(cs, gamma, gsum, dgamma, dbeta, N, C, G, HW);
+    const size_t cs_smem = dx_colsum ? C * sizeof(float) : 0;
+    if (dx_colsum) VQB_CUDA(cudaMemsetAsync(dx_colsum, 0, sizeof(float) * C, st));
+    if (add) {
+        cv_grid(HW, C, N, gn_bwd_apply_kernel<true, 2>, cs_smem, chunks, ppc);
+        gn_bwd_apply_kernel<true, 2><<<dim3(chunks, N), T, cs_smem, st>>>(
+            static_cast<const __nv_bfloat16*>(x), static_cast<const __nv_bfloat16*>(dy),
+            static_cast<const __nv_bfloat16*>(add), static_cast<__nv_bfloat16*>(dx), mr, gsum, gamma, beta, HW, C, G,
+            ppc, silu, dx_colsum);
+    } else {
+        cv_grid(HW, C, N, gn_bwd_apply_kernel<false, 3>, cs_smem, chunks, ppc);
+        gn_bwd_apply_kernel<false, 3><<<dim3(chunks, N), T, cs_smem, st>>>(
+            static_cast<const __nv_bfloat16*>(x), static_cast<const __nv_bfloat16*>(dy), nullptr,
+            static_cast<__nv_bfloat16*>(dx), mr, gsum, gamma, beta, HW, C, G, ppc, silu, dx_colsum);
+    }
+    VQB_CUDA(cudaGetLastError());
+    count_launch(2);
+    return VQB_OK;
+}
+
 int vqb_gn_silu_bwd(const void* x, const void* dy, const void* add, void* dx, const float* gamma, const float* beta,
                     const float* mr, float* dgamma, float* dbeta, float* ws, int N, int HW, int C, int G, int silu,
                     float* dx_colsum, void* stream) {
@@ -1012,25 +1013,19 @@
         static_cast<const __nv_bfloat16*>(x), static_cast<const __nv_bfloat16*>(dy), mr, gamma, beta, cs, HW, C, G,
         ppc, silu);
     count_launch();
-    const int fin = (N * G > C ? N * G : C);
-    gn_bwd_finalize_kernel<<<(fin + 127) / 128, 128, 0, st>>>(cs, gamma, gsum, dgamma, dbeta, N, C, G, HW);
-    const size_t cs_smem = dx_colsum ? C * sizeof(float) : 0;
-    if (dx_colsum) VQB_CUDA(cudaMemsetAsync(dx_colsum, 0, sizeof(float) * C, st));
-    if (add) {
-        cv_grid(HW, C, N, gn_bwd_apply_kernel<true, 2>, cs_smem, chunks, ppc);
-        gn_bwd_apply_kernel<true, 2><<<dim3(chunks, N), T, cs_smem, st>>>(
-            static_cast<const __nv_bfloat16*>(x), static_cast<const __nv_bfloat16*>(dy),
-            static_cast<const __nv_bfloat16*>(add), static_cast<__nv_bfloat16*>(dx), mr, gsum, gamma, beta, HW, C, G,
-            ppc, silu, dx_colsum);
-    } else {
-        cv_grid(HW, C, N, gn_bwd_apply_kernel<false, 3>, cs_smem, chunks, ppc);
-        gn_bwd_apply_kernel<false, 3><<<dim3(chunks, N), T, cs_smem, st>>>(
-            static_cast<const __nv_bfloat16*>(x), static_cast<const __nv_bfloat16*>(dy), nullptr,
-            static_cast<__nv_bfloat16*>(dx), mr, gsum, gamma, beta, HW, C, G, ppc, silu, dx_colsum);
-    }
-    VQB_CUDA(cudaGetLastError());
-    count_launch(2);
-    return VQB_OK;
+    return gn_bwd_finish(x, dy, add, dx, gamma, beta, mr, dgamma, dbeta, cs, gsum, N, HW, C, G, silu, dx_colsum, st);
+}
+
+int vqb_gn_silu_bwd_sums(const void* x, const void* dy, const void* add, void* dx, const float* gamma,
+                         const float* beta, const float* mr, const float* sums, float* dgamma, float* dbeta, float* ws,
+                         int N, int HW, int C, int G, int silu, float* dx_colsum, void* stream) {
+    VQB_CHECK(x && dy && dx && gamma && beta && mr && sums && dgamma && dbeta && ws,
+              "vqb_gn_silu_bwd_sums: null pointer");
+    VQB_CHECK(N > 0 && HW > 0 && G > 0 && C % 8 == 0 && C % G == 0 && C <= 2048 && (silu == 0 || silu == 1),
+              "vqb_gn_silu_bwd_sums: N=%d HW=%d C=%d G=%d silu=%d unsupported", N, HW, C, G, silu);
+    if (!device_is_sm90()) return set_error(VQB_ENODEVICE, "vqb_gn_silu_bwd_sums: current device is not sm_90");
+    return gn_bwd_finish(x, dy, add, dx, gamma, beta, mr, dgamma, dbeta, sums, ws, N, HW, C, G, silu, dx_colsum,
+                         static_cast<cudaStream_t>(stream));
 }
 
 int vqb_wavelet_fwd(const float* x, void* y, const float* filt, int N, int C, int H, int W, int Cpad, void* stream) {
diff --git a/vqgan-training_b200/csrc/ptx.cuh b/vqgan-training_b200/csrc/ptx.cuh
--- a/vqgan-training_b200/csrc/ptx.cuh
+++ b/vqgan-training_b200/csrc/ptx.cuh
@@ -4,6 +4,10 @@
 #include <cuda.h>
 #include <cuda_runtime.h>
 #include <cuda_bf16.h>
+
+#ifndef VQB_EXACT_SIGMOID
+#define VQB_EXACT_SIGMOID 0
+#endif
 
 namespace vqb {
 
@@ -278,4 +282,27 @@
 __device__ __forceinline__ void from_f32(float& d, float v) { d = v; }
 __device__ __forceinline__ void from_f32(__nv_bfloat16& d, float v) { d = __float2bfloat16(v); }
 
-}
+__device__ __forceinline__ void red_add_v4(float* p, float4 v) {
+    asm volatile("red.global.add.v4.f32 [%0], {%1, %2, %3, %4};" ::"l"(p), "f"(v.x), "f"(v.y), "f"(v.z), "f"(v.w)
+                 : "memory");
+}
+
+__device__ __forceinline__ float tanh_fast(float x) {
+#if VQB_EXACT_SIGMOID
+    return 2.f / (1.f + __expf(-2.f * x)) - 1.f;
+#else
+    float t;
+    asm("tanh.approx.f32 %0, %1;" : "=f"(t) : "f"(x));
+    return t;
+#endif
+}
+
+__device__ __forceinline__ float gn_bwd_du2(float dy, float x, float a2, float b2, bool silu) {
+    if (!silu) return 2.f * dy;
+    const float h = fmaf(x, a2, b2);
+    const float t = tanh_fast(h);
+    const float r = fmaf(-h, t, h + 1.f);
+    return dy * fmaf(t, r, r);
+}
+
+}
diff --git a/vqgan-training_b200/native.py b/vqgan-training_b200/native.py
--- a/vqgan-training_b200/native.py
+++ b/vqgan-training_b200/native.py
@@ -75,6 +75,11 @@
                 ("W", C.c_int32), ("nviews", C.c_int32), ("ntaps", C.c_int32), ("ksplit", C.c_int32),
                 ("_pad", C.c_int32), ("ld_override", C.c_int64), ("col_offset", C.c_int64), ("dy_view", VqbView3d),
                 ("views", VqbView3d * VQB_MAX_VIEWS_3D), ("taps", VqbTap3d * VQB_MAX_TAPS_3D)]
+
+
+class VqbGnBwdFuse(C.Structure):
+    _fields_ = [("x", C.c_void_p), ("mr", C.c_void_p), ("gamma", C.c_void_p), ("beta", C.c_void_p),
+                ("sums", C.c_void_p), ("groups", C.c_int32), ("silu", C.c_int32)]
 
 
 class VqbAdamwGroup(C.Structure):
@@ -129,6 +134,9 @@
         "vqb_nhwc_to_nchw_pad": (i32, [vp, vp, i32, i32, i32, i32, i32, i32, vp, vp]),
         "vqb_gn_silu_fwd_pre": (i32, [vp, vp, vp, vp, vp, vp, i32, i32, i32, i32, f32, i32, vp]),
         "vqb_conv_stats_ok": (i32, [C.POINTER(VqbConvDesc)]),
+        "vqb_conv_gemm_gnbwd": (i32, [C.POINTER(VqbConvDesc), vp, vp, vp, C.POINTER(VqbGnBwdFuse), vp]),
+        "vqb_conv_gnbwd_ok": (i32, [C.POINTER(VqbConvDesc)]),
+        "vqb_gn_silu_bwd_sums": (i32, [vp] * 11 + [i32] * 5 + [vp, vp]),
         "vqb_pack_weights_fold": (i32, [vp, vp, i32, i32, i32, i32, vp, i32, i32, vp]),
         "vqb_wgrad_reduce_fold": (i32, [vp, vp, i32, i32, i32, i32, i32, i32, i32, vp, vp]),
         "vqb_adamw_flat": (i32, [vp, vp, vp, vp, vp, i64, i32, C.POINTER(VqbAdamwGroup), f32, vp]),
diff --git a/vqgan-training_b200/ops.py b/vqgan-training_b200/ops.py
--- a/vqgan-training_b200/ops.py
+++ b/vqgan-training_b200/ops.py
@@ -1,5 +1,6 @@
 from __future__ import annotations
 
+import collections
 import math
 import os
 import threading
@@ -303,7 +304,8 @@
 
 
 def run_conv_gemm(g: plans.ConvGeom, a: torch.Tensor, wp: torch.Tensor, Cout: int, out: torch.Tensor, out_strides,
-                  out_ptr_offset_bytes=0, bias=None, res=None, mask=None, relu=False, out_f32=False, stats=None):
+                  out_ptr_offset_bytes=0, bias=None, res=None, mask=None, relu=False, out_f32=False, stats=None,
+                  gn=None, gn_sums=None):
     flags = (EPI_BIAS if bias is not None else 0) | (EPI_RES if res is not None else 0) | \
             (EPI_MASK if mask is not None else 0) | (EPI_RELU if relu else 0) | \
             (native.EPI_STATS if stats is not None else 0)
@@ -314,9 +316,27 @@
         d = plans.conv_desc(g, Cout, out_strides, flags, out_f32)
         descs[dk] = d
     off = out_ptr_offset_bytes
+    if gn is not None:
+        assert flags == 0 and not out_f32 and off == 0
+        x, mr, gamma, beta, groups, silu = gn
+        ga, be = gamma.detach().float(), beta.detach().float()
+        f = native.VqbGnBwdFuse(x=ptr(x), mr=ptr(mr), gamma=ptr(ga), beta=ptr(be), sums=ptr(gn_sums), groups=groups,
+                                silu=1 if silu else 0)
+        check(_L().vqb_conv_gemm_gnbwd(d, ptr(a), ptr(wp), ptr(out), f, stream_ptr()), "conv_gemm_gnbwd")
+        return
     check(_L().vqb_conv_gemm(d, ptr(a), ptr(wp), ptr(bias), (ptr(res) + off) if res is not None else 0,
                              (ptr(mask) + off) if mask is not None else 0, ptr(out) + off, ptr(stats), stream_ptr()),
           "conv_gemm")
+
+
+def conv_gnbwd_supported(g: plans.ConvGeom, Cout: int, out_strides) -> bool:
+    descs = g.__dict__.setdefault("_descs", {})
+    key = ("gnbwd_ok", Cout, tuple(out_strides))
+    ok = descs.get(key)
+    if ok is None:
+        ok = bool(_L().vqb_conv_gnbwd_ok(plans.conv_desc(g, Cout, out_strides, 0, False)))
+        descs[key] = ok
+    return ok
 
 
 def conv_stats_supported(g: plans.ConvGeom, Cout: int, out_strides) -> bool:
@@ -377,6 +397,34 @@
     return None
 
 
+class _GnSums(threading.local):
+    def __init__(self):
+        self.d = collections.OrderedDict()
+
+
+_gn_sums = _GnSums()
+_GN_SUMS_KEEP = 4
+
+
+def _put_gn_sums(dy: torch.Tensor, x: torch.Tensor, sums: torch.Tensor):
+    d = _gn_sums.d
+    d[dy.data_ptr()] = (dy, dy._version, x.data_ptr(), sums)
+    while len(d) > _GN_SUMS_KEEP:
+        d.popitem(last=False)
+
+
+def _take_gn_sums(dy: torch.Tensor, x: torch.Tensor):
+    ent = _gn_sums.d.pop(dy.data_ptr(), None)
+    if ent is None:
+        return None
+    t, ver, xp, sums = ent
+    N, H, W, C = x.shape
+    if (t.shape == dy.shape and t.stride() == dy.stride() and t.dtype == dy.dtype and dy._version == ver
+            and xp == x.data_ptr() and sums.shape == (N, C, 2)):
+        return sums
+    return None
+
+
 def colsum(x2d_rows: int, x: torch.Tensor, C: int, out=None) -> torch.Tensor:
     if out is None:
         out = torch.empty(C, device=x.device, dtype=torch.float32)
@@ -569,7 +617,8 @@
 class ConvFn(torch.autograd.Function):
 
     @staticmethod
-    def forward(ctx, x, weight, bias, residual, cache, kind, relu, input_is_relu, nchw_out, want_stats=False):
+    def forward(ctx, x, weight, bias, residual, cache, kind, relu, input_is_relu, nchw_out, want_stats=False,
+                gn=None):
         require_cuda(x)
         N, H, W, Cp = x.shape
         Cout, Cin, KH, KW = weight.shape
@@ -605,6 +654,7 @@
         ctx.cache, ctx.kind = cache, kind
         ctx.has_bias, ctx.has_res = bias is not None, residual is not None
         ctx.input_is_relu, ctx.nchw_out = input_is_relu, nchw_out
+        ctx.gn = gn
         if want_stats and not nchw_out:
             if stats is None:
                 stats = torch.empty(0, device=x.device)
@@ -617,8 +667,8 @@
         x, weight = ctx.saved_tensors
         inference_only(weight)
         gx, gw, gb, gres = conv_backward(x, weight, gout, ctx.cache, ctx.kind, ctx.has_bias, ctx.has_res,
-                                         ctx.input_is_relu, ctx.nchw_out, ctx.needs_input_grad[:4])
-        return gx, gw, gb, gres, None, None, None, None, None, None
+                                         ctx.input_is_relu, ctx.nchw_out, ctx.needs_input_grad[:4], gn_link=ctx.gn)
+        return gx, gw, gb, gres, None, None, None, None, None, None, None
 
 
 def _conv_geom(cache, kind, N, H, W, Cp, KH):
@@ -634,7 +684,7 @@
     raise ValueError(kind)
 
 
-def conv_backward(x, weight, gout, cache, kind, has_bias, has_res, input_is_relu, nchw_out, needs):
+def conv_backward(x, weight, gout, cache, kind, has_bias, has_res, input_is_relu, nchw_out, needs, gn_link=None):
     N, H, W, Cp = x.shape
     Cout, Cin, KH, KW = weight.shape
     g, H, W = _conv_geom(cache, kind, N, H, W, Cp, KH)
@@ -667,7 +717,7 @@
             gx = gx_alloc(N, H, W, Cp, device=x.device, dtype=torch.bfloat16)
             gdf = cache.geom(("dfat", N, H, W), lambda: plans.geom_fat3(N, H, W, dgrad=True))
             wpd = _fat_weights(cache, weight, ("dgrad", "fat3"), gdf.tapmap, True, Cop)
-            run_conv_gemm(gdf, dy, wpd, Cin, gx, plans.nhwc_strides(H, W, Cp), mask=mask)
+            _dgrad_s1(gdf, dy, wpd, Cin, gx, mask, gn_link)
         else:
             gx = gx_alloc(N, H, W, Cp, device=x.device, dtype=torch.bfloat16)
         if kind == "fat3" or dy_framed:
@@ -675,7 +725,7 @@
         elif kind == "s1":
             gd = cache.geom(("d", N, H, W), lambda: plans.geom_s1_dgrad(N, H, W, Cop, KH))
             wpd = cache.get(weight, ("dgrad", kind), gd.tapmap, True, Cop)
-            run_conv_gemm(gd, dy, wpd, Cin, gx, plans.nhwc_strides(H, W, Cp), mask=mask)
+            _dgrad_s1(gd, dy, wpd, Cin, gx, mask, gn_link)
         elif kind == "s2":
             for ph, pw, gd in cache.geom(("d", N, H, W), lambda: plans.geom_s2_dgrad_classes(N, H, W, Cop)):
                 wpd = cache.get(weight, ("dgrad", kind, ph, pw), gd.tapmap, True, Cop)
@@ -709,12 +759,23 @@
     return gx, gw, gb, gres
 
 
+def _dgrad_s1(gd, dy, wpd, Cin, gx, mask, gn):
+    N, H, W, Cp = gx.shape
+    ostr = plans.nhwc_strides(H, W, Cp)
+    if gn is not None and mask is None and Cp == Cin and conv_gnbwd_supported(gd, Cin, ostr):
+        sums = torch.zeros(N, Cin, 2, device=gx.device, dtype=torch.float32)
+        run_conv_gemm(gd, dy, wpd, Cin, gx, ostr, gn=gn, gn_sums=sums)
+        _put_gn_sums(gx, gn[0], sums)
+    else:
+        run_conv_gemm(gd, dy, wpd, Cin, gx, ostr, mask=mask)
+
+
 def conv(x, weight, bias, cache, kind="s1", residual=None, relu=False, input_is_relu=False, nchw_out=False,
-         want_stats=False):
+         want_stats=False, gn=None):
     if want_stats and not nchw_out:
-        out, st = ConvFn.apply(x, weight, bias, residual, cache, kind, relu, input_is_relu, nchw_out, True)
+        out, st = ConvFn.apply(x, weight, bias, residual, cache, kind, relu, input_is_relu, nchw_out, True, gn)
         return out, (st if st.numel() > 0 else None)
-    return ConvFn.apply(x, weight, bias, residual, cache, kind, relu, input_is_relu, nchw_out, False)
+    return ConvFn.apply(x, weight, bias, residual, cache, kind, relu, input_is_relu, nchw_out, False, gn)
 
 
 class UpConvFn(torch.autograd.Function):
@@ -815,13 +876,15 @@
         ctx.save_for_backward(x, gamma, beta, mr)
         ctx.groups, ctx.silu, ctx.with_skip = groups, silu, with_skip
         ctx.set_materialize_grads(False)
+        ctx.mark_non_differentiable(mr)
         if with_skip:
-            return y, x.view_as(x)
-        return y
-
-    @staticmethod
-    def backward(ctx, gy, gskip=None):
+            return y, x.view_as(x), mr
+        return y, mr
+
+    @staticmethod
+    def backward(ctx, gy, *grads):
         x, gamma, beta, mr = ctx.saved_tensors
+        gskip = grads[0] if ctx.with_skip else None
         inference_only(gamma, beta)
         if gy is None:
             return (gskip, None, None, None, None, None, None, None)
@@ -865,17 +928,28 @@
     add = gskip.contiguous() if gskip is not None else None
     dx = torch.empty_like(x)
     dg, db = grad_out(gamma), grad_out(beta)
-    ws = torch.empty(N * C * 2 + N * groups * 2, device=x.device, dtype=torch.float32)
     ga, be = gamma.detach().float(), beta.detach().float()
     cs = torch.empty(C, device=x.device, dtype=torch.float32)
-    check(_L().vqb_gn_silu_bwd(ptr(x), ptr(gy), ptr(add), ptr(dx), ptr(ga), ptr(be), ptr(mr), ptr(dg), ptr(db),
-                               ptr(ws), N, H * W, C, groups, 1 if silu else 0, ptr(cs), stream_ptr()), "gn_silu_bwd")
+    sums = _take_gn_sums(gy, x)
+    if sums is not None:
+        ws = torch.empty(N * groups * 2, device=x.device, dtype=torch.float32)
+        check(_L().vqb_gn_silu_bwd_sums(ptr(x), ptr(gy), ptr(add), ptr(dx), ptr(ga), ptr(be), ptr(mr), ptr(sums),
+                                        ptr(dg), ptr(db), ptr(ws), N, H * W, C, groups, 1 if silu else 0, ptr(cs),
+                                        stream_ptr()), "gn_silu_bwd_sums")
+    else:
+        ws = torch.empty(N * C * 2 + N * groups * 2, device=x.device, dtype=torch.float32)
+        check(_L().vqb_gn_silu_bwd(ptr(x), ptr(gy), ptr(add), ptr(dx), ptr(ga), ptr(be), ptr(mr), ptr(dg), ptr(db),
+                                   ptr(ws), N, H * W, C, groups, 1 if silu else 0, ptr(cs), stream_ptr()),
+              "gn_silu_bwd")
     _dx_colsum_slot[0] = (dx, dx._version, cs)
     return dx, dg, db
 
 
-def group_norm_silu(x, gamma, beta, groups=32, eps=1e-6, silu=True, with_skip=False, chsums=None):
-    return GroupNormSiLUFn.apply(x, gamma, beta, groups, eps, silu, with_skip, chsums)
+def group_norm_silu(x, gamma, beta, groups=32, eps=1e-6, silu=True, with_skip=False, chsums=None, with_mr=False):
+    out = GroupNormSiLUFn.apply(x, gamma, beta, groups, eps, silu, with_skip, chsums)
+    if with_mr:
+        return out
+    return out[:-1] if with_skip else out[0]
 
 
 class ResnetBlockRecomputeFn(torch.autograd.Function):
@@ -920,7 +994,8 @@
         need_res = need_hn or (sw is not None and (nig[11] or nig[12]))
         gx = gn1w = gn1b = gc1w = gc1b = gn2w = gn2b = gsw = gsb = None
         gh2, gc2w, gc2b, gskip = conv_backward(h2, c2w, gout, k2, "s1", c2b is not None, True, False, False,
-                                               (need_h2, nig[9], nig[10], need_res))
+                                               (need_h2, nig[9], nig[10], need_res),
+                                               gn_link=(h, mr2, n2w, n2b, g2, True))
         del h2
         if sw is not None and need_res:
             gskip, gsw, gsb, _ = conv_backward(x, sw, gskip, ks, "s1", sb is not None, False, False, False,
@@ -930,7 +1005,8 @@
             del h, gh2
             if need_h:
                 ghn, gc1w, gc1b, _ = conv_backward(hn, c1w, gh, k1, "s1", c1b is not None, False, False, False,
-                                                   (need_hn, nig[5], nig[6], False))
+                                                   (need_hn, nig[5], nig[6], False),
+                                                   gn_link=(x, mr1, n1w, n1b, g1, True))
                 del hn, gh
                 if need_hn:
                     gx, gn1w, gn1b = gn_silu_bwd(x, ghn, gskip, n1w, n1b, mr1, g1, True)
```

Measured after the change: 166.4 (median of 6 runs). About the same (+0.8%).
